# CUG-EMI/HMCMT2D

Measured on NVIDIA B200. Metric: leapfrog_steps_per_sec, higher is better.
Workload: dtype f64 (complex128)

## Files before the change

hmcmt2d_b200/csrc/hmcmt_b200.cu:

```cuda
#include <dlfcn.h>
#include <nccl.h>

#include <algorithm>
#include <cmath>
#include <cstdlib>
#include <cstring>
#include <new>
#include <vector>

#include "../../include/hmcmt_b200.h"
#include "band_factor.cuh"
#include "band_solve.cuh"
#include "mf_solver.cuh"
#include "mt_kernels.cuh"

using namespace hmcmt;

namespace {

template <typename Tp>
struct DevBuf {
    Tp* p = nullptr;
    size_t n = 0;
    int alloc(size_t count) {
// ... 796 lines not shown
        pl->useMf = pl->T == 0 || wantMf;
        if (pl->useMf) pl->T = 0;
    }
    {
        const char* env = std::getenv("HMCMT_SPLIT");
        int want = env ? std::atoi(env) : 1;
        pl->dom = BandDom{M.N, M.nf, pl->b, M.nl, (!pl->useMf && want && M.nl >= 9) ? 1 : 0, M.nl / 2};
        if (!pl->useMf) {
            LocalDom L0 = LocalDom::make(pl->dom, 0);
            pl->steps0 = L0.sTot;
            pl->steps1 = pl->dom.split ? LocalDom::make(pl->dom, 1).sOwn : 0;
            pl->S = pl->steps0 + pl->steps1;
        }
    }
    pl->nSysPerChain = pl->nModes * pl->nFreq;
    pl->nSys = pl->nSysPerChain * pl->nChains;
    pl->nFull = pl->nFreq * pl->nRx * pl->nComp;
    pl->sm = SysMap{pl->nFreq, pl->nModes, pl->modeList[0], pl->modeList[1]};
    pl->h_yLen.assign(pr->yLen, pr->yLen + ny);
    pl->h_zLen.assign(pr->zLen, pr->zLen + nz);
    pl->h_freqs.assign(pr->freqs, pr->freqs + pr->nFreq);
    std::vector<double> yNode(ny + 1), zNode0(nz + 1), zNode(nz + 1);
    yNode[0] = 0; zNode0[0] = 0;
    for (int j = 0; j < ny; ++j) yNode[j + 1] = yNode[j] + pr->yLen[j];
    for (int k = 0; k < nz; ++k) zNode0[k + 1] = zNode0[k] + pr->zLen[k];
    for (auto& v : yNode) v -= pr->origin[0];
    for (int k = 0; k <= nz; ++k) zNode[k] = zNode0[k] - pr->origin[1];
    int zid = -1;
    for (int k = 0; k <= nz; ++k) if (std::fabs(zNode[k] - pr->rxLoc[1]) < 0.1) { zid = k; break; }
    if (zid < 0 || zid >= nz) { delete pl; return kErrArg; }
    M.zid = zid;
    std::vector<double> yCen(ny);
    for (int j = 0; j < ny; ++j) yCen[j] = 0.5 * (yNode[j] + yNode[j + 1]);
    std::vector<int> fid(pr->nRx), iL(pr->nRx), iR(pr->nRx), tjL(pr->nRx), tjR(pr->nRx);
    std::vector<double> d1(pr->nRx), d2(pr->nRx), wL(pr->nRx), wR(pr->nRx), twL(pr->nRx), twR(pr->nRx);
    for (int r = 0; r < pr->nRx; ++r) {
        double y = pr->rxLoc[2 * r];
        int id = -1;
        for (int j = 0; j <= ny; ++j) if (yNode[j] > y) { id = j; break; }
        if (id <= 0) { delete pl; return kErrArg; }
        fid[r] = id; d1[r] = y - yNode[id - 1]; d2[r] = yNode[id] - y;
        linear_interp(y, yNode, iL[r], iR[r], wL[r], wR[r]);
        linear_interp(y, yCen, tjL[r], tjR[r], twL[r], twR[r]);
    }
    std::vector<double> wdFull(pl->nFull, 0.0), wpFull(dataKind ? pl->nFull : 0, 0.0);
    std::vector<cplx> obsFull(pl->nFull, mk(0.0, 0.0));
    pl->h_packed2full.resize(pr->nData);
    const long nDt = dataKind ? 2 * pr->nComp : pr->nComp;
    long prev = -1;
    for (int i = 0; i < pr->nData; ++i) {
        long f = pr->freqID[i] - 1, r = pr->rxID[i] - 1, c = pr->dtID[i] - 1;
        if (f < 0 || f >= pr->nFreq || r < 0 || r >= pr->nRx || c < 0 || c >= nDt) { delete pl; return kErrArg; }
        const long ci = dataKind ? c / 2 : c, part = dataKind ? c % 2 : 0;
        const long slot = (f * pr->nRx + r) * pl->nComp + ci;
        const long full = dataKind ? 2 * slot + part : slot;
        if (full <= prev) {
            fprintf(stderr, "[hmcmt_b200] data rows must be sorted by (freq, rx, comp) without duplicates\n");
            delete pl;
            return kErrArg;
        }
        prev = full;
        pl->h_packed2full[i] = (int)full;
        const double w = 1.0 / std::fabs(pr->dataErr[i]);
        if (!dataKind) {
            wdFull[slot] = w;
            obsFull[slot] = mk(pr->obsData[2 * i], pr->obsData[2 * i + 1]);
        } else if (part == 0) {
            wdFull[slot] = w;
            obsFull[slot].x = pr->obsData[i];
        } else {
            wpFull[slot] = w;
            obsFull[slot].y = pr->obsData[i];
        }
    }
    std::vector<int> cell2act(M.nCell, -1);
    for (int a = 0; a < pr->nAC; ++a) {
        int c = pr->activeIdx[a];
        if (c < 0 || c >= M.nCell) { delete pl; return kErrArg; }
        cell2act[c] = a;
    }
    int rc = kOk;
    auto ok = [&](int r) { if (r && !rc) rc = r; };
    ok(pl->yLen.upload(pr->yLen, ny)); ok(pl->zLen.upload(pr->zLen, nz)); ok(pl->zNode.upload(zNode0.data(), nz + 1));
    ok(pl->freqs.upload(pr->freqs, pr->nFreq));
    ok(pl->fid.upload(fid.data(), pr->nRx)); ok(pl->iL.upload(iL.data(), pr->nRx)); ok(pl->iR.upload(iR.data(), pr->nRx));
    ok(pl->fdy1.upload(d1.data(), pr->nRx)); ok(pl->fdy2.upload(d2.data(), pr->nRx));
    ok(pl->wL.upload(wL.data(), pr->nRx)); ok(pl->wR.upload(wR.data(), pr->nRx));
    ok(pl->tjL.upload(tjL.data(), pr->nRx)); ok(pl->tjR.upload(tjR.data(), pr->nRx));
    ok(pl->twL.upload(twL.data(), pr->nRx)); ok(pl->twR.upload(twR.data(), pr->nRx));
    ok(pl->cell2act.upload(cell2act.data(), M.nCell)); ok(pl->act2cell.upload(pr->activeIdx, pr->nAC));
    ok(pl->bg.upload(pr->bgModel, M.nCell));
    ok(pl->wmPtr.upload(pr->wmRowPtr, pr->nAC + 1));
    int nnzWm = pr->wmRowPtr[pr->nAC];
    ok(pl->wmIdx.upload(pr->wmColIdx, nnzWm)); ok(pl->wmVal.upload(pr->wmVal, nnzWm));
    ok(pl->wd.upload(wdFull.data(), pl->nFull)); ok(pl->obs.upload(obsFull.data(), pl->nFull));
    ok(pl->wdPha.upload(wpFull.data(), wpFull.size()));
    ok(pl->packed2full.upload(pl->h_packed2full.data(), pr->nData));
    {
        std::vector<int> f2p((dataKind ? 2 : 1) * (size_t)pl->nFull, -1);
        for (int i = 0; i < pr->nData; ++i) f2p[pl->h_packed2full[i]] = i;
        ok(pl->full2packed.upload(f2p.data(), f2p.size()));
    }
    const size_t nCh = pl->nChains, nSys = pl->nSys, N = M.N;
    ok(pl->m.alloc(nCh * pr->nAC)); ok(pl->p.alloc(nCh * pr->nAC)); ok(pl->mref.alloc(nCh * pr->nAC));
    ok(pl->curM.alloc(nCh * pr->nAC)); ok(pl->curP.alloc(nCh * pr->nAC)); ok(pl->zmom.alloc(nCh * pr->nAC)); ok(pl->driftPart.alloc(nCh * 128));
    ok(pl->sigma.alloc(nCh * M.nCell)); ok(pl->meanSig.alloc(nCh * nz));
    ok(pl->planes.alloc(nCh * pl->nModes * 4 * N));
    ok(pl->bc.alloc(nSys * M.nb)); ok(pl->bcs.alloc(nSys * M.nb));
    ok(pl->rhs.alloc(nSys * N)); ok(pl->x.alloc(nSys * N)); ok(pl->lam.alloc(nSys * N));
    ok(pl->F.alloc(nSys * M.nNode)); ok(pl->Lam.alloc(nSys * M.nNode));
    ok(pl->srows.alloc(nSys * 2 * (ny + 1))); ok(pl->qrow.alloc(nSys * ny));
    ok(pl->scratch.alloc(nSys * 3 * prof_stride(nz)));
    ok(pl->Gpart.alloc(nSys * M.nCell)); ok(pl->phiPart.alloc(nSys)); ok(pl->phi.alloc(nCh));
    ok(pl->gsig.alloc(nCh * pr->nAC)); ok(pl->gdata.alloc(nCh * pr->nAC)); ok(pl->gtotal.alloc(nCh * pr->nAC)); ok(pl->xbuf.alloc((size_t)nCh * (pl->nAC + 1))); ok(pl->energies.alloc(nCh * 2));
    ok(pl->chainScal.alloc(nCh * 4));
    ok(pl->predFull.alloc(nCh * pl->nFull)); ok(pl->respFull.alloc(nCh * pl->nFull)); ok(pl->vin.alloc(nCh * pl->nFull)); ok(pl->predPacked.alloc(nCh * pr->nData));
    ok(pl->panels.alloc(nSys * (size_t)pl->S * panel_doubles(pl->T)));
    ok(pl->ainvz.alloc(nSys * (size_t)pl->S * AZ)); ok(pl->zadj.alloc(nSys * (size_t)pl->S * 8));
    const size_t wexpN = split_scratch_entries(TS * pl->T);
    ok(pl->wexp.alloc(pl->dom.split ? nSys * wexpN : 0));
    ok(pl->conCols.alloc(nSys * contract_cols_out(ny, nz)));
    ok(pl->fwdJobs.alloc(nSys));
    ok(pl->status.alloc(nSys)); ok(pl->driftFlag.alloc(1)); ok(pl->Lsteps.alloc(nCh));
    ok(pl->sysDesc.alloc(nSys)); ok(pl->jobs.alloc(nSys));
    if (rc) { hmcmt_destroy(pl); return rc; }
    cudaMemset(pl->status.p, 0, sizeof(int) * nSys);
    cudaMemset(pl->driftFlag.p, 0, sizeof(int));
    cudaMemset(pl->m.p, 0, sizeof(double) * nCh * pr->nAC);
    cudaMemset(pl->p.p, 0, sizeof(double) * nCh * pr->nAC);
    cudaMemset(pl->mref.p, 0, sizeof(double) * nCh * pr->nAC);
    M.yLen = pl->yLen.p; M.zLen = pl->zLen.p; M.zNode = pl->zNode.p;
    pl->rx = RxDev{pr->nRx, pl->fid.p, pl->fdy1.p, pl->fdy2.p, pl->iL.p, pl->iR.p, pl->wL.p, pl->wR.p, pl->tjL.p, pl->tjR.p, pl->twL.p, pl->twR.p};
    std::vector<BandSys> sd(nSys);
    std::vector<SolveJob> jb(nSys), jfw(nSys);
    for (size_t s = 0; s < nSys; ++s) {
        int f = (int)(s % pl->nFreq);
        int t = (int)(s / pl->nFreq);
        int mi = t % pl->nModes, ch = t / pl->nModes;
        double* P = pl->planes.p + ((size_t)(ch * pl->nModes + mi) * 4) * N;
        BandSys& d = sd[s];
        d.dr = P; d.dm = P + N; d.e1 = P + 2 * N; d.e2 = P + 3 * N;
        d.omega = 2.0 * kPi * pr->freqs[f];
        d.band = nullptr;
        d.rhs = pl->rhs.p + s * N;
        d.panels[0] = pl->panels.p + s * (size_t)pl->S * panel_doubles(pl->T);
        d.panels[1] = d.panels[0] + (size_t)pl->steps0 * panel_doubles(pl->T);
        d.ainvz[0] = pl->ainvz.p + s * (size_t)pl->S * AZ;
        d.ainvz[1] = d.ainvz[0] + (size_t)pl->steps0 * AZ;
        d.wexp = pl->dom.split ? pl->wexp.p + s * wexpN : nullptr;
        d.x = pl->x.p + s * N;
        d.status = pl->status.p + s;
        SolveJob& j = jb[s];
        j.panels[0] = d.panels[0]; j.panels[1] = d.panels[1];
        j.ainvz[0] = d.ainvz[0]; j.ainvz[1] = d.ainvz[1];
        j.rhs = pl->lam.p + s * N; j.x = pl->lam.p + s * N;
        j.zbuf[0] = pl->zadj.p + s * (size_t)pl->S * 8;
        j.zbuf[1] = j.zbuf[0] + (size_t)pl->steps0 * 8;
        j.wexp = d.wexp;
        SolveJob& jf = jfw[s];
        jf = j;
        jf.rhs = nullptr; jf.x = d.x;
    }
    if (cudaMemcpy(pl->sysDesc.p, sd.data(), sizeof(BandSys) * nSys, cudaMemcpyHostToDevice) != cudaSuccess ||
        cudaMemcpy(pl->jobs.p, jb.data(), sizeof(SolveJob) * nSys, cudaMemcpyHostToDevice) != cudaSuccess ||
        (pl->fwdJobs.p && cudaMemcpy(pl->fwdJobs.p, jfw.data(), sizeof(SolveJob) * nSys, cudaMemcpyHostToDevice) != cudaSuccess)) {
        hmcmt_destroy(pl);
        return kErrCuda;
    }
    {
        const size_t rxSmem = (size_t)(6 * (M.ny + 1) + 3 * M.ny) * sizeof(cplx);
        const size_t bcSmem = (size_t)boundary_profiles_per_block(M.nz) * M.nz * 6 * sizeof(cplx);
        if (bcSmem > 227 * 1024) {
            fprintf(stderr, "[hmcmt_b200] nz = %d: the boundary kernel needs %zu bytes of shared memory per profile\n", M.nz, bcSmem);
            hmcmt_destroy(pl);
            return kErrArg;
        }
        if (bcSmem > 48 * 1024 && cudaFuncSetAttribute(k_boundary, cudaFuncAttributeMaxDynamicSharedMemorySize, (int)bcSmem) != cudaSuccess) {
            hmcmt_destroy(pl);
            return kErrCuda;
        }
        pl->conStaged = contract_cols_smem(M.ny, M.nz, 1) <= 200 * 1024 ? 1 : 0;
        const size_t cSmem = contract_cols_smem(M.ny, M.nz, pl->conStaged);
        if ((rxSmem > 48 * 1024 && cudaFuncSetAttribute(rx_kernel(pl), cudaFuncAttributeMaxDynamicSharedMemorySize, (int)rxSmem) != cudaSuccess) ||
            (cSmem > 48 * 1024 && cudaFuncSetAttribute(k_contract_cols, cudaFuncAttributeMaxDynamicSharedMemorySize, (int)cSmem) != cudaSuccess)) {
            hmcmt_destroy(pl);
            return kErrArg;
        }
    }
    if (pl->useMf) {
        std::vector<std::vector<int>> sn;
        std::vector<mf::Entry> ent;
        mf::mf_order_grid(M.nl, M.nf, mf_leaf_size(), sn, mf_cross_size(), mf_push_size());
        mf::mf_grid_entries(M.nl, M.nf, ent);
        mf::Symbolic S;
        if (!mf::mf_symbolic(M.N, sn, ent, mf_small_front(), S)) { hmcmt_destroy(pl); return kErrArg; }
        int mrc = kOk;
        pl->mfs = mf::Solver::create(std::move(S), pl->nSys, 2, 3 * (int64_t)M.N, &mrc);
        if (!pl->mfs) { hmcmt_destroy(pl); return mrc; }
        std::vector<unsigned char> nzR(M.N, 0), nzA(M.N, 0);
        for (int kn = 1; kn <= nz - 1; ++kn)
            for (int jn = 1; jn <= ny - 1; ++jn) {
                const int q = M.fastZ ? (jn - 1) * M.nf + (kn - 1) : (kn - 1) * M.nf + (jn - 1);
                if (jn == 1 || jn == ny - 1 || kn == 1 || kn == nz - 1) nzR[q] = 1;
                if (kn == M.zid || kn == M.zid + 1) nzA[q] = 1;
            }
        pl->patRx = pl->mfs->add_rhs_pattern(nzA);
        if (pl->patRx < 0) { hmcmt_destroy(pl); return kErrAlloc; }
        if (const char* e = std::getenv("HMCMT_MF_PRUNE"); !e || std::atoi(e)) {
            pl->patRhs = pl->mfs->add_rhs_pattern(nzR);
            pl->patAdj = pl->patRx;
            if (pl->patRhs < 0) { hmcmt_destroy(pl); return kErrAlloc; }
        }
        std::vector<mf::MtValSys> mv(nSys);
        for (size_t s = 0; s < nSys; ++s) { mv[s].planes = sd[s].dr; mv[s].omega = sd[s].omega; }
        if (pl->mfSys.upload(mv.data(), nSys) != kOk) { hmcmt_destroy(pl); return kErrAlloc; }
    }
    if (cudaStreamCreateWithFlags(&pl->stream, cudaStreamNonBlocking) != cudaSuccess ||
        cudaStreamCreateWithFlags(&pl->side, cudaStreamNonBlocking) != cudaSuccess ||
        cudaEventCreateWithFlags(&pl->evFork, cudaEventDisableTiming) != cudaSuccess ||
        cudaEventCreateWithFlags(&pl->evJoin, cudaEventDisableTiming) != cudaSuccess ||
        cudaEventCreateWithFlags(&pl->evPre, cudaEventDisableTiming) != cudaSuccess ||
        cudaEventCreateWithFlags(&pl->evRhs, cudaEventDisableTiming) != cudaSuccess ||
        cudaEventCreate(&pl->evA) != cudaSuccess || cudaEventCreate(&pl->evB) != cudaSuccess) {
        hmcmt_destroy(pl);
        return kErrCuda;
    }
    if (const char* e = std::getenv("HMCMT_GRAPH"); e && !std::atoi(e)) pl->graphState = -1;
    if (pl->useMf) {
        const char* env = std::getenv("HMCMT_GROUPS");
        int G = env ? std::atoi(env) : kDefaultGroups;
        G = std::max(1, std::min(G, std::min(pl->nSys, 8)));
        for (int g = 0; G >= 2 && g < G; ++g) {
            cudaStream_t s = nullptr;
            cudaEvent_t e = nullptr;
            if (cudaStreamCreateWithFlags(&s, cudaStreamNonBlocking) != cudaSuccess) { hmcmt_destroy(pl); return kErrCuda; }
            pl->groupStreams.push_back(s);
            if (cudaEventCreateWithFlags(&e, cudaEventDisableTiming) != cudaSuccess) { hmcmt_destroy(pl); return kErrCuda; }
            pl->groupDone.push_back(e);
        }
    }
    *out = pl;
    return kOk;
}

int hmcmt_plan_create(const hmcmt_problem* pr, hmcmt_plan** out) { return plan_create(pr, out, 0); }
int hmcmt_plan_create_rho_phase(const hmcmt_problem* pr, hmcmt_plan** out) { return plan_create(pr, out, 1); }

void hmcmt_destroy(hmcmt_plan* pl) {
    if (!pl) return;
    cudaSetDevice(pl->device);
    if (pl->comm) {
        if (pl->stream) cudaStreamSynchronize(pl->stream);
        if (NcclApi* a = nccl_api()) a->commDestroy(pl->comm);
        pl->comm = nullptr;
    }
    if (pl->stream) { cudaStreamSynchronize(pl->stream); cudaStreamDestroy(pl->stream); }
    if (pl->side) { cudaStreamSynchronize(pl->side); cudaStreamDestroy(pl->side); }
    if (pl->graphExec) cudaGraphExecDestroy(pl->graphExec);
    for (cudaStream_t s : pl->groupStreams) { cudaStreamSynchronize(s); cudaStreamDestroy(s); }
    for (cudaEvent_t e : pl->groupDone) cudaEventDestroy(e);
    if (pl->evPre) cudaEventDestroy(pl->evPre);
    if (pl->evRhs) cudaEventDestroy(pl->evRhs);
    if (pl->evFork) cudaEventDestroy(pl->evFork);
    if (pl->evJoin) cudaEventDestroy(pl->evJoin);
    if (pl->evA) cudaEventDestroy(pl->evA);
    if (pl->evB) cudaEventDestroy(pl->evB);
    for (auto& e : pl->factorEvents) { cudaEventDestroy(e.first); cudaEventDestroy(e.second); }
    for (cudaEvent_t e : pl->factorMid) cudaEventDestroy(e);
    pl->yLen.release(); pl->zLen.release(); pl->zNode.release(); pl->freqs.release(); pl->fdy1.release(); pl->fdy2.release();
    pl->wL.release(); pl->wR.release(); pl->twL.release(); pl->twR.release(); pl->tjL.release(); pl->tjR.release(); pl->bg.release(); pl->wmVal.release(); pl->wd.release(); pl->wdPha.release(); pl->m.release(); pl->p.release();
    pl->mref.release(); pl->sigma.release(); pl->meanSig.release(); pl->planes.release(); pl->Gpart.release(); pl->phiPart.release();
    pl->phi.release(); pl->gsig.release(); pl->gdata.release(); pl->gtotal.release(); pl->energies.release(); pl->panels.release(); pl->curM.release();
    pl->curP.release(); pl->driftPart.release(); pl->chainScal.release(); pl->zmom.release(); pl->fid.release(); pl->iL.release(); pl->iR.release();
    pl->cell2act.release(); pl->act2cell.release(); pl->wmPtr.release(); pl->wmIdx.release(); pl->status.release();
    pl->driftFlag.release(); pl->packed2full.release(); pl->full2packed.release(); pl->Lsteps.release(); pl->obs.release(); pl->bc.release(); pl->bcs.release();
    pl->rhs.release(); pl->x.release(); pl->F.release(); pl->lam.release(); pl->Lam.release(); pl->srows.release(); pl->qrow.release();
    pl->scratch.release(); pl->predFull.release(); pl->ainvz.release(); pl->zadj.release(); pl->vin.release();
    pl->predPacked.release(); pl->conCols.release(); pl->dbc.release(); pl->jvFull.release(); pl->dsigA.release(); pl->gnBuf.release(); pl->gnVec.release(); pl->gnPart.release(); pl->gnS.release(); pl->gnE.release(); pl->gnAct.release(); pl->gnI.release(); pl->xbuf.release(); pl->wexp.release(); pl->respFull.release(); pl->gradK.release(); pl->Lband.release(); pl->massBuf.release(); pl->massStatus.release(); delete pl->massSolver; pl->massSolver = nullptr; pl->mfSys.release(); delete pl->mfs; pl->mfs = nullptr; pl->fwdJobs.release(); pl->sysDesc.release(); pl->jobs.release();
    if (pl->pin) cudaFreeHost(pl->pin);
    delete pl;
}

int64_t hmcmt_plan_info(const hmcmt_plan* pl, int what) {
    if (!pl) return -1;
    switch (what) {
        case 0: return pl->M.N;
        case 1: return pl->M.nNode;
        case 2: return pl->M.nCell;
        case 3: return pl->M.nb;
        case 4: return pl->b;
        case 5: return pl->T;
        case 6: return pl->S;
        case 7: return pl->nSysPerChain;
        case 8: return pl->M.zid;
        case 9: return pl->useMf ? pl->mfs->factor_doubles() * 8 : (int64_t)pl->S * (panel_doubles(pl->T) * 8 + AZ * 16);
        case 10: return pl->launches;
        case 11: return pl->useMf ? 1 : 0;
        case 12: return pl->useMf ? (int64_t)pl->mfs->factor_flops() : (int64_t)(4.0 * pl->M.N * (double)pl->b * pl->b);
        case 13: return pl->dom.split;
        default: return -1;
    }
}

int hmcmt_sync(hmcmt_plan* pl) {
    if (!pl) return kErrArg;
    HMCMT_CUDA_TRY(cudaStreamSynchronize(pl->stream));
    return kOk;
}
int hmcmt_set_mass_matrix(hmcmt_plan* pl, int32_t kind) {
    if (!pl || kind < 0 || kind > 1) return kErrArg;
    HMCMT_CUDA_TRY(cudaSetDevice(pl->device));
    if (kind == 0) { pl->massOn = false; return kOk; }
    if (pl->massSolver) { pl->massOn = true; return kOk; }
    const int n = pl->nAC;
    std::vector<int> ptr(n + 1), idx;
    std::vector<double> val;
    HMCMT_CUDA_TRY(cudaMemcpy(ptr.data(), pl->wmPtr.p, sizeof(int) * (n + 1), cudaMemcpyDeviceToHost));
    idx.resize(ptr[n]); val.resize(ptr[n]);
    HMCMT_CUDA_TRY(cudaMemcpy(idx.data(), pl->wmIdx.p, sizeof(int) * ptr[n], cudaMemcpyDeviceToHost));
    HMCMT_CUDA_TRY(cudaMemcpy(val.data(), pl->wmVal.p, sizeof(double) * ptr[n], cudaMemcpyDeviceToHost));
    std::vector<mf::Entry> ent;
    std::vector<int> aptr(n + 1, 0);
    int bw = 0;
    for (int a = 0; a < n; ++a)
        for (int q = ptr[a]; q < ptr[a + 1]; ++q) {
            const int j = idx[q];
            if (j > a) continue;
            ent.push_back(mf::Entry{a, j, q});
            bw = std::max(bw, a - j);
            if (j != a) { ++aptr[a + 1]; ++aptr[j + 1]; }
        }
    for (int a = 0; a < n; ++a) aptr[a + 1] += aptr[a];
    std::vector<int> adj(aptr[n]), at(aptr.begin(), aptr.end() - 1);
    for (const mf::Entry& e : ent)
        if (e.row != e.col) { adj[at[e.row]++] = e.col; adj[at[e.col]++] = e.row; }
    std::vector<std::vector<int>> sn;
    mf::mf_order_graph(n, aptr, adj, mf_leaf_size(), sn);
    mf::Symbolic S;
    if (!mf::mf_symbolic(n, sn, ent, mf_small_front(), S)) return kErrArg;
    int rc = kOk;
    pl->massSolver = mf::Solver::create(std::move(S), 1, pl->nChains, (int64_t)ptr[n], &rc);
    if (!pl->massSolver) return rc;
    {
        std::vector<cplx> cv(ptr[n]);
        for (int q = 0; q < ptr[n]; ++q) cv[q] = mk(val[q], 0.0);
        HMCMT_CUDA_TRY(cudaMemcpy(pl->massSolver->vals(), cv.data(), sizeof(cplx) * cv.size(), cudaMemcpyHostToDevice));
    }
    if ((rc = pl->massStatus.alloc(1)) != kOk) return rc;
    HMCMT_CUDA_TRY(cudaMemset(pl->massStatus.p, 0, sizeof(int)));
    rc = pl->massSolver->factor(pl->stream, pl->massStatus.p, &pl->launches);
    if (rc) return rc;
    int hst = 0;
    HMCMT_CUDA_TRY(cudaMemcpyAsync(&hst, pl->massStatus.p, sizeof(int), cudaMemcpyDeviceToHost, pl->stream));
    HMCMT_CUDA_TRY(cudaStreamSynchronize(pl->stream));
    if (hst) return hst;
    std::vector<double> Lb((size_t)n * (bw + 1), 0.0);
    for (int a = 0; a < n; ++a)
        for (int q = ptr[a]; q < ptr[a + 1]; ++q)
            if (idx[q] <= a) Lb[(size_t)a * (bw + 1) + (a - idx[q])] = val[q];
    for (int j = 0; j < n; ++j) {
        double* rj = Lb.data() + (size_t)j * (bw + 1);
        double d = rj[0];
        for (int k = std::max(0, j - bw); k < j; ++k) d -= rj[j - k] * rj[j - k];
        if (!(d > 0.0)) return kErrNotPosDef;
        d = std::sqrt(d);
        rj[0] = d;
        for (int i = j + 1; i <= std::min(n - 1, j + bw); ++i) {
            double* ri = Lb.data() + (size_t)i * (bw + 1);
            double v = ri[i - j];
            for (int k = std::max(0, i - bw); k < j; ++k) v -= ri[i - k] * rj[j - k];
            ri[i - j] = v / d;
        }
    }
    if ((rc = pl->Lband.upload(Lb.data(), Lb.size())) != kOk) return rc;
    if ((rc = pl->gradK.alloc((size_t)pl->nChains * n)) != kOk) return rc;
    if ((rc = pl->massBuf.alloc((size_t)pl->nChains * n)) != kOk) return rc;
    pl->massBw = bw;
    pl->massOn = true;
    return kOk;
}

int hmcmt_status(hmcmt_plan* pl) {
    if (!pl) return kErrArg;
    HMCMT_CUDA_TRY(cudaSetDevice(pl->device));
    return check_status(pl);
}
int hmcmt_set_response_kind(hmcmt_plan* pl, int32_t kind) {
    if (!pl || kind < 0 || kind > 1) return kErrArg;
    pl->respKind = kind;
    return kOk;
}
int hmcmt_get_responses(hmcmt_plan* pl, double* out) {
    if (!pl || !out || !pl->haveForward) return kErrArg;
    HMCMT_CUDA_TRY(cudaSetDevice(pl->device));
    const cplx* src = (pl->respKind == 1 || pl->dataKind == 1) ? pl->respFull.p : pl->predFull.p;
    HMCMT_CUDA_TRY(cudaMemcpyAsync(out, src, sizeof(cplx) * (size_t)pl->nChains * pl->nFull, cudaMemcpyDeviceToHost, pl->stream));
    HMCMT_CUDA_TRY(cudaStreamSynchronize(pl->stream));
    return kOk;
}
int hmcmt_timer_start(hmcmt_plan* pl) {
    if (!pl) return kErrArg;
    HMCMT_CUDA_TRY(cudaEventRecord(pl->evA, pl->stream));
    return kOk;
}
int hmcmt_timer_stop(hmcmt_plan* pl, float* ms) {
    if (!pl || !ms) return kErrArg;
    HMCMT_CUDA_TRY(cudaEventRecord(pl->evB, pl->stream));
    HMCMT_CUDA_TRY(cudaEventSynchronize(pl->evB));
    HMCMT_CUDA_TRY(cudaEventElapsedTime(ms, pl->evA, pl->evB));
    return kOk;
}
int hmcmt_kernel_time_split(hmcmt_plan* pl, float* factor_only_ms, float* forward_solve_ms) {
    if (!pl) return kErrArg;
    HMCMT_CUDA_TRY(cudaStreamSynchronize(pl->stream));
    float a = 0.f, b = 0.f;
    for (size_t i = 0; i < pl->factorEventsUsed; ++i) {
        float ms = 0.f;
        HMCMT_CUDA_TRY(cudaEventElapsedTime(&ms, pl->factorEvents[i].first, pl->factorMid[i]));
        a += ms;
        HMCMT_CUDA_TRY(cudaEventElapsedTime(&ms, pl->factorMid[i], pl->factorEvents[i].second));
        b += ms;
    }
    if (factor_only_ms) *factor_only_ms = a;
    if (forward_solve_ms) *forward_solve_ms = b;
    return kOk;
}
int hmcmt_kernel_time(hmcmt_plan* pl, int reset, float* factor_ms, int64_t* factor_launches) {
    if (!pl) return kErrArg;
    HMCMT_CUDA_TRY(cudaStreamSynchronize(pl->stream));
    float tot = 0.f;
    for (size_t i = 0; i < pl->factorEventsUsed; ++i) {
        float ms = 0.f;
        HMCMT_CUDA_TRY(cudaEventElapsedTime(&ms, pl->factorEvents[i].first, pl->factorEvents[i].second));
        tot += ms;
    }
    if (factor_ms) *factor_ms = tot;
    if (factor_launches) *factor_launches = (int64_t)pl->factorEventsUsed;
    if (reset) { pl->factorEventsUsed = 0; pl->timeFactor = reset > 0; }
    return kOk;
}

static int upload_model(hmcmt_plan* pl, const double* m) {
    size_t bytes = sizeof(double) * (size_t)pl->nChains * pl->nAC;
    int rc = ensure_pin(pl, std::max(bytes, (size_t)1 << 20));
    if (rc) return rc;
    std::memcpy(pl->pin, m, bytes);
    HMCMT_CUDA_TRY(cudaMemcpyAsync(pl->m.p, pl->pin, bytes, cudaMemcpyHostToDevice, pl->stream));
    return kOk;
}
static size_t datum_bytes(const hmcmt_plan* pl) { return pl->dataKind ? sizeof(double) : sizeof(cplx); }
static int pack_pred(hmcmt_plan* pl) {
    const dim3 grid((pl->nData + 255) / 256, pl->nChains);
    if (pl->dataKind)
        k_pack_pred_real<<<grid, 256, 0, pl->stream>>>(pl->nData, pl->nFull, pl->packed2full.p, reinterpret_cast<const double*>(pl->respFull.p),
                                                       reinterpret_cast<double*>(pl->predPacked.p));
    else
        k_pack_pred<<<grid, 256, 0, pl->stream>>>(pl->nData, pl->nFull, pl->packed2full.p, pl->predFull.p, pl->predPacked.p);
    LAUNCH_CHECK(pl);
    return kOk;
}
static int download_pred(hmcmt_plan* pl, double* pred) {
    int rc = pack_pred(pl);
    if (rc) return rc;
    HMCMT_CUDA_TRY(cudaMemcpyAsync(pred, pl->predPacked.p, datum_bytes(pl) * (size_t)pl->nChains * pl->nData, cudaMemcpyDeviceToHost, pl->stream));
    return kOk;
}

static int forward_common(hmcmt_plan* pl, double* pred, double* exTE, double* hxTM);

int hmcmt_forward(hmcmt_plan* pl, const double* m, double* pred, double* exTE, double* hxTM) {
    if (!pl || !m) return kErrArg;
    HMCMT_CUDA_TRY(cudaSetDevice(pl->device));
    pl->sigmaDirect = false;
    int rc = upload_model(pl, m);
    if (rc) return rc;
    return forward_common(pl, pred, exTE, hxTM);
}

int hmcmt_forward_sigma(hmcmt_plan* pl, const double* sigma, double* pred, double* exTE, double* hxTM) {
    if (!pl || !sigma) return kErrArg;
    HMCMT_CUDA_TRY(cudaSetDevice(pl->device));
    pl->sigmaDirect = true;
    HMCMT_CUDA_TRY(cudaMemcpyAsync(pl->sigma.p, sigma, sizeof(double) * (size_t)pl->nChains * pl->M.nCell, cudaMemcpyHostToDevice, pl->stream));
    HMCMT_CUDA_TRY(cudaStreamSynchronize(pl->stream));
    return forward_common(pl, pred, exTE, hxTM);
}

static int forward_common(hmcmt_plan* pl, double* pred, double* exTE, double* hxTM) {
    int rc = compute_step(pl, false, nullptr);
    if (rc) return rc;
    if (pred) { rc = download_pred(pl, pred); if (rc) return rc; }
    const MeshDev& M = pl->M;
    for (int ch = 0; ch < pl->nChains; ++ch)
        for (int mi = 0; mi < pl->nModes; ++mi) {
            double* dst = pl->modeList[mi] == 0 ? exTE : hxTM;
            if (!dst) continue;
            size_t sys0 = ((size_t)ch * pl->nModes + mi) * pl->nFreq;
            HMCMT_CUDA_TRY(cudaMemcpyAsync(dst + 2 * (size_t)ch * pl->nFreq * M.nNode, pl->F.p + sys0 * M.nNode,
                                           sizeof(cplx) * (size_t)pl->nFreq * M.nNode, cudaMemcpyDeviceToHost, pl->stream));
        }
    HMCMT_CUDA_TRY(cudaStreamSynchronize(pl->stream));
    return check_status(pl);
}

int hmcmt_jtvec(hmcmt_plan* pl, const double* v, double* gsig) {
    if (!pl || !v || !gsig) return kErrArg;
    if (!pl->haveForward) return kErrArg;
    HMCMT_CUDA_TRY(cudaSetDevice(pl->device));
    std::vector<cplx> full((size_t)pl->nChains * pl->nFull, mk(0.0, 0.0));
    double* fullD = reinterpret_cast<double*>(full.data());
    for (int ch = 0; ch < pl->nChains; ++ch)
        for (int i = 0; i < pl->nData; ++i) {
            const size_t src = (size_t)ch * pl->nData + i;
            if (pl->dataKind) fullD[(size_t)ch * 2 * pl->nFull + pl->h_packed2full[i]] = v[src];
            else full[(size_t)ch * pl->nFull + pl->h_packed2full[i]] = mk(v[2 * src], v[2 * src + 1]);
        }
    HMCMT_CUDA_TRY(cudaMemcpyAsync(pl->vin.p, full.data(), sizeof(cplx) * full.size(), cudaMemcpyHostToDevice, pl->stream));
    HMCMT_CUDA_TRY(cudaStreamSynchronize(pl->stream));
    int rc = kOk;
    if (!pl->haveSens) rc = launch_sens_side(pl);
    if (rc) return rc;
    rc = rx_phase(pl, true, pl->vin.p);
    if (rc) return rc;
    rc = adjoint_phase(pl);
    if (rc) return rc;
    HMCMT_CUDA_TRY(cudaMemcpyAsync(gsig, pl->gsig.p, sizeof(double) * (size_t)pl->nChains * pl->nAC, cudaMemcpyDeviceToHost, pl->stream));
    HMCMT_CUDA_TRY(cudaStreamSynchronize(pl->stream));
    return check_status(pl);
}

int hmcmt_jacobian(hmcmt_plan* pl, double* J) {
    if (!pl || !J || !pl->haveForward) return kErrArg;
    HMCMT_CUDA_TRY(cudaSetDevice(pl->device));
    const MeshDev& M = pl->M;
    cudaStream_t st = pl->stream;
    const size_t nJ = (size_t)pl->nChains * pl->nData * pl->nAC * (pl->dataKind ? 1 : 2);
    DevBuf<double> dJ;
    int rc = dJ.alloc(nJ);
    if (rc) return rc;
    HMCMT_CUDA_TRY(cudaMemsetAsync(dJ.p, 0, nJ * sizeof(double), st));
    if (!pl->haveSens) rc = launch_sens_side(pl);
    struct Group { unsigned mask; int2 comp; };
    std::vector<Group> groups;
    const CompMap& cm = pl->cm;
    if (!pl->tipper) groups.push_back(Group{(1u << pl->nComp) - 1u, make_int2(0, 1)});
    else if (cm.zc[0] >= 0 || cm.zc[1] >= 0)
        groups.push_back(Group{(cm.zc[0] >= 0 ? 1u << cm.zc[0] : 0u) | (cm.zc[1] >= 0 ? 1u << cm.zc[1] : 0u), make_int2(cm.zc[0], cm.zc[1])});
    if (pl->tipper) groups.push_back(Group{1u << cm.tc, make_int2(cm.tmi == 0 ? cm.tc : -1, cm.tmi == 1 ? cm.tc : -1)});
    for (const Group& grp : groups)
        for (int r = 0; r < pl->nRx && rc == kOk; ++r)
            for (int part = 0; part < 2 && rc == kOk; ++part) {
                k_jac_vin<<<dim3((pl->nFull + 255) / 256, pl->nChains), 256, 0, st>>>(pl->nFull, pl->nRx, pl->nComp, grp.mask, r,
                                                                                     part == 0 ? mk(1.0, 0.0) : mk(0.0, 1.0), pl->vin.p);
                ++pl->launches;
                rc = rx_phase(pl, true, pl->vin.p);
                if (rc == kOk) rc = adjoint_phase(pl, false);
                if (rc != kOk) break;
                const dim3 grid((pl->nAC + 255) / 256, pl->nSys);
                if (pl->dataKind)
                    k_jac_rows_real<<<grid, 256, 0, st>>>(pl->nAC, M.nCell, pl->nFreq, pl->nRx, pl->nModes, pl->nData, r, part, pl->act2cell.p,
                                                          pl->full2packed.p, pl->Gpart.p, dJ.p);
                else
                    k_jac_rows<<<grid, 256, 0, st>>>(pl->nAC, M.nCell, pl->nFreq, pl->nRx, pl->nModes, pl->nComp, grp.comp, pl->nData, r,
                                                     part, pl->act2cell.p, pl->full2packed.p, pl->Gpart.p, dJ.p);
                ++pl->launches;
            }
    if (rc == kOk && cudaGetLastError() != cudaSuccess) rc = kErrCuda;
    if (rc == kOk && cudaMemcpyAsync(J, dJ.p, nJ * sizeof(double), cudaMemcpyDeviceToHost, st) != cudaSuccess) rc = kErrCuda;
    if (cudaStreamSynchronize(st) != cudaSuccess && rc == kOk) rc = kErrCuda;
    dJ.release();
    if (rc) return rc;
    rc = rx_phase(pl, false, nullptr);
    if (rc) return rc;
    return check_status(pl);
}

static int ensure_tangent(hmcmt_plan* pl) {
    if (pl->jvFull.p) return kOk;
    const MeshDev& M = pl->M;
    int rc;
    if ((rc = pl->dbc.alloc((size_t)pl->nSys * M.nb)) || (rc = pl->dsigA.alloc((size_t)pl->nChains * pl->nAC))) return rc;
    const size_t smem = (size_t)(6 * (M.ny + 1) + 2 * M.ny) * sizeof(cplx);
    auto k = pl->dataKind ? k_rx_tangent<true, false> : pl->tipper ? k_rx_tangent<false, true> : k_rx_tangent<false, false>;
    if (smem > 48 * 1024) HMCMT_CUDA_TRY(cudaFuncSetAttribute(k, cudaFuncAttributeMaxDynamicSharedMemorySize, (int)smem));
    return pl->jvFull.alloc((size_t)pl->nChains * pl->nFull);
}

static int jvec_device(hmcmt_plan* pl) {
    const MeshDev& M = pl->M;
    cudaStream_t st = pl->stream;
    const int nSys = pl->nSys;
    int rc = kOk;
    if (!pl->haveSens && (rc = launch_sens_side(pl))) return rc;
    HMCMT_CUDA_TRY(cudaStreamWaitEvent(st, pl->evJoin, 0));
    k_bc_tangent<<<dim3((M.ny + 1 + 127) / 128, nSys), 128, 0, st>>>(M, pl->sm, pl->freqs.p, pl->cell2act.p, pl->dsigA.p, pl->nAC,
                                                                     pl->scratch.p, pl->dbc.p);
    LAUNCH_CHECK(pl);
    k_tangent_rhs<<<dim3((M.N + 255) / 256, nSys), 256, 0, st>>>(M, pl->sm, pl->freqs.p, pl->sigma.p, pl->cell2act.p, pl->dsigA.p, pl->nAC,
                                                                 pl->F.p, pl->bcs.p, pl->dbc.p, pl->lam.p);
    LAUNCH_CHECK(pl);
    if (pl->useMf) {
        if ((rc = pl->mfs->forward_slot(st, 0, pl->lam.p, M.N, &pl->launches, 0, nSys, 0)) ||
            (rc = pl->mfs->backward_slot(st, 0, pl->lam.p, M.N, &pl->launches, 0, nSys, pl->patRx)))
            return rc;
    } else {
        if ((rc = launch_solve(st, pl->T, pl->jobs.p, nSys, pl->dom))) return rc;
// ... 555 lines not shown
```

hmcmt2d_b200/csrc/mf_kernels.cuh:

```cuda
#pragma once
#include "band_factor.cuh"
#include "mf_solver.cuh"

namespace hmcmt {
namespace mf {

__host__ __device__ __forceinline__ size_t kg_off(int ld, int i, int j, int plane) {
    return ((size_t)((j >> 2) * 2 + plane) * ld + i) * 4 + (j & 3);
}

struct Tables {
    const Front* fronts;
    const int* rows;
    const int* rel;
    const int* children;
    const OrigEntry* orig;
    const Chunk* chunks;
    const int* pos2orig;
    double* fac;
    double* arena[2];
    int64_t facStride, arenaStride[2];
    const cplx* vals;
    int64_t valStride;
    int* status;
    unsigned long long* prof;
};
#define MF_PROF_MARK(slot) do { if (tb.prof && threadIdx.x == 0) { const long long _t = clock64(); atomicAdd(tb.prof + _pc * 8 + (slot), (unsigned long long)(_t - _t0)); _t0 = _t; } } while (0)

__device__ __forceinline__ int tl_off(int r, int c) { return ((c >> 2) << 5) | (r << 2) | (c & 3); }
__device__ __forceinline__ double* mf_tile(double* tiles, int I, int J) { return tiles + (size_t)(I * (I + 1) / 2 + J) * 128; }
__device__ __forceinline__ int mf_pc_row(int I, int npb) { return I < npb ? I * (I + 1) / 2 : npb * (npb + 1) / 2 + (I - npb) * npb; }
template <bool PC>
__device__ __forceinline__ double* mf_tile(double* tiles, int npb, int I, int J) {
    return PC ? tiles + (size_t)(mf_pc_row(I, npb) + J) * 128 : mf_tile(tiles, I, J);
}

struct TileFrag {
    double re[2], im[2];
};
__device__ __forceinline__ void frag_load(TileFrag& f, const double* T, int lane) {
    f.re[0] = T[lane]; f.re[1] = T[32 + lane]; f.im[0] = T[64 + lane]; f.im[1] = T[96 + lane];
}
__device__ __forceinline__ void frag_load_t(TileFrag& f, const double* T, int g, int t) {
    const int o0 = tl_off(t, g), o1 = tl_off(4 + t, g);
    f.re[0] = T[o0]; f.re[1] = T[o1]; f.im[0] = T[64 + o0]; f.im[1] = T[64 + o1];
}
__device__ __forceinline__ void frag_store(const TileFrag& f, double* T, int lane) {
    T[lane] = f.re[0]; T[32 + lane] = f.re[1]; T[64 + lane] = f.im[0]; T[96 + lane] = f.im[1];
}
__device__ __forceinline__ void cfrag_load(TileFrag& c, const double* T, int g, int t) {
    const int o = tl_off(g, 2 * t);
    const double2 r = *reinterpret_cast<const double2*>(T + o), i = *reinterpret_cast<const double2*>(T + 64 + o);
    c.re[0] = r.x; c.re[1] = r.y; c.im[0] = i.x; c.im[1] = i.y;
}
__device__ __forceinline__ void cfrag_store(const TileFrag& c, double* T, int g, int t, double sign = 1.0) {
    const int o = tl_off(g, 2 * t);
    *reinterpret_cast<double2*>(T + o) = make_double2(sign * c.re[0], sign * c.re[1]);
    *reinterpret_cast<double2*>(T + 64 + o) = make_double2(sign * c.im[0], sign * c.im[1]);
}
__device__ __forceinline__ void frag_mma(TileFrag& c, TileFrag& x, const TileFrag& a, const TileFrag& b) {
#pragma unroll
    for (int kk = 0; kk < 2; ++kk) {
        dmma884(c.re, a.re[kk], b.re[kk]);
        dmma884(c.im, a.re[kk], b.im[kk]);
        dmma884(x.re, -a.im[kk], b.im[kk]);
        dmma884(x.im, a.im[kk], b.re[kk]);
    }
}
__device__ __forceinline__ void frag_zero(TileFrag& c) { c.re[0] = c.re[1] = c.im[0] = c.im[1] = 0.0; }
__device__ __forceinline__ void frag_add(TileFrag& c, const TileFrag& x) {
    c.re[0] += x.re[0]; c.re[1] += x.re[1]; c.im[0] += x.im[0]; c.im[1] += x.im[1];
}

template <int NW, bool PC = false, bool STREAM = false>
__device__ __forceinline__ void mf_front_factor(double* __restrict__ tiles, double* __restrict__ scratch, double* __restrict__ mbuf,
                                                double* __restrict__ nainv, int* __restrict__ fail, const int nb, const int npb,
                                                const int sReal, unsigned long long* __restrict__ prof = nullptr,
                                                double* mglob = nullptr, const int ldm = 0) {
    const int tid = threadIdx.x, lane = tid & 31;
    long long _s0 = prof ? clock64() : 0;
#define MF_SWEEP_MARK(slot) do { if (prof && tid == 0) { const long long _t = clock64(); atomicAdd(prof + (slot), (unsigned long long)(_t - _s0)); _s0 = _t; } } while (0)
    const int warp = __shfl_sync(0xffffffffu, tid >> 5, 0);
    const int g = lane >> 2, t = lane & 3;
    double* const rawb = scratch;
    double* const mmb = scratch + (size_t)npb * 128;
    for (int kb = 0; kb < npb; ++kb) {
        if (warp == 0) {
            const double* D = mf_tile(tiles, kb, kb);
            auto sym = [&](int r, int c, int pl) { return r >= c ? D[pl * 64 + tl_off(r, c)] : D[pl * 64 + tl_off(c, r)]; };
            cplx a0 = mk(sym(g, 2 * t, 0), sym(g, 2 * t, 1)), a1 = mk(sym(g, 2 * t + 1, 0), sym(g, 2 * t + 1, 1));
            bool bad = false;
            const int left = sReal - 8 * kb;
            gj_invert8<(NW > 4)>(a0, a1, bad, g, t, left < 8 ? (left < 0 ? 0 : left) : 8);
            if (__any_sync(0xffffffffu, bad) && lane == 0) *fail = 1;
            TileFrag p;
            p.re[0] = -a0.x; p.re[1] = -a1.x; p.im[0] = -a0.y; p.im[1] = -a1.y;
            cfrag_store(p, nainv, g, t);
            __syncwarp();
            double* Dw = mf_tile(tiles, kb, kb);
            cfrag_store(p, Dw, g, t);
        }
        if (npb == 1) break;
        __syncthreads();
        MF_SWEEP_MARK(0);
        for (int I = warp; I < npb; I += NW) {
            if (I == kb) continue;
            TileFrag a, b, c, x;
            if (I > kb) frag_load(a, mf_tile(tiles, I, kb), lane);
            else frag_load_t(a, mf_tile(tiles, kb, I), g, t);
            frag_load(b, nainv, lane);
            frag_zero(c); frag_zero(x);
            frag_mma(c, x, a, b);
            frag_add(c, x);
            frag_store(a, rawb + (size_t)I * 128, lane);
            cfrag_store(c, mmb + (size_t)I * 128, g, t);
        }
        __syncthreads();
        MF_SWEEP_MARK(1);
        {
            int I = 0, J = warp;
            while (J > I) { J -= I + 1; ++I; }
            for (int L = warp; L < npb * (npb + 1) / 2; L += NW) {
                double* T = mf_tile(tiles, I, J);
                if (I == kb && J == kb) {
                } else if (J == kb) {
                    TileFrag c;
                    cfrag_load(c, mmb + (size_t)I * 128, g, t);
                    cfrag_store(c, T, g, t, -1.0);
                } else if (I == kb) {
                    const double* Ms = mmb + (size_t)J * 128;
                    TileFrag c;
                    c.re[0] = Ms[tl_off(2 * t, g)]; c.re[1] = Ms[tl_off(2 * t + 1, g)];
                    c.im[0] = Ms[64 + tl_off(2 * t, g)]; c.im[1] = Ms[64 + tl_off(2 * t + 1, g)];
                    cfrag_store(c, T, g, t, -1.0);
                } else {
                    TileFrag a, b, c, x;
                    frag_load(a, mmb + (size_t)I * 128, lane);
                    frag_load(b, rawb + (size_t)J * 128, lane);
                    cfrag_load(c, T, g, t);
                    frag_zero(x);
                    frag_mma(c, x, a, b);
                    frag_add(c, x);
                    cfrag_store(c, T, g, t);
                }
                J += NW;
                while (J > I) { J -= I + 1; ++I; }
            }
        }
        __syncthreads();
        MF_SWEEP_MARK(1);
    }
    const int nub = nb - npb;
    if (nub == 0) { __syncthreads(); return; }
    __syncthreads();
    if (npb == 1) MF_SWEEP_MARK(0);
    for (int Iu = warp; Iu < nub; Iu += NW) {
        const int I = npb + Iu;
        for (int kb = 0; kb < npb; ++kb) {
            TileFrag c, x;
            frag_zero(c); frag_zero(x);
            for (int j = 0; j < npb; ++j) {
                TileFrag a, b;
                frag_load(a, mf_tile<PC>(tiles, npb, I, j), lane);
                if (kb >= j) frag_load(b, mf_tile(tiles, kb, j), lane);
                else frag_load_t(b, mf_tile(tiles, j, kb), g, t);
                frag_mma(c, x, a, b);
            }
            frag_add(c, x);
            if (STREAM) {
                double* o = mglob + kg_off(ldm, 8 * Iu + g, 8 * kb + 2 * t, 0);
                *reinterpret_cast<double2*>(o) = make_double2(-c.re[0], -c.re[1]);
                *reinterpret_cast<double2*>(o + 4 * ldm) = make_double2(-c.im[0], -c.im[1]);
            } else {
                cfrag_store(c, mbuf + (size_t)(Iu * npb + kb) * 128, g, t);
            }
        }
    }
    __syncthreads();
    MF_SWEEP_MARK(2);
    if (PC) return;
    {
        const int nU = nub * (nub + 1) / 2;
        int I = 0, J = warp;
        while (J > I) { J -= I + 1; ++I; }
        constexpr bool kPair = NW > 4;
        for (int L = warp; L < nU; L += (kPair ? 2 : 1) * NW) {
            const int I0 = I, J0 = J;
            J += NW;
            while (J > I) { J -= I + 1; ++I; }
            const bool two = kPair && L + NW < nU;
            const int I1 = I, J1 = J;
            if (kPair) {
                J += NW;
                while (J > I) { J -= I + 1; ++I; }
            }
            double* T0 = mf_tile(tiles, npb + I0, npb + J0);
            double* T1 = mf_tile(tiles, npb + I1, npb + J1);
            TileFrag c0, x0, c1, x1;
            cfrag_load(c0, T0, g, t);
            frag_zero(x0);
            if (two) { cfrag_load(c1, T1, g, t); frag_zero(x1); }
            for (int kb = 0; kb < npb; ++kb) {
                TileFrag a, b;
                frag_load(a, mbuf + (size_t)(I0 * npb + kb) * 128, lane);
                frag_load(b, mf_tile(tiles, npb + J0, kb), lane);
                frag_mma(c0, x0, a, b);
                if (two) {
                    frag_load(a, mbuf + (size_t)(I1 * npb + kb) * 128, lane);
                    frag_load(b, mf_tile(tiles, npb + J1, kb), lane);
                    frag_mma(c1, x1, a, b);
                }
            }
            frag_add(c0, x0);
            cfrag_store(c0, T0, g, t);
            if (two) { frag_add(c1, x1); cfrag_store(c1, T1, g, t); }
        }
    }
    __syncthreads();
    MF_SWEEP_MARK(3);
#undef MF_SWEEP_MARK
}

template <bool TRANSPOSED>
__device__ __forceinline__ void mf_store_tile(const double* __restrict__ T, double* __restrict__ dst, int ld, int row0, int col0,
                                              double sign, int lane) {
#pragma unroll
    for (int h = 0; h < 2; ++h) {
        const int idx = lane + 32 * h;
        const int chunk = idx >> 4, w = idx & 15, pl = chunk >> 1, cg = chunk & 1, r = w >> 1, c2 = (w & 1) * 2;
        double2 v;
        if (!TRANSPOSED) v = *reinterpret_cast<const double2*>(T + chunk * 32 + w * 2);
        else v = make_double2(T[pl * 64 + tl_off(cg * 4 + c2, r)], T[pl * 64 + tl_off(cg * 4 + c2 + 1, r)]);
        double* out = dst + kg_off(ld, row0 + r, col0 + cg * 4, pl) + c2;
        *reinterpret_cast<double2*>(out) = make_double2(sign * v.x, sign * v.y);
    }
}

template <int NW, bool STREAM>
__device__ __forceinline__ void mf_small_front(const Tables& tb, const SmallDesc* __restrict__ descs) {
    constexpr int NT = NW * 32;
    constexpr bool kMid = NW >= 8;
    static_assert(!STREAM || kMid, "streamed M' exists in the pivot-column layout only");
    extern __shared__ __align__(16) unsigned char mf_smem[];
    SmallDesc& F = *reinterpret_cast<SmallDesc*>(mf_smem);
    const int sys = blockIdx.y, tid = threadIdx.x, lane = tid & 31;
    const int warp = __shfl_sync(0xffffffffu, tid >> 5, 0);
    constexpr int _pc = NW <= 2 ? 0 : (NW == 4 ? 1 : (NW == 8 ? 2 : 3));
    long long _t0 = clock64();
    static_assert(sizeof(SmallDesc) % 4 == 0 && sizeof(SmallDesc) <= kFrontDescBytes, "SmallDesc is copied word by word into the head of the dynamic shared memory");
    for (int i = tid; i < (int)(sizeof(SmallDesc) / 4); i += NT)
        reinterpret_cast<int*>(&F)[i] = reinterpret_cast<const int*>(descs + blockIdx.x)[i];
    __syncthreads();
    const int fp = F.sp + F.up, nb = fp >> 3, npb = F.sp >> 3, nub = nb - npb;
    const int nT = kMid ? mf_pc_row(nb, npb) : nb * (nb + 1) / 2;
    double* tiles = reinterpret_cast<double*>(mf_smem + kFrontDescBytes);
    double* mbuf = tiles + (size_t)nT * 128;
    double* nainv = mbuf + (size_t)(STREAM || 2 * npb > nub * npb ? 2 * npb : nub * npb) * 128;
    int* fail = reinterpret_cast<int*>(nainv + 128);
    int2* relS = reinterpret_cast<int2*>(fail + 4);
    auto rel_parts = [npb](int r) {
        return make_int2((kMid ? mf_pc_row(r >> 3, npb) : (r >> 3) * ((r >> 3) + 1) / 2) * 128 + (r & 7) * 4, (r >> 3) * 128 + ((r & 4) << 3) + (r & 3));
    };
    const int nChild = F.nChild;
    {
        int base = 0;
        for (int c = 0; c < nChild; ++c) {
            const int cu = F.cU[c];
            const int* rel = tb.rel + F.cRel[c];
            for (int i = tid; i < cu; i += NT) relS[base + i] = rel_parts(rel[i]);
            base += cu;
        }
    }
    int* invS = reinterpret_cast<int*>(relS + ((F.cU[0] + F.cU[1] + F.cU[2] + F.cU[3] + 1) & ~1));
    const double* carena = tb.arena[F.par ^ 1] + (size_t)sys * tb.arenaStride[F.par ^ 1];
    constexpr int kBatch = 1;
    struct Batch {
        double2 r01[kBatch], r23[kBatch], i01[kBatch], i23[kBatch];
        int ii[kBatch], jg[kBatch];
        int c;
    };
    int curC = 0, curQ = warp * kBatch;
    auto load_batch = [&](Batch& bt) {
        while (curC < nChild) {
            const int cu = F.cU[curC];
            if (curQ < (((kMid ? F.cPiv[curC] : cu) + 3) >> 2) * ((cu + 31) >> 5)) break;
            ++curC;
            curQ = warp * kBatch;
        }
        bt.c = curC < nChild ? curC : -1;
        if (bt.c < 0) return;
        const int cu = F.cU[curC], ld = F.cLd[curC], off = F.cFirst[curC];
        const double* U = carena + F.cOff[curC];
        const int ng = ((kMid ? F.cPiv[curC] : cu) + 3) >> 2, nrb = (cu + 31) >> 5;
#pragma unroll
        for (int bq = 0; bq < kBatch; ++bq) {
            const int q = curQ + bq;
            const int jg = nrb == 1 ? q : q / nrb, i = (q - jg * nrb) * 32 + lane;
            bt.jg[bq] = jg;
            bt.ii[bq] = (q < ng * nrb && i < cu && i >= 4 * jg) ? i : -1;
            if (bt.ii[bq] >= 0) {
                const double* pr = U + kg_off(ld, off + i, off + 4 * jg, 0);
                const double* pi = U + kg_off(ld, off + i, off + 4 * jg, 1);
                bt.r01[bq] = *reinterpret_cast<const double2*>(pr); bt.r23[bq] = *reinterpret_cast<const double2*>(pr + 2);
                bt.i01[bq] = *reinterpret_cast<const double2*>(pi); bt.i23[bq] = *reinterpret_cast<const double2*>(pi + 2);
            }
        }
        curQ += NW * kBatch;
    };
    Batch b0, b1;
    load_batch(b0);
    load_batch(b1);
    const cplx* vals = tb.vals + (size_t)sys * tb.valStride;
    OrigEntry oe0{0, 0, -1};
    cplx ov0 = mk(0.0, 0.0);
    if (tid < F.nOrig) {
        oe0 = tb.orig[F.origPtr + tid];
        ov0 = oe0.src < 0 ? mk(1.0, 0.0) : vals[oe0.src];
    }
    for (int i = tid; i < nT * 64; i += NT) reinterpret_cast<double2*>(tiles)[i] = make_double2(0.0, 0.0);
    if (kMid)
        for (int i = tid; i < nChild * F.up; i += NT) invS[i] = -1;
    if (tid == 0) *fail = 0;
    __syncthreads();
    MF_PROF_MARK(0);
    if (kMid) {
        int base = 0;
        for (int c = 0; c < nChild; ++c) {
            const int cu = F.cU[c];
            const int* rel = tb.rel + F.cRel[c];
            for (int i = F.cPiv[c] + tid; i < cu; i += NT) invS[base + rel[i] - F.sp] = i;
            base += F.up;
        }
    }
    auto addr = [&](int a, int b) {
        return tiles + (size_t)((kMid ? mf_pc_row(a >> 3, npb) : (a >> 3) * ((a >> 3) + 1) / 2) + (b >> 3)) * 128 + tl_off(a & 7, b & 7);
    };
    {
        auto scatter = [&](const Batch& bt) {
            const int2* relC = relS + ((bt.c > 0 ? F.cU[0] : 0) + (bt.c > 1 ? F.cU[1] : 0) + (bt.c > 2 ? F.cU[2] : 0));
            const int jEnd = kMid ? F.cPiv[bt.c] : 0;
#pragma unroll
            for (int bq = 0; bq < kBatch; ++bq) {
                const int i = bt.ii[bq];
                if (i < 0) continue;
                const int jg = bt.jg[bq];
                const double re[4] = {bt.r01[bq].x, bt.r01[bq].y, bt.r23[bq].x, bt.r23[bq].y};
                const double im[4] = {bt.i01[bq].x, bt.i01[bq].y, bt.i23[bq].x, bt.i23[bq].y};
                double* rowp = tiles + relC[i].x;
#pragma unroll
                for (int jj = 0; jj < 4; ++jj) {
                    if (4 * jg + jj > i || (kMid && 4 * jg + jj >= jEnd)) break;
                    double* d = rowp + relC[4 * jg + jj].y;
                    d[0] += re[jj];
                    d[64] += im[jj];
                }
            }
        };
        for (int c = 0; c < nChild; ++c) {
            while (b0.c == c) {
                scatter(b0);
                b0 = b1;
                load_batch(b1);
            }
            __syncwarp();
            __syncthreads();
        }
        if (nChild == 0) __syncthreads();
    }
    MF_PROF_MARK(2);
    if (tid < F.nOrig) {
        double* d = addr(oe0.lrow, oe0.lcol);
        d[0] += ov0.x;
        d[64] += ov0.y;
    }
    for (int e = tid + NT; e < F.nOrig; e += NT) {
        const OrigEntry oe = tb.orig[F.origPtr + e];
        const cplx v = oe.src < 0 ? mk(1.0, 0.0) : vals[oe.src];
        double* d = addr(oe.lrow, oe.lcol);
        d[0] += v.x;
        d[64] += v.y;
    }
    __syncthreads();
    MF_PROF_MARK(1);
    double* fac = tb.fac + (size_t)sys * tb.facStride;
    mf_front_factor<NW, kMid, STREAM>(tiles, mbuf, mbuf, nainv, fail, nb, npb, F.s, tb.prof ? tb.prof + 32 + _pc * 4 : nullptr,
                                      fac + F.mOff, F.up);
    if (kMid && nub > 0) {
        const long long tD = tb.prof ? clock64() : 0;
        const int g = lane >> 2, t = lane & 3, up = F.up;
        double* U = tb.arena[F.par] + (size_t)sys * tb.arenaStride[F.par] + F.uOff;
        auto gather = [&](TileFrag& c, int I, int J) {
            const int a = 8 * I + g, b = 8 * J + 2 * t;
            frag_zero(c);
#pragma unroll
            for (int ch = 0; ch < kSmallChildren; ++ch) {
                const int* inv = invS + ch * up;
                const int ia = ch < nChild ? inv[a] : -1;
                if (ia < 0) continue;
                const int ib0 = inv[b], ib1 = inv[b + 1];
                const double* Uc = carena + F.cOff[ch];
                const int ld = F.cLd[ch], off = F.cFirst[ch];
                if (ib0 >= 0 && ib0 <= ia) { c.re[0] += Uc[kg_off(ld, off + ia, off + ib0, 0)]; c.im[0] += Uc[kg_off(ld, off + ia, off + ib0, 1)]; }
                if (ib1 >= 0 && ib1 <= ia) { c.re[1] += Uc[kg_off(ld, off + ia, off + ib1, 0)]; c.im[1] += Uc[kg_off(ld, off + ia, off + ib1, 1)]; }
            }
        };
        auto store = [&](const TileFrag& c, int I, int J) {
            double* o = U + kg_off(up, 8 * I + g, 8 * J + 2 * t, 0);
            *reinterpret_cast<double2*>(o) = make_double2(c.re[0], c.re[1]);
            *reinterpret_cast<double2*>(o + 4 * up) = make_double2(c.im[0], c.im[1]);
        };
        if (!STREAM) {
            const int nU = nub * (nub + 1) / 2;
            int I = 0, J = warp;
            while (J > I) { J -= I + 1; ++I; }
            for (int L = warp; L < nU; L += 2 * NW) {
                const int I0 = I, J0 = J;
                J += NW;
                while (J > I) { J -= I + 1; ++I; }
                const bool two = L + NW < nU;
                const int I1 = I, J1 = J;
                J += NW;
                while (J > I) { J -= I + 1; ++I; }
                TileFrag c0, x0, c1, x1;
                gather(c0, I0, J0);
                frag_zero(x0);
                if (two) { gather(c1, I1, J1); frag_zero(x1); }
                for (int kb = 0; kb < npb; ++kb) {
                    TileFrag a, b;
                    frag_load(a, mbuf + (size_t)(I0 * npb + kb) * 128, lane);
                    frag_load(b, mf_tile<true>(tiles, npb, npb + J0, kb), lane);
                    frag_mma(c0, x0, a, b);
                    if (two) {
                        frag_load(a, mbuf + (size_t)(I1 * npb + kb) * 128, lane);
                        frag_load(b, mf_tile<true>(tiles, npb, npb + J1, kb), lane);
                        frag_mma(c1, x1, a, b);
                    }
                }
                frag_add(c0, x0);
                store(c0, I0, J0);
                if (two) { frag_add(c1, x1); store(c1, I1, J1); }
            }
        } else {
            constexpr int kRow = 4;
            const double* Mg = fac + F.mOff;
            auto load_a = [&](TileFrag& a, int I, int kb) {
#pragma unroll
                for (int kk = 0; kk < 2; ++kk) {
                    const double* p = Mg + kg_off(up, 8 * I + g, 8 * kb + 4 * kk + t, 0);
                    a.re[kk] = -p[0];
                    a.im[kk] = -p[4 * up];
                }
            };
            int I = 0, q = warp;
            while (q > I / kRow) { q -= I / kRow + 1; ++I; }
            while (I < nub) {
                const int J0 = kRow * q, nJ = min(kRow, I + 1 - J0);
                TileFrag c[kRow], x[kRow];
#pragma unroll
                for (int r = 0; r < kRow; ++r)
                    if (r < nJ) { gather(c[r], I, J0 + r); frag_zero(x[r]); }
                TileFrag a;
                load_a(a, I, 0);
                for (int kb = 0; kb < npb; ++kb) {
                    TileFrag an;
                    if (kb + 1 < npb) load_a(an, I, kb + 1);
#pragma unroll
                    for (int r = 0; r < kRow; ++r)
                        if (r < nJ) {
                            TileFrag b;
                            frag_load(b, mf_tile<true>(tiles, npb, npb + J0 + r, kb), lane);
                            frag_mma(c[r], x[r], a, b);
                        }
                    a = an;
                }
#pragma unroll
                for (int r = 0; r < kRow; ++r)
                    if (r < nJ) { frag_add(c[r], x[r]); store(c[r], I, J0 + r); }
                q += NW;
                while (I < nub && q > I / kRow) { q -= I / kRow + 1; ++I; }
            }
        }
        if (tb.prof && tid == 0) atomicAdd(tb.prof + 32 + _pc * 4 + 3, (unsigned long long)(clock64() - tD));
    }
    MF_PROF_MARK(4);
    if (tid == 0 && *fail) tb.status[sys] = kErrSingular;
    const int sp = F.sp, up = F.up;
    {
        double* G = fac + F.gOff;
        for (int I = warp; I < npb; I += NW)
            for (int J = 0; J < npb; ++J) {
                if (I >= J) mf_store_tile<false>(mf_tile(tiles, I, J), G, sp, I * 8, J * 8, -1.0, lane);
                else mf_store_tile<true>(mf_tile(tiles, J, I), G, sp, I * 8, J * 8, -1.0, lane);
            }
    }
    if (!STREAM && up > 0) {
        double* M = fac + F.mOff;
        for (int I = warp; I < nub; I += NW)
            for (int J = 0; J < npb; ++J) mf_store_tile<false>(mbuf + (size_t)(I * npb + J) * 128, M, up, I * 8, J * 8, -1.0, lane);
    }
    if (!kMid && up > 0) {
        double* U = tb.arena[F.par] + (size_t)sys * tb.arenaStride[F.par] + F.uOff;
        int I = 0, J = warp;
        while (J > I) { J -= I + 1; ++I; }
        for (int L = warp; L < nub * (nub + 1) / 2; L += NW) {
            mf_store_tile<false>(mf_tile(tiles, npb + I, npb + J), U, up, I * 8, J * 8, 1.0, lane);
            J += NW;
            while (J > I) { J -= I + 1; ++I; }
        }
    }
    MF_PROF_MARK(5);
    if (tb.prof && tid == 0) { atomicAdd(tb.prof + _pc * 8 + 6, 1ull); atomicAdd(tb.prof + _pc * 8 + 7, (unsigned long long)npb); }
}

template <int NW>
__global__ void __launch_bounds__(NW * 32, NW <= 4 ? (NW == 1 ? 16 : 32 / NW) : (NW == 8 ? 4 : 2))
mf_small_kernel(Tables tb, const SmallDesc* __restrict__ descs) {
    mf_small_front<NW, false>(tb, descs);
}
__global__ void __launch_bounds__(16 * 32, 1) mf_small_stream_kernel(Tables tb, const SmallDesc* __restrict__ descs) {
    mf_small_front<16, true>(tb, descs);
}

__global__ void mf_asm_orig_kernel(Tables tb, const int2* __restrict__ pairs, int n) {
    const int idx = blockIdx.x * blockDim.x + threadIdx.x, sys = blockIdx.y;
    if (idx >= n) return;
    const int2 pr = pairs[idx];
    const Front& F = tb.fronts[pr.x];
    const OrigEntry oe = tb.orig[pr.y];
    const cplx v = oe.src < 0 ? mk(1.0, 0.0) : tb.vals[(size_t)sys * tb.valStride + oe.src];
    double* A = tb.arena[F.depth & 1] + (size_t)sys * tb.arenaStride[F.depth & 1] + F.frontOff;
    const int fp = F.sp + F.up;
    A[kg_off(fp, oe.lrow, oe.lcol, 0)] += v.x;
    A[kg_off(fp, oe.lrow, oe.lcol, 1)] += v.y;
}
struct AsmTile {
    int front, bi, bj;
    int invPtr;
};
__global__ void __launch_bounds__(256)
mf_asm_gather_kernel(Tables tb, const AsmTile* __restrict__ tilesList, const int* __restrict__ invMaps) {
    const AsmTile at = tilesList[blockIdx.x];
    const int sys = blockIdx.y;
    const Front P = tb.fronts[at.front];
    const int fp = P.sp + P.up, par = P.depth & 1;
    double* A = tb.arena[par] + (size_t)sys * tb.arenaStride[par] + P.frontOff;
    const double* carena = tb.arena[par ^ 1] + (size_t)sys * tb.arenaStride[par ^ 1];
    for (int item = threadIdx.x; item < 64 * 16; item += 256) {
        const int a = at.bi * 64 + (item & 63), b0 = at.bj * 64 + (item >> 6) * 4;
        if (a >= fp || b0 >= ((a >> 3) + 1) * 8) continue;
        double re[4] = {0.0, 0.0, 0.0, 0.0}, im[4] = {0.0, 0.0, 0.0, 0.0};
        for (int c = 0; c < P.nChild; ++c) {
            const int* inv = invMaps + at.invPtr + (size_t)c * fp;
            const int ia = inv[a];
            if (ia < 0) continue;
            const Front& C = tb.fronts[tb.children[P.childPtr + c]];
            const int ld = C.isBig ? C.sp + C.up : C.up, off = C.isBig ? C.sp : 0;
            const double* U = carena + C.frontOff;
#pragma unroll
            for (int k = 0; k < 4; ++k) {
                if (b0 + k > a) break;
                const int ib = inv[b0 + k];
                if (ib < 0) continue;
                re[k] += U[kg_off(ld, off + ia, off + ib, 0)];
                im[k] += U[kg_off(ld, off + ia, off + ib, 1)];
            }
        }
        double* pr = A + kg_off(fp, a, b0, 0);
        double* pi = A + kg_off(fp, a, b0, 1);
        *reinterpret_cast<double2*>(pr) = make_double2(re[0], re[1]); *reinterpret_cast<double2*>(pr + 2) = make_double2(re[2], re[3]);
        *reinterpret_cast<double2*>(pi) = make_double2(im[0], im[1]); *reinterpret_cast<double2*>(pi + 2) = make_double2(im[2], im[3]);
    }
}

constexpr int kInvWarps = 8;
__global__ void __launch_bounds__(kInvWarps * 32)
mf_inv_kernel(Tables tb, const int* __restrict__ list, int c) {
    constexpr int NT = kInvWarps * 32;
    extern __shared__ __align__(16) unsigned char mf_smem[];
    const Front F = tb.fronts[list[blockIdx.x]];
    const Chunk ch = tb.chunks[F.chunkPtr + c];
    const int sys = blockIdx.y, tid = threadIdx.x, lane = tid & 31, warp = tid >> 5;
    const int sc = ch.p1 - ch.p0, nb = sc >> 3, fp = F.sp + F.up;
    const int nT = nb * (nb + 1) / 2;
    double* tiles = reinterpret_cast<double*>(mf_smem);
    double* scratch = tiles + (size_t)nT * 128;
    double* nainv = scratch + (size_t)2 * nb * 128;
    int* fail = reinterpret_cast<int*>(nainv + 128);
    const double* A = tb.arena[F.depth & 1] + (size_t)sys * tb.arenaStride[F.depth & 1] + F.frontOff;
    if (tid == 0) *fail = 0;
    for (int idx = tid; idx < nT * 64; idx += NT) {
        const int L = idx >> 6, w = idx & 63, chunk = w >> 4, pl = chunk >> 1, cg = chunk & 1, r = (w & 15) >> 1, c2 = (w & 1) * 2;
        int I = 0, J = L;
        while (J > I) { J -= I + 1; ++I; }
        const double* src = A + kg_off(fp, ch.p0 + I * 8 + r, ch.p0 + J * 8 + cg * 4, pl) + c2;
        *reinterpret_cast<double2*>(tiles + (size_t)L * 128 + chunk * 32 + (w & 15) * 2) = *reinterpret_cast<const double2*>(src);
    }
    __syncthreads();
    const int sReal = F.s - ch.p0 < sc ? (F.s - ch.p0 < 0 ? 0 : F.s - ch.p0) : sc;
    mf_front_factor<kInvWarps>(tiles, scratch, scratch, nainv, fail, nb, nb, sReal);
    if (tid == 0 && *fail) tb.status[sys] = kErrSingular;
    double* G = tb.fac + (size_t)sys * tb.facStride + ch.gOff;
    for (int q = warp; q < nb * nb; q += kInvWarps) {
        const int I = q / nb, J = q - I * nb;
        if (I >= J) mf_store_tile<false>(mf_tile(tiles, I, J), G, sc, I * 8, J * 8, -1.0, lane);
        else mf_store_tile<true>(mf_tile(tiles, J, I), G, sc, I * 8, J * 8, -1.0, lane);
    }
}

struct GemmJob {
    int64_t aOff, bOff, cOff;
    int aSp, bSp, cSp;
    int ldA, rA, kA, ldB, rB, kB, ldC, rC, cC;
    int m, n, K;
    int lower, beta;
    double alpha;
};
struct GemmTile {
    int job, bi, bj;
};
constexpr int kGemmKC = 16, kGemmStages = 3, kGemmThreads = 256;
constexpr int kGemmStageDoubles = 2 * (kGemmKC / 4) * 2 * 64 * 4;
constexpr size_t kGemmSmemBytes = (size_t)kGemmStages * kGemmStageDoubles * sizeof(double);

__global__ void __launch_bounds__(kGemmThreads)
mf_gemm_kernel(Tables tb, const GemmJob* __restrict__ jobs, const GemmTile* __restrict__ tilesList) {
    extern __shared__ __align__(16) unsigned char mf_smem[];
    double* sm = reinterpret_cast<double*>(mf_smem);
    const GemmTile gt = tilesList[blockIdx.x];
    const GemmJob jb = jobs[gt.job];
    const int sys = blockIdx.y, tid = threadIdx.x, lane = tid & 31;
    const int warp = __shfl_sync(0xffffffffu, tid >> 5, 0);
    const int g = lane >> 2, t = lane & 3;
    const int wr = warp >> 1, wc = warp & 1;
    auto base = [&](int sp, int64_t off) -> double* {
        return (sp == 2 ? tb.fac + (size_t)sys * tb.facStride : tb.arena[sp] + (size_t)sys * tb.arenaStride[sp]) + off;
    };
    const double* A = base(jb.aSp, jb.aOff);
    const double* B = base(jb.bSp, jb.bOff);
    double* C = base(jb.cSp, jb.cOff);
    const int r0 = gt.bi * 64, c0 = gt.bj * 64;
    const int nk = (jb.K + kGemmKC - 1) / kGemmKC;
    auto load_stage = [&](int ks, int st) {
        double* dst = sm + (size_t)st * kGemmStageDoubles;
        const int k0 = ks * kGemmKC;
#pragma unroll
        for (int it = 0; it < 2 * (kGemmKC / 4) * 2 * 128 / kGemmThreads; ++it) {
            const int c = tid + it * kGemmThreads;
            const int which = c / ((kGemmKC / 4) * 2 * 128);
            const int cc = c - which * ((kGemmKC / 4) * 2 * 128);
            const int grp = cc >> 8, pl = (cc >> 7) & 1, row = (cc & 127) >> 1, half = cc & 1;
            const int k = k0 + 4 * grp;
            const double* src;
            bool ok;
            if (which == 0) {
                ok = (r0 + row < jb.m) && (k < jb.K);
                src = A + kg_off(jb.ldA, jb.rA + r0 + row, jb.kA + k, pl) + half * 2;
            } else {
                ok = (c0 + row < jb.n) && (k < jb.K);
                src = B + kg_off(jb.ldB, jb.rB + c0 + row, jb.kB + k, pl) + half * 2;
            }
            cp_async16(dst + (size_t)c * 2, ok ? src : A, ok ? 16u : 0u);
        }
        cp_async_commit();
    };
    double cre[2][4][2], cim[2][4][2];
#pragma unroll
    for (int a = 0; a < 2; ++a)
#pragma unroll
        for (int b = 0; b < 4; ++b) cre[a][b][0] = cre[a][b][1] = cim[a][b][0] = cim[a][b][1] = 0.0;
    unsigned act = 0;
#pragma unroll
    for (int a = 0; a < 2; ++a)
#pragma unroll
        for (int b = 0; b < 4; ++b) {
            const int rb = r0 + wr * 16 + a * 8, cb = c0 + wc * 32 + b * 8;
            if (rb < jb.m && cb < jb.n && !(jb.lower && jb.cC + cb > jb.rC + rb)) act |= 1u << (a * 4 + b);
        }
    for (int s = 0; s < kGemmStages - 1; ++s) {
        if (s < nk) load_stage(s, s); else cp_async_commit();
    }
    for (int ks = 0; ks < nk; ++ks) {
        cp_async_wait<kGemmStages - 2>();
        __syncthreads();
        if (ks + kGemmStages - 1 < nk) load_stage(ks + kGemmStages - 1, (ks + kGemmStages - 1) % kGemmStages); else cp_async_commit();
        if (!act) continue;
        const double* sA = sm + (size_t)(ks % kGemmStages) * kGemmStageDoubles;
        const double* sB = sA + (kGemmKC / 4) * 2 * 64 * 4;
        const int ngrp = min(kGemmKC / 4, (jb.K - ks * kGemmKC + 3) >> 2);
#pragma unroll
        for (int grp = 0; grp < kGemmKC / 4; ++grp) {
            if (grp >= ngrp) break;
            double are[2], aim[2], nai[2], bre[4], bim[4];
#pragma unroll
            for (int a = 0; a < 2; ++a) {
                are[a] = sA[((grp * 2 + 0) * 64 + wr * 16 + a * 8 + g) * 4 + t];
                aim[a] = sA[((grp * 2 + 1) * 64 + wr * 16 + a * 8 + g) * 4 + t];
                nai[a] = -aim[a];
            }
#pragma unroll
            for (int b = 0; b < 4; ++b) {
                bre[b] = sB[((grp * 2 + 0) * 64 + wc * 32 + b * 8 + g) * 4 + t];
                bim[b] = sB[((grp * 2 + 1) * 64 + wc * 32 + b * 8 + g) * 4 + t];
            }
#pragma unroll
            for (int a = 0; a < 2; ++a)
#pragma unroll
                for (int b = 0; b < 4; ++b) {
                    const int on = (act >> (a * 4 + b)) & 1;
                    dmma884_p(cre[a][b], are[a], bre[b], on);
                    dmma884_p(cim[a][b], are[a], bim[b], on);
                }
#pragma unroll
            for (int a = 0; a < 2; ++a)
#pragma unroll
                for (int b = 0; b < 4; ++b) {
                    const int on = (act >> (a * 4 + b)) & 1;
                    dmma884_p(cre[a][b], nai[a], bim[b], on);
                    dmma884_p(cim[a][b], aim[a], bre[b], on);
                }
        }
    }
    cp_async_wait<0>();
#pragma unroll
    for (int a = 0; a < 2; ++a)
#pragma unroll
        for (int b = 0; b < 4; ++b) {
            const int rb = r0 + wr * 16 + a * 8, cb = c0 + wc * 32 + b * 8;
            if (!((act >> (a * 4 + b)) & 1)) continue;
            double* pr = C + kg_off(jb.ldC, jb.rC + rb + g, jb.cC + cb + 2 * t, 0);
            double* pi = C + kg_off(jb.ldC, jb.rC + rb + g, jb.cC + cb + 2 * t, 1);
            double2 vr = make_double2(jb.alpha * cre[a][b][0], jb.alpha * cre[a][b][1]);
            double2 vi = make_double2(jb.alpha * cim[a][b][0], jb.alpha * cim[a][b][1]);
            if (jb.beta) {
                const double2 orr = *reinterpret_cast<const double2*>(pr), oi = *reinterpret_cast<const double2*>(pi);
                vr.x += orr.x; vr.y += orr.y; vi.x += oi.x; vi.y += oi.y;
            }
            *reinterpret_cast<double2*>(pr) = vr;
            *reinterpret_cast<double2*>(pi) = vi;
        }
}

__global__ void mf_mt_vals_kernel(int N, const MtValSys* __restrict__ sysv, cplx* __restrict__ vals, int64_t valStride) {
    const int e = blockIdx.x * blockDim.x + threadIdx.x, sys = blockIdx.y;
    if (e >= 3 * N) return;
    const MtValSys sv = sysv[sys];
    cplx v;
    if (e < N) v = mk(sv.planes[e], sv.omega * sv.planes[N + e]);
    else v = mk(sv.planes[(size_t)N + e], 0.0);
    vals[(size_t)sys * valStride + e] = v;
}

struct SolveArgs {
    const cplx* B;
    cplx* X;
    int64_t ldb, ldx;
    cplx* v;
    cplx* upd;
    int64_t vStride, uStride;
    int nrhs;
};

__global__ void __launch_bounds__(kSolveMfThreads)
mf_fwd_kernel(Tables tb, SolveArgs sa, const int* __restrict__ list) {
    extern __shared__ __align__(16) unsigned char mf_smem[];
    cplx* w = reinterpret_cast<cplx*>(mf_smem);
    const Front F = tb.fronts[list[blockIdx.x]];
    const int vec = blockIdx.y, sys = vec / sa.nrhs, tid = threadIdx.x, nthr = blockDim.x;
    const int fp = F.sp + F.up;
    const cplx* b = sa.B + (size_t)vec * sa.ldb;
    cplx* v = sa.v + (size_t)vec * sa.vStride;
    cplx* upd = sa.upd + (size_t)vec * sa.uStride;
    for (int i = tid; i < fp; i += nthr) {
        cplx x = mk(0.0, 0.0);
        if (i < F.s) x = b[tb.pos2orig[F.cbp + i]];
        w[i] = x;
    }
    __syncthreads();
    for (int c = 0; c < F.nChild; ++c) {
        const Front& C = tb.fronts[tb.children[F.childPtr + c]];
        const int* rel = tb.rel + C.rowPtr;
        const cplx* uv = upd + C.updOff;
        const int cu = C.u;
        for (int i = tid; i < cu; i += nthr) w[rel[i]] += uv[i];
        __syncthreads();
    }
    const double* fac = tb.fac + (size_t)sys * tb.facStride;
    for (int c = 0; c < F.nChunk; ++c) {
        const Chunk ch = tb.chunks[F.chunkPtr + c];
        const int sc = ch.p1 - ch.p0, mr = fp - ch.p1;
        const double* M = fac + ch.mOff;
        for (int i = tid; i < mr; i += nthr) {
            cplx acc = mk(0.0, 0.0);
            for (int kg = 0; kg < (sc >> 2); ++kg) {
                const double* pr = M + kg_off(mr, i, 4 * kg, 0);
                const double* pi = M + kg_off(mr, i, 4 * kg, 1);
                const double2 r01 = *reinterpret_cast<const double2*>(pr), r23 = *reinterpret_cast<const double2*>(pr + 2);
                const double2 i01 = *reinterpret_cast<const double2*>(pi), i23 = *reinterpret_cast<const double2*>(pi + 2);
                const cplx* wk = w + ch.p0 + 4 * kg;
                cfma(acc, mk(r01.x, i01.x), wk[0]);
                cfma(acc, mk(r01.y, i01.y), wk[1]);
                cfma(acc, mk(r23.x, i23.x), wk[2]);
                cfma(acc, mk(r23.y, i23.y), wk[3]);
            }
            w[ch.p1 + i] -= acc;
        }
        __syncthreads();
    }
    for (int i = tid; i < F.sp; i += nthr) v[F.cbp + i] = w[i];
    for (int i = tid; i < F.up; i += nthr) upd[F.updOff + i] = w[F.sp + i];
}

template <int NV>
__device__ __forceinline__ void mf_bwd_front(const Tables& tb, const Front& F, int sys, cplx* const (&v)[NV], cplx* const (&x)[NV],
                                             cplx* smem) {
    const int tid = threadIdx.x, lane = tid & 31, warp = tid >> 5, nthr = blockDim.x;
    const int fp = F.sp + F.up;
    cplx* xf[NV];
    cplx* tmp[NV];
#pragma unroll
    for (int t = 0; t < NV; ++t) { xf[t] = smem + t * fp; tmp[t] = smem + NV * fp + t * F.sp; }
// ... 266 lines not shown
```

hmcmt2d_b200/csrc/mf_solver.cu:

```cuda
#include "mf_solver.cuh"

#include <algorithm>
#include <cstdio>
#include <cstdlib>

#include "mf_kernels.cuh"

namespace hmcmt {
namespace mf {

namespace {
struct PerDeviceOnceMf {
    bool done[64] = {};
    bool need() {
        int dev = 0;
        if (cudaGetDevice(&dev) != cudaSuccess || dev < 0 || dev >= 64) return true;
        if (done[dev]) return false;
        done[dev] = true;
        return true;
    }
};
constexpr size_t kMaxSmem = 227 * 1024;

template <int NW>
int launch_small(cudaStream_t st, const Tables& tb, const SmallDesc* list, int n, int nsys, size_t smem) {
    static PerDeviceOnceMf once;
    if (once.need()) HMCMT_CUDA_TRY(cudaFuncSetAttribute(mf_small_kernel<NW>, cudaFuncAttributeMaxDynamicSharedMemorySize, (int)kMaxSmem));
    mf_small_kernel<NW><<<dim3(n, nsys), NW * 32, smem, st>>>(tb, list);
    return kOk;
}
int launch_stream(cudaStream_t st, const Tables& tb, const SmallDesc* list, int n, int nsys, size_t smem) {
    static PerDeviceOnceMf once;
    if (once.need()) HMCMT_CUDA_TRY(cudaFuncSetAttribute(mf_small_stream_kernel, cudaFuncAttributeMaxDynamicSharedMemorySize, (int)kMaxSmem));
    mf_small_stream_kernel<<<dim3(n, nsys), 16 * 32, smem, st>>>(tb, list);
    return kOk;
}
}

template <typename Tp>
int Solver::upload(const std::vector<Tp>& h, Tp** d) {
    *d = nullptr;
    const size_t n = std::max<size_t>(h.size(), 1);
    if (cudaMalloc(d, n * sizeof(Tp)) != cudaSuccess) return kErrAlloc;
    owned.push_back(*d);
    bytes += n * sizeof(Tp);
    if (!h.empty() && cudaMemcpy(*d, h.data(), h.size() * sizeof(Tp), cudaMemcpyHostToDevice) != cudaSuccess) return kErrCuda;
    return kOk;
}

int Solver::upload_solve_descs(const std::vector<int>& fr, const SolveDesc** d) {
    std::vector<SolveDesc> v;
    v.reserve(fr.size());
    for (int k : fr) {
        const Front& F = S.fronts[k];
        SolveDesc sd{};
        sd.sp = F.sp; sd.up = F.up; sd.s = F.s; sd.u = F.u; sd.cbp = F.cbp; sd.rowPtr = F.rowPtr; sd.updOff = (int)F.updOff;
        sd.nChild = F.nChild;
        sd.gOff = S.chunks[F.chunkPtr].gOff; sd.mOff = S.chunks[F.chunkPtr].mOff;
        for (int c = 0; c < std::min(F.nChild, kDescChildren); ++c) {
            const Front& C = S.fronts[S.children[F.childPtr + c]];
            sd.cRel[c] = C.rowPtr; sd.cUpd[c] = (int)C.updOff; sd.cU[c] = C.u;
        }
        for (int i = 0; i < std::min(F.u, kDescRows); ++i) sd.rows[i] = S.rows[F.rowPtr + i];
        v.push_back(sd);
    }
    SolveDesc* p = nullptr;
    int rc = upload(v, &p);
    *d = p;
    return rc;
}

Solver* Solver::create(Symbolic&& S, int nsys, int maxRhs, int64_t valCount, int* rc) {
    Solver* s = new Solver();
    s->S = std::move(S);
    int r = s->build(nsys, maxRhs, valCount);
    if (rc) *rc = r;
    if (r != kOk) { delete s; return nullptr; }
    return s;
}

Solver::~Solver() {
    if (d_prof) {
        unsigned long long h[48] = {};
        cudaDeviceSynchronize();
        cudaMemcpy(h, d_prof, sizeof(h), cudaMemcpyDeviceToHost);
        for (int c = 0; c < 4; ++c) {
            const unsigned long long* q = h + 8 * c;
            if (q[6])
                fprintf(stderr, "[hmcmt_b200] mf_small_kernel<%d> cycles per front (%llu fronts, %.2f pivot blocks each): zero %.0f  orig %.0f  "
                        "children %.0f  mirror %.0f  sweep %.0f  output %.0f\n", 2 << c, q[6], (double)q[7] / q[6], (double)q[0] / q[6],
                        (double)q[1] / q[6], (double)q[2] / q[6], (double)q[3] / q[6], (double)q[4] / q[6], (double)q[5] / q[6]);
            const unsigned long long* w = h + 32 + 4 * c;
            if (q[7])
                fprintf(stderr, "[hmcmt_b200]     factorisation of the front, cycles per pivot block: 8x8 inversions %.0f  rest of the pivot-block sweep %.0f  M' = F21 (-G) %.0f  U += M' F21^T %.0f\n",
                        (double)w[0] / q[7], (double)w[1] / q[7], (double)w[2] / q[7], (double)w[3] / q[7]);
        }
    }
    for (void* p : owned) cudaFree(p);
}

int Solver::build(int nsys_, int maxRhs_, int64_t valCount_) {
    nsys = nsys_; maxRhs = std::max(1, maxRhs_); valCount = valCount_;
    int rc;
#define MF_TRY(x) do { rc = (x); if (rc) return rc; } while (0)
    MF_TRY(upload(S.fronts, &d_fronts));
    MF_TRY(upload(S.rows, &d_rows));
    MF_TRY(upload(S.rel, &d_rel));
    MF_TRY(upload(S.children, &d_children));
    MF_TRY(upload(S.orig, &d_orig));
    MF_TRY(upload(S.chunks, &d_chunks));
    MF_TRY(upload(S.pos2orig, &d_pos2orig));
    auto dalloc = [&](void** p, size_t nbytes) {
        *p = nullptr;
        if (nbytes == 0) nbytes = 16;
        if (cudaMalloc(p, nbytes) != cudaSuccess) return (int)kErrAlloc;
        owned.push_back(*p);
        bytes += nbytes;
        return (int)kOk;
    };
    MF_TRY(dalloc((void**)&d_fac, (size_t)nsys * S.factorDoubles * sizeof(double)));
    for (int p = 0; p < 2; ++p) MF_TRY(dalloc((void**)&d_arena[p], (size_t)nsys * S.arenaDoubles[p] * sizeof(double)));
    MF_TRY(dalloc((void**)&d_vals, (size_t)nsys * valCount * sizeof(cplx)));
    MF_TRY(dalloc((void**)&d_v, (size_t)nsys * maxRhs * S.Np * sizeof(cplx)));
    MF_TRY(dalloc((void**)&d_upd, (size_t)nsys * maxRhs * S.updEntries * sizeof(cplx)));
    if (const char* e = std::getenv("HMCMT_MF_PROF"); e && std::atoi(e)) {
        MF_TRY(dalloc((void**)&d_prof, 48 * sizeof(unsigned long long)));
        cudaMemset(d_prof, 0, 48 * sizeof(unsigned long long));
    }

    std::vector<int> invMapsHost;
    const SchedKnobs knobs = SchedKnobs::from_env();
    sched.assign(S.maxDepth + 1, DepthSchedule());
    for (int d = 0; d <= S.maxDepth; ++d) {
        DepthSchedule& D = sched[d];
        const std::vector<int>& sm = S.byDepthSmall[d];
        const std::vector<int>& bg = S.byDepthBig[d];
        int* p = nullptr;
        D.nSmall = (int)sm.size();
        if (D.nSmall) {
            int mx = 0;
            for (int k : sm) mx = std::max(mx, S.fronts[k].fp());
            D.smallStream = mf_small_stream(S, sm);
            D.smallWarps = D.smallStream ? 16 : mf_small_warps(mx, knobs);
            D.smallSmem = 0;
            std::vector<SmallDesc> descs;
            for (int k : sm) {
                const Front& F = S.fronts[k];
                const int nb = F.fp() / 8, npb = F.sp / 8, rt = mf_rel_total(S, k);
                D.smallSmem = std::max(D.smallSmem, D.smallStream ? mf_stream_front_smem_bytes(nb, npb, rt, F.nChild)
                                                    : D.smallWarps >= 8 ? mf_mid_front_smem_bytes(nb, npb, rt, F.nChild)
                                                                        : mf_front_smem_bytes(nb, npb, rt));
                SmallDesc sd{};
                sd.sp = F.sp; sd.up = F.up; sd.s = F.s; sd.nChild = F.nChild; sd.nOrig = F.nOrig; sd.origPtr = F.origPtr;
                sd.par = F.depth & 1; sd.front = k;
                sd.gOff = S.chunks[F.chunkPtr].gOff; sd.mOff = S.chunks[F.chunkPtr].mOff; sd.uOff = F.frontOff;
                for (int c = 0; c < std::min(F.nChild, kDescChildren); ++c) {
                    const Front& C = S.fronts[S.children[F.childPtr + c]];
                    sd.cOff[c] = C.frontOff; sd.cLd[c] = C.ldU(); sd.cFirst[c] = C.offU(); sd.cU[c] = C.u; sd.cRel[c] = C.rowPtr;
                    int piv = 0;
                    while (piv < C.u && S.rel[C.rowPtr + piv] < F.sp) ++piv;
                    if (piv > 255) return kErrArg;
                    sd.cPiv[c] = (unsigned char)piv;
                }
                descs.push_back(sd);
            }
            SmallDesc* pd = nullptr;
            if (D.smallSmem > kMaxSmem) return kErrArg;
            MF_TRY(upload(descs, &pd));
            D.smallDescs = pd;
        }
        D.nBig = (int)bg.size();
        D.bigBytes = (size_t)S.bigDoublesAtDepth[d] * sizeof(double);
        std::vector<int> sw, sc(bg);
        for (int k : sm) (mf_solve_by_warp(S.fronts[k]) ? sw : sc).push_back(k);
        D.nSolveWarp = (int)sw.size();
        D.nSolveCta = (int)sc.size();
        if (D.nSolveWarp) MF_TRY(upload_solve_descs(sw, &D.solveWarpList));
        if (D.nSolveCta) { MF_TRY(upload(sc, &p)); D.solveCtaList = p; }
        {
            int mxc = 0;
            for (int k : sc) mxc = std::max(mxc, S.fronts[k].fp());
            D.solveCtaThreads = mf_solve_cta_threads(mxc, knobs);
        }
        if (!D.nBig) continue;
        MF_TRY(upload(bg, &p));
        D.bigList = p;
        std::vector<int2> op;
        int maxChunk = 0;
        for (int k : bg) {
            const Front& F = S.fronts[k];
            for (int e = 0; e < F.nOrig; ++e) op.push_back(make_int2(k, F.origPtr + e));
            maxChunk = std::max(maxChunk, F.nChunk);
        }
        int2* p2 = nullptr;
        D.nOrigPairs = (int)op.size();
        if (D.nOrigPairs) { MF_TRY(upload(op, &p2)); D.origPairs = p2; }
        {
            std::vector<AsmTile> tiles;
            for (int k : bg) {
                const Front& F = S.fronts[k];
                const int fp = F.fp(), nt = (fp + 63) / 64;
                const int invPtr = (int)invMapsHost.size();
                for (int c = 0; c < F.nChild; ++c) {
                    const Front& C = S.fronts[S.children[F.childPtr + c]];
                    std::vector<int> inv(fp, -1);
                    for (int i = 0; i < C.u; ++i) inv[S.rel[C.rowPtr + i]] = i;
                    invMapsHost.insert(invMapsHost.end(), inv.begin(), inv.end());
                }
                for (int bi = 0; bi < nt; ++bi)
                    for (int bj = 0; bj <= bi; ++bj) tiles.push_back(AsmTile{k, bi, bj, invPtr});
            }
            AsmTile* pt = nullptr;
            MF_TRY(upload(tiles, &pt));
            D.asmTiles = pt;
            D.nAsmTiles = (int)tiles.size();
        }
        for (int c = 0; c < maxChunk; ++c) {
            DepthSchedule::ChunkStep cs;
            std::vector<int> inv;
            std::vector<GemmJob> jobs;
            std::vector<GemmTile> pt, st;
            int maxSc = 0;
            for (int k : bg) {
                const Front& F = S.fronts[k];
                if (F.nChunk <= c) continue;
                const Chunk& ch = S.chunks[F.chunkPtr + c];
                const int sc = ch.p1 - ch.p0, fp = F.fp(), mr = fp - ch.p1, par = F.depth & 1;
                inv.push_back(k);
                maxSc = std::max(maxSc, sc);
                if (mr <= 0) continue;
                GemmJob jp{};
                jp.aOff = F.frontOff; jp.aSp = par; jp.ldA = fp; jp.rA = ch.p1; jp.kA = ch.p0;
                jp.bOff = ch.gOff; jp.bSp = 2; jp.ldB = sc; jp.rB = 0; jp.kB = 0;
                jp.cOff = ch.mOff; jp.cSp = 2; jp.ldC = mr; jp.rC = 0; jp.cC = 0;
                jp.m = mr; jp.n = sc; jp.K = sc; jp.lower = 0; jp.beta = 0; jp.alpha = 1.0;
                const int jpi = (int)jobs.size();
                jobs.push_back(jp);
                for (int bi = 0; bi < (mr + 63) / 64; ++bi)
                    for (int bj = 0; bj < (sc + 63) / 64; ++bj) pt.push_back(GemmTile{jpi, bi, bj});
                GemmJob js{};
                js.aOff = ch.mOff; js.aSp = 2; js.ldA = mr; js.rA = 0; js.kA = 0;
                js.bOff = F.frontOff; js.bSp = par; js.ldB = fp; js.rB = ch.p1; js.kB = ch.p0;
                js.cOff = F.frontOff; js.cSp = par; js.ldC = fp; js.rC = ch.p1; js.cC = ch.p1;
                js.m = mr; js.n = mr; js.K = sc; js.lower = 1; js.beta = 1; js.alpha = -1.0;
                const int jsi = (int)jobs.size();
                jobs.push_back(js);
                for (int bi = 0; bi < (mr + 63) / 64; ++bi)
                    for (int bj = 0; bj <= bi; ++bj) st.push_back(GemmTile{jsi, bi, bj});
            }
            MF_TRY(upload(inv, &p));
            cs.invList = p; cs.nInv = (int)inv.size();
            cs.invSmem = mf_front_smem_bytes(maxSc / 8, maxSc / 8);
            GemmJob* pj = nullptr;
            GemmTile* ptile = nullptr;
            MF_TRY(upload(jobs, &pj));
            cs.jobs = pj;
            MF_TRY(upload(pt, &ptile));
            cs.panelTiles = ptile; cs.nPanelTiles = (int)pt.size();
            MF_TRY(upload(st, &ptile));
            cs.schurTiles = ptile; cs.nSchurTiles = (int)st.size();
            D.chunkSteps.push_back(cs);
        }
    }
    MF_TRY(upload(invMapsHost, &d_invMaps));
    solveSmem = (size_t)(2 * S.maxFp + 16) * sizeof(cplx);
    if (solveSmem > kMaxSmem) return kErrArg;
    {
        int mx = 0;
        for (const Front& F : S.fronts) if (!mf_solve_by_warp(F)) mx = std::max(mx, F.fp() + F.sp);
        pairSmem = (size_t)2 * mx * sizeof(cplx);
    }
#undef MF_TRY
    return kOk;
}

int Solver::set_mt_values(cudaStream_t st, int N, const MtValSys* dSys, int sys0, int n) {
    if (valCount < 3 * (int64_t)N) return kErrArg;
    if (n < 0) n = nsys - sys0;
    if (sys0 < 0 || n < 1 || sys0 + n > nsys) return kErrArg;
    mf_mt_vals_kernel<<<dim3((3 * N + 255) / 256, n), 256, 0, st>>>(N, dSys + sys0, d_vals + (size_t)sys0 * valCount, valCount);
    HMCMT_CUDA_TRY(cudaGetLastError());
    return kOk;
}

int Solver::factor(cudaStream_t st, int* dStatus, int64_t* nLaunches, int sys0, int n) {
    if (n < 0) n = this->nsys - sys0;
    if (sys0 < 0 || n < 1 || sys0 + n > this->nsys) return kErrArg;
    const int nsys = n;
    Tables tb{};
    tb.fronts = d_fronts; tb.rows = d_rows; tb.rel = d_rel; tb.children = d_children; tb.orig = d_orig; tb.chunks = d_chunks;
    tb.pos2orig = d_pos2orig; tb.fac = d_fac + (size_t)sys0 * S.factorDoubles;
    tb.arena[0] = d_arena[0] + (size_t)sys0 * S.arenaDoubles[0]; tb.arena[1] = d_arena[1] + (size_t)sys0 * S.arenaDoubles[1];
    tb.facStride = S.factorDoubles; tb.arenaStride[0] = S.arenaDoubles[0]; tb.arenaStride[1] = S.arenaDoubles[1];
    tb.vals = d_vals + (size_t)sys0 * valCount; tb.valStride = valCount; tb.status = dStatus ? dStatus + sys0 : nullptr; tb.prof = d_prof;
    static PerDeviceOnceMf once;
    if (once.need()) {
        HMCMT_CUDA_TRY(cudaFuncSetAttribute(mf_inv_kernel, cudaFuncAttributeMaxDynamicSharedMemorySize, (int)kMaxSmem));
        HMCMT_CUDA_TRY(cudaFuncSetAttribute(mf_gemm_kernel, cudaFuncAttributeMaxDynamicSharedMemorySize, (int)kGemmSmemBytes));
    }
    int64_t nl = 0;
    for (int d = S.maxDepth; d >= 0; --d) {
        const DepthSchedule& D = sched[d];
        if (D.nSmall) {
            int rc = kOk;
            if (D.smallStream) rc = launch_stream(st, tb, D.smallDescs, D.nSmall, nsys, D.smallSmem);
            else if (D.smallWarps == 1) rc = launch_small<1>(st, tb, D.smallDescs, D.nSmall, nsys, D.smallSmem);
            else if (D.smallWarps == 2) rc = launch_small<2>(st, tb, D.smallDescs, D.nSmall, nsys, D.smallSmem);
            else if (D.smallWarps == 4) rc = launch_small<4>(st, tb, D.smallDescs, D.nSmall, nsys, D.smallSmem);
            else if (D.smallWarps == 8) rc = launch_small<8>(st, tb, D.smallDescs, D.nSmall, nsys, D.smallSmem);
            else rc = launch_small<16>(st, tb, D.smallDescs, D.nSmall, nsys, D.smallSmem);
            if (rc) return rc;
            ++nl;
        }
        if (!D.nBig) continue;
        if (D.nAsmTiles) {
            mf_asm_gather_kernel<<<dim3(D.nAsmTiles, nsys), 256, 0, st>>>(tb, (const AsmTile*)D.asmTiles, d_invMaps);
            ++nl;
        }
        if (D.nOrigPairs) {
            mf_asm_orig_kernel<<<dim3((D.nOrigPairs + 255) / 256, nsys), 256, 0, st>>>(tb, D.origPairs, D.nOrigPairs);
            ++nl;
        }
        for (size_t c = 0; c < D.chunkSteps.size(); ++c) {
            const DepthSchedule::ChunkStep& cs = D.chunkSteps[c];
            if (!cs.nInv) continue;
            mf_inv_kernel<<<dim3(cs.nInv, nsys), kInvWarps * 32, cs.invSmem, st>>>(tb, cs.invList, (int)c);
            ++nl;
            if (cs.nPanelTiles) {
                mf_gemm_kernel<<<dim3(cs.nPanelTiles, nsys), kGemmThreads, kGemmSmemBytes, st>>>(
                    tb, (const GemmJob*)cs.jobs, (const GemmTile*)cs.panelTiles);
                ++nl;
            }
            if (cs.nSchurTiles) {
                mf_gemm_kernel<<<dim3(cs.nSchurTiles, nsys), kGemmThreads, kGemmSmemBytes, st>>>(
                    tb, (const GemmJob*)cs.jobs, (const GemmTile*)cs.schurTiles);
                ++nl;
            }
        }
    }
    HMCMT_CUDA_TRY(cudaGetLastError());
    if (nLaunches) *nLaunches += nl;
    return kOk;
}

int Solver::add_rhs_pattern(const std::vector<unsigned char>& nz) {
    if ((int)nz.size() != S.N) return kErrArg;
    std::vector<char> active(S.K, 0);
    for (int k = 0; k < S.K; ++k) {
        const Front& F = S.fronts[k];
        for (int i = 0; i < F.s && !active[k]; ++i) {
            const int o = S.pos2orig[F.cbp + i];
            if (o >= 0 && nz[o]) active[k] = 1;
        }
        if (active[k] && F.parent >= 0) active[F.parent] = 1;
    }
    PatternLists L;
    int rc;
#define MF_TRY(x) do { rc = (x); if (rc) return rc; } while (0)
    for (int d = 0; d <= S.maxDepth; ++d) {
        std::vector<int> sw, sc, pw, pc;
        for (int k : S.byDepthBig[d]) if (active[k]) sc.push_back(k);
        for (int k : S.byDepthSmall[d]) if (active[k]) (mf_solve_by_warp(S.fronts[k]) ? sw : sc).push_back(k);
        for (int k : S.byDepthBig[d]) if (!active[k]) pc.push_back(k);
        for (int k : S.byDepthSmall[d]) if (!active[k]) (mf_solve_by_warp(S.fronts[k]) ? pw : pc).push_back(k);
        L.nPairWarpBoth.push_back((int)pw.size());
        L.nPairCtaBoth.push_back((int)pc.size());
        pw.insert(pw.end(), sw.begin(), sw.end());
        pc.insert(pc.end(), sc.begin(), sc.end());
        const SolveDesc* pd = nullptr;
        if (!sw.empty()) MF_TRY(upload_solve_descs(sw, &pd));
        L.warpList.push_back(pd);
        L.nWarp.push_back((int)sw.size());
        int* p = nullptr;
        if (!sc.empty()) MF_TRY(upload(sc, &p));
        L.ctaList.push_back(sc.empty() ? nullptr : p);
        L.nCta.push_back((int)sc.size());
        L.nFronts += (int)(sw.size() + sc.size());
        pd = nullptr;
        if (!pw.empty()) MF_TRY(upload_solve_descs(pw, &pd));
        L.pairWarpList.push_back(pd);
        p = nullptr;
        if (!pc.empty()) MF_TRY(upload(pc, &p));
        L.pairCtaList.push_back(p);
    }
#undef MF_TRY
    patterns.push_back(std::move(L));
    return (int)patterns.size();
}

int Solver::fwd_fronts(int pattern) const {
    return pattern >= 1 && pattern <= (int)patterns.size() ? patterns[pattern - 1].nFronts : S.K;
}

Tables Solver::tables(int sys0) const {
    Tables tb{};
    tb.fronts = d_fronts; tb.rows = d_rows; tb.rel = d_rel; tb.children = d_children; tb.orig = d_orig; tb.chunks = d_chunks;
    tb.pos2orig = d_pos2orig; tb.fac = d_fac + (size_t)sys0 * S.factorDoubles;
    tb.arena[0] = d_arena[0] + (size_t)sys0 * S.arenaDoubles[0]; tb.arena[1] = d_arena[1] + (size_t)sys0 * S.arenaDoubles[1];
    tb.facStride = S.factorDoubles; tb.arenaStride[0] = S.arenaDoubles[0]; tb.arenaStride[1] = S.arenaDoubles[1];
    tb.vals = d_vals; tb.valStride = valCount; tb.status = nullptr; tb.prof = nullptr;
    return tb;
}

SolveArgs Solver::solve_args(const cplx* B, int64_t ldb, cplx* X, int64_t ldx, int sys0, int nrhs, int slot) const {
    const size_t vec0 = (size_t)sys0 * nrhs, ws0 = (size_t)sys0 * maxRhs + slot;
    const int64_t per = nrhs == 1 ? maxRhs : 1;
    return SolveArgs{B ? B + vec0 * ldb : nullptr, X ? X + vec0 * ldx : nullptr, ldb, ldx, d_v + ws0 * S.Np, d_upd + ws0 * S.updEntries,
                     per * S.Np, per * S.updEntries, nrhs};
}

int Solver::set_solve_attributes() {
    static PerDeviceOnceMf once;
    if (once.need()) {
        HMCMT_CUDA_TRY(cudaFuncSetAttribute(mf_fwd_kernel, cudaFuncAttributeMaxDynamicSharedMemorySize, (int)kMaxSmem));
        HMCMT_CUDA_TRY(cudaFuncSetAttribute(mf_bwd_kernel, cudaFuncAttributeMaxDynamicSharedMemorySize, (int)kMaxSmem));
        HMCMT_CUDA_TRY(cudaFuncSetAttribute(mf_bwd_pair_kernel, cudaFuncAttributeMaxDynamicSharedMemorySize, (int)kMaxSmem));
    }
    return kOk;
}

int Solver::clear_ws(cudaStream_t st, const SolveArgs& sa, int nvec) {
    const struct { cplx* p; int64_t len, stride; } ws[2] = {{sa.v, (int64_t)S.Np, sa.vStride}, {sa.upd, S.updEntries, sa.uStride}};
    for (const auto& w : ws) {
        if (w.stride == w.len) HMCMT_CUDA_TRY(cudaMemsetAsync(w.p, 0, (size_t)nvec * w.len * sizeof(cplx), st));
        else HMCMT_CUDA_TRY(cudaMemset2DAsync(w.p, (size_t)w.stride * sizeof(cplx), 0, (size_t)w.len * sizeof(cplx), nvec, st));
    }
    return kOk;
}

int Solver::fwd_sweep(cudaStream_t st, const Tables& tb, const SolveArgs& sa, int nvec, int pattern, int64_t& nl) {
    const PatternLists* P = pattern ? &patterns[pattern - 1] : nullptr;
    for (int d = S.maxDepth; d >= 0; --d) {
        const DepthSchedule& D = sched[d];
        const int nW = P ? P->nWarp[d] : D.nSolveWarp, nC = P ? P->nCta[d] : D.nSolveCta;
        const SolveDesc* wl = P ? P->warpList[d] : D.solveWarpList;
        const int* cl = P ? P->ctaList[d] : D.solveCtaList;
        if (nW) {
            mf_fwd_warp_kernel<<<dim3((nW + kSolveWarpsPerCta - 1) / kSolveWarpsPerCta, nvec), kSolveWarpsPerCta * 32, 0, st>>>(tb, sa, wl, nW);
            ++nl;
        }
        if (nC) {
            mf_fwd_kernel<<<dim3(nC, nvec), D.solveCtaThreads, solveSmem, st>>>(tb, sa, cl);
            ++nl;
        }
    }
    return kOk;
}

int Solver::solve(cudaStream_t st, int nrhs, const cplx* B, int64_t ldb, cplx* X, int64_t ldx, int64_t* nLaunches, int sys0, int n,
                  int pattern) {
    if (nrhs < 1 || nrhs > maxRhs || pattern < 0 || pattern > (int)patterns.size()) return kErrArg;
    if (n < 0) n = this->nsys - sys0;
    if (sys0 < 0 || n < 1 || sys0 + n > this->nsys) return kErrArg;
    int rc = set_solve_attributes();
    if (rc) return rc;
    const Tables tb = tables(sys0);
    const SolveArgs sa = solve_args(B, ldb, X, ldx, sys0, nrhs, 0);
    const int nvec = n * nrhs;
    int64_t nl = 0;
    if (pattern && (rc = clear_ws(st, sa, nvec))) return rc;
    fwd_sweep(st, tb, sa, nvec, pattern, nl);
    for (int d = 0; d <= S.maxDepth; ++d) {
        const DepthSchedule& D = sched[d];
        if (D.nSolveWarp) {
            mf_bwd_warp_kernel<<<dim3((D.nSolveWarp + kSolveWarpsPerCta - 1) / kSolveWarpsPerCta, nvec), kSolveWarpsPerCta * 32, 0, st>>>(
                tb, sa, D.solveWarpList, D.nSolveWarp);
            ++nl;
        }
        if (D.nSolveCta) {
            mf_bwd_kernel<<<dim3(D.nSolveCta, nvec), D.solveCtaThreads, solveSmem, st>>>(tb, sa, D.solveCtaList);
            ++nl;
        }
    }
    HMCMT_CUDA_TRY(cudaGetLastError());
    if (nLaunches) *nLaunches += nl;
    return kOk;
}

int Solver::forward_slot(cudaStream_t st, int slot, const cplx* B, int64_t ldb, int64_t* nLaunches, int sys0, int n, int pattern) {
    if (slot < 0 || slot >= maxRhs || pattern < 0 || pattern > (int)patterns.size()) return kErrArg;
    if (n < 0) n = this->nsys - sys0;
    if (sys0 < 0 || n < 1 || sys0 + n > this->nsys) return kErrArg;
    int rc = set_solve_attributes();
    if (rc) return rc;
    const SolveArgs sa = solve_args(B, ldb, nullptr, 0, sys0, 1, slot);
    int64_t nl = 0;
    if (pattern && (rc = clear_ws(st, sa, n))) return rc;
    fwd_sweep(st, tables(sys0), sa, n, pattern, nl);
    HMCMT_CUDA_TRY(cudaGetLastError());
    if (nLaunches) *nLaunches += nl;
    return kOk;
}

int Solver::backward_slot(cudaStream_t st, int slot, cplx* X, int64_t ldx, int64_t* nLaunches, int sys0, int n, int pattern) {
    if (slot < 0 || slot >= maxRhs || pattern < 1 || pattern > (int)patterns.size()) return kErrArg;
    if (n < 0) n = this->nsys - sys0;
    if (sys0 < 0 || n < 1 || sys0 + n > this->nsys) return kErrArg;
    int rc = set_solve_attributes();
    if (rc) return rc;
    const Tables tb = tables(sys0);
    const SolveArgs sa = solve_args(nullptr, 0, X, ldx, sys0, 1, slot);
    const PatternLists& P = patterns[pattern - 1];
    int64_t nl = 0;
    for (int d = 0; d <= S.maxDepth; ++d) {
        if (const int nW = P.nWarp[d]) {
            mf_bwd_warp_kernel<<<dim3((nW + kSolveWarpsPerCta - 1) / kSolveWarpsPerCta, n), kSolveWarpsPerCta * 32, 0, st>>>(
                tb, sa, P.warpList[d], nW);
            ++nl;
        }
        if (const int nC = P.nCta[d]) {
            mf_bwd_kernel<<<dim3(nC, n), sched[d].solveCtaThreads, solveSmem, st>>>(tb, sa, P.ctaList[d]);
            ++nl;
        }
    }
    HMCMT_CUDA_TRY(cudaGetLastError());
    if (nLaunches) *nLaunches += nl;
    return kOk;
}

int Solver::backward_pair(cudaStream_t st, cplx* Xa, cplx* Xb, int64_t ldx, int64_t* nLaunches, int sys0, int n, int done) {
    if (maxRhs < 2 || done < 1 || done > (int)patterns.size() || pairSmem > kMaxSmem) return kErrArg;
    if (n < 0) n = this->nsys - sys0;
    if (sys0 < 0 || n < 1 || sys0 + n > this->nsys) return kErrArg;
    int rc = set_solve_attributes();
    if (rc) return rc;
    const Tables tb = tables(sys0);
    const SolveArgs sa = solve_args(nullptr, 0, Xa, ldx, sys0, 1, 0), sb = solve_args(nullptr, 0, Xb, ldx, sys0, 1, 1);
    const PatternLists& P = patterns[done - 1];
    int64_t nl = 0;
    for (int d = 0; d <= S.maxDepth; ++d) {
        const DepthSchedule& D = sched[d];
        if (D.nSolveWarp) {
            mf_bwd_pair_warp_kernel<<<dim3((D.nSolveWarp + kSolveWarpsPerCta - 1) / kSolveWarpsPerCta, n), kSolveWarpsPerCta * 32, 0, st>>>(
                tb, sa, sb, P.pairWarpList[d], D.nSolveWarp, P.nPairWarpBoth[d]);
            ++nl;
        }
        if (D.nSolveCta) {
            mf_bwd_pair_kernel<<<dim3(D.nSolveCta, n), D.solveCtaThreads, pairSmem, st>>>(tb, sa, sb, P.pairCtaList[d], P.nPairCtaBoth[d]);
            ++nl;
        }
    }
    HMCMT_CUDA_TRY(cudaGetLastError());
    if (nLaunches) *nLaunches += nl;
    return kOk;
}

}
}
```

hmcmt2d_b200/csrc/mf_solver.cuh:

```cuda
#pragma once
#include <cstdint>
#include <vector>

#include "common.cuh"
#include "mf_symbolic.h"

namespace hmcmt {
namespace mf {

struct MtValSys {
    const double* planes;
    double omega;
};

constexpr int kDescChildren = kSmallChildren;
struct SmallDesc {
    int sp, up, s, nChild;
    int nOrig, origPtr, par, front;
    int64_t gOff, mOff, uOff;
    int64_t cOff[kDescChildren];
    int cLd[kDescChildren], cFirst[kDescChildren], cU[kDescChildren], cRel[kDescChildren];
    unsigned char cPiv[kDescChildren];
};

constexpr int kDescRows = 40;
struct SolveDesc {
    int sp, up, s, u;
    int cbp, rowPtr, updOff, nChild;
    int64_t gOff, mOff;
    int cRel[kDescChildren], cUpd[kDescChildren], cU[kDescChildren];
    int rows[kDescRows];
};

struct DepthSchedule {
    int nSmall = 0, smallWarps = 4;
    bool smallStream = false;
    size_t smallSmem = 0;
    const SmallDesc* smallDescs = nullptr;
    int nBig = 0;
    const int* bigList = nullptr;
    int nOrigPairs = 0;
    const int2* origPairs = nullptr;
    const void* asmTiles = nullptr;
    int nAsmTiles = 0;
    struct ChunkStep {
        const int* invList = nullptr;
        int nInv = 0;
        size_t invSmem = 0;
        const void* jobs = nullptr;
        const void* panelTiles = nullptr;
        int nPanelTiles = 0;
        const void* schurTiles = nullptr;
        int nSchurTiles = 0;
    };
    std::vector<ChunkStep> chunkSteps;
    size_t bigBytes = 0;
    const SolveDesc* solveWarpList = nullptr;
    const int* solveCtaList = nullptr;
    int nSolveWarp = 0, nSolveCta = 0;
    int solveCtaThreads = 256;
};

struct Tables;
struct SolveArgs;

class Solver {
  public:
    static Solver* create(Symbolic&& S, int nsys, int maxRhs, int64_t valCount, int* rc);
    ~Solver();
    cplx* vals() { return d_vals; }
    int64_t val_stride() const { return valCount; }
    const Symbolic& symbolic() const { return S; }
    int set_mt_values(cudaStream_t st, int N, const MtValSys* dSys, int sys0 = 0, int n = -1);
    int factor(cudaStream_t st, int* dStatus, int64_t* nLaunches = nullptr, int sys0 = 0, int n = -1);
    int solve(cudaStream_t st, int nrhs, const cplx* B, int64_t ldb, cplx* X, int64_t ldx, int64_t* nLaunches = nullptr, int sys0 = 0,
              int n = -1, int pattern = 0);
    int forward_slot(cudaStream_t st, int slot, const cplx* B, int64_t ldb, int64_t* nLaunches, int sys0, int n, int pattern);
    int backward_slot(cudaStream_t st, int slot, cplx* X, int64_t ldx, int64_t* nLaunches, int sys0, int n, int pattern);
    int backward_pair(cudaStream_t st, cplx* Xa, cplx* Xb, int64_t ldx, int64_t* nLaunches, int sys0, int n, int done);
    int add_rhs_pattern(const std::vector<unsigned char>& nz);
    int fwd_fronts(int pattern) const;
    size_t device_bytes() const { return bytes; }
    double factor_flops() const { return S.flops; }
    int64_t factor_doubles() const { return S.factorDoubles; }

  private:
    Solver() = default;
    int build(int nsys, int maxRhs, int64_t valCount);
    template <typename Tp>
    int upload(const std::vector<Tp>& h, Tp** d);
    int upload_solve_descs(const std::vector<int>& fronts, const SolveDesc** d);
    Tables tables(int sys0) const;
    SolveArgs solve_args(const cplx* B, int64_t ldb, cplx* X, int64_t ldx, int sys0, int nrhs, int slot) const;
    int set_solve_attributes();
    int clear_ws(cudaStream_t st, const SolveArgs& sa, int nvec);
    int fwd_sweep(cudaStream_t st, const Tables& tb, const SolveArgs& sa, int nvec, int pattern, int64_t& nl);
    Symbolic S;
    int nsys = 0, maxRhs = 1;
    int64_t valCount = 0;
    size_t bytes = 0;
    std::vector<void*> owned;
    std::vector<DepthSchedule> sched;
    struct PatternLists {
        std::vector<const SolveDesc*> warpList;
        std::vector<const int*> ctaList;
        std::vector<int> nWarp, nCta;
        int nFronts = 0;
        std::vector<const SolveDesc*> pairWarpList;
        std::vector<const int*> pairCtaList;
        std::vector<int> nPairWarpBoth, nPairCtaBoth;
    };
    std::vector<PatternLists> patterns;
    Front* d_fronts = nullptr;
    int *d_rows = nullptr, *d_rel = nullptr, *d_children = nullptr, *d_pos2orig = nullptr;
    OrigEntry* d_orig = nullptr;
    Chunk* d_chunks = nullptr;
    double* d_fac = nullptr;
    double* d_arena[2] = {nullptr, nullptr};
    cplx *d_vals = nullptr, *d_v = nullptr, *d_upd = nullptr;
    int* d_invMaps = nullptr;
    size_t solveSmem = 0;
    size_t pairSmem = 0;
    unsigned long long* d_prof = nullptr;
};

}
}
```

hmcmt2d_b200/csrc/mf_symbolic.h:

```cpp
#pragma once
#include <algorithm>
#include <cstdint>
#include <cstdlib>
#include <functional>
#include <numeric>
#include <queue>
#include <vector>

namespace hmcmt {
namespace mf {

constexpr int kTile = 8;
constexpr int kChunkMax = 96;

inline int pad8(int x) { return (x + 7) & ~7; }

constexpr size_t kFrontDescBytes = 160;
constexpr int kSmallChildren = 4;
inline size_t mf_front_smem_bytes(int nb, int npb, int relTotal = 0) {
    const size_t nT = (size_t)nb * (nb + 1) / 2, nS = 2 * (size_t)npb, nM = (size_t)(nb - npb) * npb;
    return kFrontDescBytes + (nT + (nS > nM ? nS : nM) + 1) * 128 * sizeof(double) + 16 + (((size_t)relTotal + 1) & ~(size_t)1) * 2 * sizeof(int);
}
inline size_t mf_mid_front_smem_bytes(int nb, int npb, int relTotal, int nChild) {
    const size_t nub = (size_t)(nb - npb), nT = (size_t)npb * (npb + 1) / 2 + nub * npb, nS = 2 * (size_t)npb, nM = nub * npb;
    return kFrontDescBytes + (nT + (nS > nM ? nS : nM) + 1) * 128 * sizeof(double) + 16 + (((size_t)relTotal + 1) & ~(size_t)1) * 2 * sizeof(int) +
           (size_t)nChild * nub * 8 * sizeof(int);
}
inline size_t mf_stream_front_smem_bytes(int nb, int npb, int relTotal, int nChild) {
    const size_t nub = (size_t)(nb - npb), nT = (size_t)npb * (npb + 1) / 2 + nub * npb, nS = 2 * (size_t)npb;
    return kFrontDescBytes + (nT + nS + 1) * 128 * sizeof(double) + 16 + (((size_t)relTotal + 1) & ~(size_t)1) * 2 * sizeof(int) +
           (size_t)nChild * nub * 8 * sizeof(int);
}
constexpr size_t kFrontSmemMax = 227 * 1024;
constexpr int kFullFrontMaxFp = 144;
inline bool mf_front_needs_stream(int nb, int npb, int relTotal, int nChild) {
    return mf_mid_front_smem_bytes(nb, npb, relTotal, nChild) > kFrontSmemMax;
}
inline size_t mf_large_front_smem_bytes(int nb, int npb, int relTotal, int nChild) {
    return mf_front_needs_stream(nb, npb, relTotal, nChild) ? mf_stream_front_smem_bytes(nb, npb, relTotal, nChild)
                                                            : mf_mid_front_smem_bytes(nb, npb, relTotal, nChild);
}

struct Entry {
    int row, col, src;
};

struct OrigEntry {
    int lrow, lcol, src;
};

struct Chunk {
    int p0, p1;
    int64_t gOff, mOff;
};

struct Front {
    int s, sp, u, up;
    int cbp;
    int rowPtr;
    int parent, depth;
    int childPtr, nChild;
    int origPtr, nOrig;
    int chunkPtr, nChunk;
    int isBig;
    int64_t frontOff;
    int64_t updOff;
    int fp() const { return sp + up; }
    int ldU() const { return isBig ? sp + up : up; }
    int offU() const { return isBig ? sp : 0; }
};

struct Symbolic {
    int N = 0, Np = 0, K = 0, maxDepth = 0;
    std::vector<int> pos2orig;
    std::vector<int> orig2pos;
    std::vector<Front> fronts;
    std::vector<int> rows;
    std::vector<int> rel;
    std::vector<int> children;
    std::vector<OrigEntry> orig;
    std::vector<Chunk> chunks;
    std::vector<std::vector<int>> byDepthSmall, byDepthBig;
    std::vector<int64_t> bigDoublesAtDepth;
    int64_t factorDoubles = 0;
    int64_t arenaDoubles[2] = {0, 0};
    int64_t updEntries = 0;
    int maxFpSmall = 0, maxFpBig = 0, maxFp = 0;
    double flops = 0.0;
};


inline void mf_order_grid(int nl, int nf, int leaf, std::vector<std::vector<int>>& out, int cross = 0, int push = 0) {
    std::function<int(int, int, int, int, bool&)> rec = [&](int l0, int l1, int f0, int f1, bool& isLeaf) -> int {
        const int nL = l1 - l0, nF = f1 - f0;
        isLeaf = false;
        if (nL <= 0 || nF <= 0) return -1;
        if (nL * nF <= leaf) {
            std::vector<int> v;
            v.reserve((size_t)nL * nF);
            for (int l = l0; l < l1; ++l)
                for (int f = f0; f < f1; ++f) v.push_back(l * nf + f);
            out.push_back(std::move(v));
            isLeaf = true;
            return (int)out.size() - 1;
        }
        std::vector<int> sep;
        bool la = false, lb = false, lc = false, ld = false;
        if (std::max(nL, nF) <= cross && std::min(nL, nF) >= 3) {
            const int ml = (l0 + l1) / 2, mf = (f0 + f1) / 2;
            rec(l0, ml, f0, mf, la);
            rec(l0, ml, mf + 1, f1, lb);
            rec(ml + 1, l1, f0, mf, lc);
            rec(ml + 1, l1, mf + 1, f1, ld);
            for (int f = f0; f < f1; ++f) sep.push_back(ml * nf + f);
            for (int l = l0; l < l1; ++l)
                if (l != ml) sep.push_back(l * nf + mf);
        } else {
            const bool byLine = nL >= nF;
            const int mid = byLine ? (l0 + l1) / 2 : (f0 + f1) / 2;
            const int a = byLine ? rec(l0, mid, f0, f1, la) : rec(l0, l1, f0, mid, la);
            const int b = byLine ? rec(mid + 1, l1, f0, f1, lb) : rec(l0, l1, mid + 1, f1, lb);
            if (byLine) for (int f = f0; f < f1; ++f) sep.push_back(mid * nf + f);
            else for (int l = l0; l < l1; ++l) sep.push_back(l * nf + mid);
            const int cap = pad8((int)sep.size());
            auto absorb = [&](int ci, bool childIsLeaf, int adj) {
                if (ci < 0 || !childIsLeaf || push <= 0) return;
                std::vector<int>& v = out[ci];
                const int s = (int)v.size(), e = s % 8;
                if (s <= 8 || e == 0 || e > push || (int)sep.size() + e > cap) return;
                int moved = 0;
                for (size_t i = 0; i < v.size() && moved < e;) {
                    const int q = v[i], l = q / nf, f = q - l * nf;
                    if ((byLine ? l : f) == adj) { sep.push_back(q); v.erase(v.begin() + i); ++moved; }
                    else ++i;
                }
            };
            absorb(a, la, mid - 1);
            absorb(b, lb, mid + 1);
        }
        out.push_back(std::move(sep));
        return (int)out.size() - 1;
    };
    bool dummy = false;
    rec(0, nl, 0, nf, dummy);
}

inline void mf_order_graph(int n, const std::vector<int>& adjPtr, const std::vector<int>& adj, int leaf,
                           std::vector<std::vector<int>>& out) {
    std::vector<int> region(n, 0);
    std::vector<int> level(n, -1), queue;
    queue.reserve(n);
    int nextRegion = 1;
    struct Item {
        std::vector<int> nodes;
        std::vector<int> sep;
        int stage;
    };
    std::vector<Item> stack;
    {
        Item it;
        it.nodes.resize(n);
        std::iota(it.nodes.begin(), it.nodes.end(), 0);
        it.stage = 0;
        stack.push_back(std::move(it));
    }
    auto bfs = [&](int start, int rid, const std::vector<int>& nodes, int& nLevels) {
        for (int v : nodes) level[v] = -1;
        queue.clear();
        queue.push_back(start);
        level[start] = 0;
        size_t head = 0;
        while (head < queue.size()) {
            const int v = queue[head++];
            for (int k = adjPtr[v]; k < adjPtr[v + 1]; ++k) {
                const int w = adj[k];
                if (region[w] == rid && level[w] < 0) {
                    level[w] = level[v] + 1;
                    queue.push_back(w);
                }
            }
        }
        nLevels = level[queue.back()] + 1;
    };
    while (!stack.empty()) {
        if (stack.back().stage == 1) {
            if (!stack.back().sep.empty()) out.push_back(std::move(stack.back().sep));
            stack.pop_back();
            continue;
        }
        Item it = std::move(stack.back());
        stack.pop_back();
        std::vector<int>& nodes = it.nodes;
        if (nodes.empty()) continue;
        if ((int)nodes.size() <= leaf) {
            out.push_back(std::move(nodes));
            continue;
        }
        const int rid = nextRegion++;
        for (int v : nodes) region[v] = rid;
        int nLevels = 0;
        bfs(nodes[0], rid, nodes, nLevels);
        if (queue.size() < nodes.size()) {
            Item a, b;
            a.stage = b.stage = 0;
            for (int v : nodes) (level[v] >= 0 ? a.nodes : b.nodes).push_back(v);
            Item marker;
            marker.stage = 1;
            stack.push_back(std::move(marker));
            stack.push_back(std::move(b));
            stack.push_back(std::move(a));
            continue;
        }
        for (int rep = 0; rep < 2; ++rep) {
            const int far = queue.back();
            bfs(far, rid, nodes, nLevels);
        }
        if (nLevels < 3) {
            out.push_back(std::move(nodes));
            continue;
        }
        std::vector<int> cnt(nLevels, 0);
        for (int v : nodes) ++cnt[level[v]];
        const double tot = (double)nodes.size();
        int best = -1;
        double acc = 0.0;
        for (int L = 0; L < nLevels; ++L) {
            const double before = acc;
            acc += cnt[L];
            if (L == 0 || L == nLevels - 1) continue;
            if (before >= 0.35 * tot && before <= 0.65 * tot)
                if (best < 0 || cnt[L] < cnt[best]) best = L;
        }
        if (best < 0) {
            acc = 0.0;
            for (int L = 0; L < nLevels; ++L) {
                acc += cnt[L];
                if (acc >= 0.5 * tot) { best = std::min(std::max(L, 1), nLevels - 2); break; }
            }
        }
        Item a, b, marker;
        a.stage = b.stage = 0;
        marker.stage = 1;
        for (int v : nodes) {
            if (level[v] < best) a.nodes.push_back(v);
            else if (level[v] > best) b.nodes.push_back(v);
            else marker.sep.push_back(v);
        }
        for (int v : marker.sep) region[v] = -1;
        stack.push_back(std::move(marker));
        stack.push_back(std::move(b));
        stack.push_back(std::move(a));
    }
}

inline bool mf_symbolic(int N, const std::vector<std::vector<int>>& snodes, const std::vector<Entry>& entries, int fSmall,
                        Symbolic& S) {
    S = Symbolic();
    S.N = N;
    const int K = (int)snodes.size();
    S.K = K;
    S.fronts.resize(K);
    S.orig2pos.assign(N, -1);
    std::vector<int> cbp(K + 1, 0);
    for (int k = 0; k < K; ++k) cbp[k + 1] = cbp[k] + pad8((int)snodes[k].size());
    S.Np = cbp[K];
    S.pos2orig.assign(S.Np, -1);
    std::vector<int> snOf(S.Np, -1);
    for (int k = 0; k < K; ++k) {
        for (int i = 0; i < (int)snodes[k].size(); ++i) {
            const int o = snodes[k][i];
            if (o < 0 || o >= N || S.orig2pos[o] >= 0) return false;
            S.orig2pos[o] = cbp[k] + i;
            S.pos2orig[cbp[k] + i] = o;
        }
        for (int p = cbp[k]; p < cbp[k + 1]; ++p) snOf[p] = k;
    }
    for (int o = 0; o < N; ++o) if (S.orig2pos[o] < 0) return false;
    std::vector<int> aPtr(S.Np + 1, 0);
    for (const Entry& e : entries) {
        const int a = S.orig2pos[e.row], b = S.orig2pos[e.col];
        if (a != b) ++aPtr[std::min(a, b) + 1];
    }
    for (int p = 0; p < S.Np; ++p) aPtr[p + 1] += aPtr[p];
    std::vector<int> aIdx(aPtr[S.Np]), fill(aPtr.begin(), aPtr.end() - 1);
    for (const Entry& e : entries) {
        const int a = S.orig2pos[e.row], b = S.orig2pos[e.col];
        if (a != b) aIdx[fill[std::min(a, b)]++] = std::max(a, b);
    }
    std::vector<std::vector<int>> pending(K);
    std::vector<int> mark(S.Np, -1);
    S.rows.clear();
    std::vector<std::vector<int>> kids(K);
    for (int k = 0; k < K; ++k) {
        Front& F = S.fronts[k];
        F.s = (int)snodes[k].size();
        F.sp = pad8(F.s);
        F.cbp = cbp[k];
        const int c1 = cbp[k + 1];
        std::vector<int> st;
        for (int p = cbp[k]; p < cbp[k] + F.s; ++p)
            for (int q = aPtr[p]; q < aPtr[p + 1]; ++q) {
                const int r = aIdx[q];
                if (r >= c1 && mark[r] != k) { mark[r] = k; st.push_back(r); }
            }
        for (int r : pending[k])
            if (r >= c1 && mark[r] != k) { mark[r] = k; st.push_back(r); }
        std::vector<int>().swap(pending[k]);
        std::sort(st.begin(), st.end());
        F.u = (int)st.size();
        F.up = pad8(F.u);
        F.rowPtr = (int)S.rows.size();
        F.parent = -1;
        if (F.u) {
            F.parent = snOf[st[0]];
            kids[F.parent].push_back(k);
            std::vector<int>& pp = pending[F.parent];
            pp.insert(pp.end(), st.begin(), st.end());
        }
        S.rows.insert(S.rows.end(), st.begin(), st.end());
        for (int i = F.u; i < F.up; ++i) S.rows.push_back(-1);
    }
    S.maxDepth = 0;
    for (int k = K - 1; k >= 0; --k) {
        Front& F = S.fronts[k];
        F.depth = F.parent < 0 ? 0 : S.fronts[F.parent].depth + 1;
        S.maxDepth = std::max(S.maxDepth, F.depth);
        F.childPtr = (int)S.children.size();
        F.nChild = (int)kids[k].size();
        S.children.insert(S.children.end(), kids[k].begin(), kids[k].end());
    }
    S.rel.assign(S.rows.size(), -1);
    for (int k = 0; k < K; ++k) {
        const Front& F = S.fronts[k];
        if (F.parent < 0) continue;
        const Front& P = S.fronts[F.parent];
        const int* prow = S.rows.data() + P.rowPtr;
        for (int i = 0; i < F.u; ++i) {
            const int r = S.rows[F.rowPtr + i];
            int loc;
            if (r < P.cbp + P.sp) loc = r - P.cbp;
            else {
                const int* it = std::lower_bound(prow, prow + P.u, r);
                if (it == prow + P.u || *it != r) return false;
                loc = P.sp + (int)(it - prow);
            }
            S.rel[F.rowPtr + i] = loc;
        }
    }
    {
        std::vector<int> cnt(K + 1, 0);
        for (const Entry& e : entries) {
            const int lo = std::min(S.orig2pos[e.row], S.orig2pos[e.col]);
            ++cnt[snOf[lo] + 1];
        }
        for (int k = 0; k < K; ++k) cnt[k + 1] += S.fronts[k].sp - S.fronts[k].s;
        for (int k = 0; k < K; ++k) cnt[k + 1] += cnt[k];
        S.orig.resize(cnt[K]);
        std::vector<int> at(cnt.begin(), cnt.end() - 1);
        for (int k = 0; k < K; ++k) {
            S.fronts[k].origPtr = cnt[k];
            S.fronts[k].nOrig = cnt[k + 1] - cnt[k];
        }
        for (const Entry& e : entries) {
            const int a = S.orig2pos[e.row], b = S.orig2pos[e.col];
            const int lo = std::min(a, b), hi = std::max(a, b);
            const int k = snOf[lo];
            const Front& F = S.fronts[k];
            int lrow;
            if (hi < F.cbp + F.sp) lrow = hi - F.cbp;
            else {
                const int* r0 = S.rows.data() + F.rowPtr;
                const int* it = std::lower_bound(r0, r0 + F.u, hi);
                if (it == r0 + F.u || *it != hi) return false;
                lrow = F.sp + (int)(it - r0);
            }
            S.orig[at[k]++] = OrigEntry{lrow, lo - F.cbp, e.src};
        }
        for (int k = 0; k < K; ++k)
            for (int i = S.fronts[k].s; i < S.fronts[k].sp; ++i) S.orig[at[k]++] = OrigEntry{i, i, -1};
    }
    S.byDepthSmall.assign(S.maxDepth + 1, {});
    S.byDepthBig.assign(S.maxDepth + 1, {});
    int64_t fac = 0, arena[2] = {0, 0}, upd = 0;
    std::vector<int64_t> arenaAtDepth(S.maxDepth + 1, 0);
    for (int k = 0; k < K; ++k) {
        Front& F = S.fronts[k];
        const int fp = F.fp();
        int relTotal = 0;
        for (int c = 0; c < F.nChild; ++c) relTotal += S.fronts[S.children[F.childPtr + c]].u;
        const size_t smem = fp <= kFullFrontMaxFp ? mf_front_smem_bytes(fp / 8, F.sp / 8, relTotal)
                                                  : mf_large_front_smem_bytes(fp / 8, F.sp / 8, relTotal, F.nChild);
        F.isBig = (fp > fSmall || F.nChild > kSmallChildren || smem > kFrontSmemMax) ? 1 : 0;
        S.maxFp = std::max(S.maxFp, fp);
        (F.isBig ? S.maxFpBig : S.maxFpSmall) = std::max(F.isBig ? S.maxFpBig : S.maxFpSmall, fp);
        (F.isBig ? S.byDepthBig : S.byDepthSmall)[F.depth].push_back(k);
        F.updOff = upd;
        upd += F.up;
        F.chunkPtr = (int)S.chunks.size();
        const int cmax = F.isBig ? kChunkMax : F.sp;
        for (int p0 = 0; p0 < F.sp; p0 += cmax) {
            const int p1 = std::min(p0 + cmax, F.sp), sc = p1 - p0;
            Chunk c{p0, p1, fac, 0};
            fac += 2 * (int64_t)sc * sc;
            c.mOff = fac;
            fac += 2 * (int64_t)(fp - p1) * sc;
            S.chunks.push_back(c);
            const double a = sc, b = fp - p1;
            S.flops += 8.0 * (0.5 * a * a * a + a * a * b + 0.5 * a * b * b);
        }
        F.nChunk = (int)S.chunks.size() - F.chunkPtr;
    }
    S.bigDoublesAtDepth.assign(S.maxDepth + 1, 0);
    for (int d = 0; d <= S.maxDepth; ++d) {
        for (int k : S.byDepthBig[d]) {
            Front& F = S.fronts[k];
            F.frontOff = arenaAtDepth[d];
            arenaAtDepth[d] += 2 * (int64_t)F.fp() * F.fp();
        }
        S.bigDoublesAtDepth[d] = arenaAtDepth[d];
        for (int k : S.byDepthSmall[d]) {
            Front& F = S.fronts[k];
            F.frontOff = arenaAtDepth[d];
            arenaAtDepth[d] += 2 * (int64_t)F.up * F.up;
        }
    }
    for (int d = 0; d <= S.maxDepth; ++d) arena[d & 1] = std::max(arena[d & 1], arenaAtDepth[d]);
    S.factorDoubles = fac;
    S.arenaDoubles[0] = arena[0];
    S.arenaDoubles[1] = arena[1];
    S.updEntries = upd;
    return true;
}

inline int mf_rel_total(const Symbolic& S, int k) {
    const Front& F = S.fronts[k];
    int n = 0;
    for (int c = 0; c < F.nChild; ++c) n += S.fronts[S.children[F.childPtr + c]].u;
    return n;
}

constexpr int kSolveWarpMaxFp = 64;
constexpr int kSolveMfThreads = 256;

struct SchedKnobs {
    int fp1 = 40, fp2 = 40, fp4 = 64, fp8 = 96;
    int solveThreads = 0;
    static SchedKnobs from_env() {
        auto knob = [](const char* name, int dflt) { const char* e = std::getenv(name); return e ? std::atoi(e) : dflt; };
        SchedKnobs k;
        k.fp1 = knob("HMCMT_MF_FP1", k.fp1); k.fp2 = knob("HMCMT_MF_FP2", k.fp2);
        k.fp4 = knob("HMCMT_MF_FP4", k.fp4); k.fp8 = knob("HMCMT_MF_FP8", k.fp8);
        k.solveThreads = knob("HMCMT_MF_SOLVE_THREADS", 0);
        return k;
    }
};

inline int mf_small_warps(int maxFp, const SchedKnobs& k) {
    const int w = maxFp <= k.fp1 ? 1 : (maxFp <= k.fp2 ? 2 : (maxFp <= k.fp4 ? 4 : (maxFp <= k.fp8 ? 8 : 16)));
    return maxFp > kFullFrontMaxFp && w < 8 ? 8 : w;
}
inline bool mf_small_stream(const Symbolic& S, const std::vector<int>& launch) {
    for (int k : launch) {
        const Front& F = S.fronts[k];
        if (F.fp() > kFullFrontMaxFp && mf_front_needs_stream(F.fp() / 8, F.sp / 8, mf_rel_total(S, k), F.nChild)) return true;
    }
    return false;
}
inline bool mf_solve_by_warp(const Front& F) { return !F.isBig && F.fp() <= kSolveWarpMaxFp && F.nChild <= kSmallChildren; }
inline int mf_solve_cta_threads(int maxFp, const SchedKnobs& k) {
    return k.solveThreads ? k.solveThreads : (maxFp <= 144 ? 128 : kSolveMfThreads);
}

inline bool mf_analyse_csc(int64_t n, const int64_t* rowval, const int64_t* colptr, int leaf, int fSmall, Symbolic& S) {
    std::vector<Entry> ent;
    ent.reserve((size_t)(colptr[n] - 1) / 2 + n);
    std::vector<int> ptr(n + 1, 0);
    for (int64_t j = 0; j < n; ++j)
        for (int64_t k = colptr[j] - 1; k < colptr[j + 1] - 1; ++k) {
            const int64_t i = rowval[k] - 1;
            if (i < 0 || i >= n) return false;
            if (i < j) continue;
            ent.push_back(Entry{(int)i, (int)j, (int)k});
            if (i != j) { ++ptr[i + 1]; ++ptr[j + 1]; }
        }
    for (int64_t i = 0; i < n; ++i) ptr[i + 1] += ptr[i];
    std::vector<int> adj(ptr[n]), at(ptr.begin(), ptr.end() - 1);
    for (const Entry& e : ent)
        if (e.row != e.col) { adj[at[e.row]++] = e.col; adj[at[e.col]++] = e.row; }
    std::vector<std::vector<int>> sn;
    mf_order_graph((int)n, ptr, adj, leaf, sn);
    return mf_symbolic((int)n, sn, ent, fSmall, S);
}

inline void mf_grid_entries(int nl, int nf, std::vector<Entry>& e) {
    const int N = nl * nf;
    e.clear();
    e.reserve((size_t)3 * N);
    for (int l = 0; l < nl; ++l)
        for (int f = 0; f < nf; ++f) {
            const int q = l * nf + f;
            e.push_back(Entry{q, q, q});
            if (f > 0) e.push_back(Entry{q, q - 1, N + q});
            if (l > 0) e.push_back(Entry{q, q - nf, 2 * N + q});
        }
}

}
}
```

hmcmt2d_b200/csrc/mumps_shim.cu:

```cuda
#include <algorithm>
#include <cmath>
#include <cstdlib>
#include <cstring>
#include <mutex>
#include <unordered_map>
#include <vector>

#include "../../include/hmcmt_b200.h"
#include "band_factor.cuh"
#include "band_solve.cuh"
#include "mf_solver.cuh"

namespace hmcmt {
int round_T(int b);
int launch_factor(cudaStream_t st, int T, const BandSys* sys, int nsys, const BandDom& dom, const SolveJob* fwdJobs, int* nLaunches);
int launch_solve(cudaStream_t st, int T, const SolveJob* jobs, int njobs, const BandDom& dom);
int mf_leaf_size();
int mf_small_front();
}
using namespace hmcmt;

namespace {

constexpr int kShimMaxRhs = 16;

struct Factor {
    int n = 0, b = 0, T = 0, S = 0;
    bool isReal = false;
    double* panels = nullptr;
    cplx* ainvz = nullptr;
    mf::Solver* mfs = nullptr;
    const void* pattern = nullptr;
    int64_t epoch = 0;
};
std::mutex g_mu;
std::unordered_map<int64_t, Factor*> g_factors;
int64_t g_next = 1;

std::unordered_map<const void*, std::vector<mf::Solver*>> g_pool;
constexpr size_t kPoolMax = 256;
int64_t g_epoch = 0;

void free_factor(Factor* f) {
    if (!f) return;
    if (f->panels) cudaFree(f->panels);
    if (f->ainvz) cudaFree(f->ainvz);
    if (f->mfs) {
        std::lock_guard<std::mutex> lk(g_mu);
        std::vector<mf::Solver*>& v = g_pool[f->pattern];
        if (f->pattern && f->epoch == g_epoch && v.size() < kPoolMax) v.push_back(f->mfs);
        else delete f->mfs;
    }
    delete f;
}

struct PatternKey {
    int64_t n, nnz;
    uint64_t h;
    bool operator==(const PatternKey& o) const { return n == o.n && nnz == o.nnz && h == o.h; }
};
struct PatternHash {
    size_t operator()(const PatternKey& k) const { return (size_t)(k.h ^ (uint64_t)k.n * 0x9e3779b97f4a7c15ull); }
};
std::unordered_map<PatternKey, mf::Symbolic*, PatternHash> g_symbolic;

uint64_t fnv(const int64_t* p, int64_t n, uint64_t h) {
    for (int64_t i = 0; i < n; ++i) { h ^= (uint64_t)p[i]; h *= 0x100000001b3ull; }
    return h;
}

const mf::Symbolic* symbolic_for(int64_t n, const int64_t* rowval, const int64_t* colptr) {
    const int64_t nnz = colptr[n] - 1;
    const mf::SchedKnobs sk = mf::SchedKnobs::from_env();
    const int64_t knobs[7] = {mf_leaf_size(), mf_small_front(), sk.fp1, sk.fp2, sk.fp4, sk.fp8, sk.solveThreads};
    PatternKey key{n, nnz, fnv(knobs, 7, fnv(rowval, nnz, fnv(colptr, n + 1, 0xcbf29ce484222325ull)))};
    {
        std::lock_guard<std::mutex> lk(g_mu);
        auto it = g_symbolic.find(key);
        if (it != g_symbolic.end()) return it->second;
    }
    mf::Symbolic* S = new mf::Symbolic();
    if (!mf::mf_analyse_csc(n, rowval, colptr, mf_leaf_size(), mf_small_front(), *S)) { delete S; return nullptr; }
    std::lock_guard<std::mutex> lk(g_mu);
    if (g_symbolic.size() >= 8) {
        for (auto& kv : g_pool)
            for (mf::Solver* sv : kv.second) delete sv;
        g_pool.clear();
        ++g_epoch;
        for (auto& kv : g_symbolic) delete kv.second;
        g_symbolic.clear();
    }
    g_symbolic[key] = S;
    return S;
}

int64_t factor_mf(int64_t n, const double* nzval, const int64_t* rowval, const int64_t* colptr, bool isReal, int64_t* status) {
    auto fail = [&](int code) { if (status) *status = code; return (int64_t)0; };
    const mf::Symbolic* S0 = symbolic_for(n, rowval, colptr);
    if (!S0) return fail(kErrArg);
    const int64_t nnz = colptr[n] - 1;
    int rc = kOk;
    mf::Solver* sv = nullptr;
    int64_t epoch = 0;
    {
        std::lock_guard<std::mutex> lk(g_mu);
        epoch = g_epoch;
        auto it = g_pool.find(S0);
        if (it != g_pool.end() && !it->second.empty()) { sv = it->second.back(); it->second.pop_back(); }
    }
    if (!sv) {
        mf::Symbolic copy = *S0;
        sv = mf::Solver::create(std::move(copy), 1, kShimMaxRhs, nnz, &rc);
    }
    if (!sv) return fail(rc);
    std::vector<cplx> hv((size_t)nnz);
    for (int64_t k = 0; k < nnz; ++k) hv[k] = isReal ? mk(nzval[k], 0.0) : mk(nzval[2 * k], nzval[2 * k + 1]);
    int* dstatus = nullptr;
    if (cudaMalloc(&dstatus, sizeof(int)) != cudaSuccess) { delete sv; return fail(kErrAlloc); }
    cudaMemset(dstatus, 0, sizeof(int));
    cudaMemcpy(sv->vals(), hv.data(), hv.size() * sizeof(cplx), cudaMemcpyHostToDevice);
    rc = sv->factor(nullptr, dstatus);
    int hst = 0;
    if (rc == kOk && cudaDeviceSynchronize() != cudaSuccess) rc = kErrCuda;
    if (rc == kOk) cudaMemcpy(&hst, dstatus, sizeof(int), cudaMemcpyDeviceToHost);
    cudaFree(dstatus);
    if (rc != kOk || hst != 0) { delete sv; return fail(rc != kOk ? rc : hst); }
    Factor* f = new Factor();
    f->n = (int)n; f->isReal = isReal; f->mfs = sv; f->pattern = S0; f->epoch = epoch;
    std::lock_guard<std::mutex> lk(g_mu);
    int64_t h = g_next++;
    g_factors[h] = f;
    return h;
}

int64_t factor_common(int64_t n, int64_t sym, const double* nzval, const int64_t* rowval, const int64_t* colptr, bool isReal,
                      int64_t* status) {
    auto fail = [&](int code) { if (status) *status = code; return (int64_t)0; };
    if (status) *status = 0;
    int ndev = 0;
    if (cudaGetDeviceCount(&ndev) != cudaSuccess || ndev == 0) {
        fprintf(stderr, "[hmcmt_b200] no CUDA device: this library has no CPU fallback\n");
        return fail(kErrNoDevice);
    }
    if (n < 1 || !nzval || !rowval || !colptr) return fail(kErrArg);
    if (sym != 1 && sym != 2) {
        fprintf(stderr, "[hmcmt_b200] factor_mumps: only symmetric matrices (sym=1,2) are supported\n");
        return fail(kErrArg);
    }
    int64_t b = 0;
    for (int64_t j = 0; j < n; ++j)
        for (int64_t k = colptr[j] - 1; k < colptr[j + 1] - 1; ++k) b = std::max<int64_t>(b, std::llabs(rowval[k] - 1 - j));
    if (b < 1) b = 1;
    int T = round_T((int)b);
    {
        const char* env = std::getenv("HMCMT_SHIM_SOLVER");
        const bool forceMf = env && !std::strcmp(env, "mf"), forceBand = env && !std::strcmp(env, "band");
        if ((T == 0 && !forceBand) || forceMf) return factor_mf(n, nzval, rowval, colptr, isReal, status);
        if (T == 0) return fail(kErrArg);
    }
    std::vector<cplx> band((size_t)n * (b + 1), mk(0.0, 0.0));
    for (int64_t j = 0; j < n; ++j)
        for (int64_t k = colptr[j] - 1; k < colptr[j + 1] - 1; ++k) {
            int64_t i = rowval[k] - 1;
            if (i < j) continue;
            cplx v = isReal ? mk(nzval[k], 0.0) : mk(nzval[2 * k], nzval[2 * k + 1]);
            band[(size_t)i * (b + 1) + (i - j)] = v;
        }
    Factor* f = new Factor();
    f->n = (int)n; f->b = (int)b; f->T = T; f->S = (int)((n + TS - 1) / TS); f->isReal = isReal;
    cplx* dband = nullptr;
    BandSys* dsys = nullptr;
    int* dstatus = nullptr;
    auto cleanup = [&]() { if (dband) cudaFree(dband); if (dsys) cudaFree(dsys); if (dstatus) cudaFree(dstatus); };
    if (cudaMalloc(&dband, band.size() * sizeof(cplx)) != cudaSuccess ||
        cudaMalloc(&f->panels, (size_t)f->S * panel_doubles(T) * sizeof(double)) != cudaSuccess ||
        cudaMalloc(&f->ainvz, (size_t)f->S * AZ * sizeof(cplx)) != cudaSuccess || cudaMalloc(&dsys, sizeof(BandSys)) != cudaSuccess ||
        cudaMalloc(&dstatus, sizeof(int)) != cudaSuccess) {
        cleanup(); free_factor(f);
        return fail(kErrAlloc);
    }
    cudaMemcpy(dband, band.data(), band.size() * sizeof(cplx), cudaMemcpyHostToDevice);
    cudaMemset(dstatus, 0, sizeof(int));
    BandSys s{};
    s.band = dband; s.omega = 0.0; s.rhs = nullptr; s.panels[0] = f->panels; s.panels[1] = nullptr; s.ainvz[0] = f->ainvz; s.ainvz[1] = nullptr; s.wexp = nullptr; s.x = nullptr; s.status = dstatus;
    cudaMemcpy(dsys, &s, sizeof(BandSys), cudaMemcpyHostToDevice);
    BandDom dom{(int)n, (int)b, (int)b, 0, 0, 0};
    int rc = launch_factor(nullptr, T, dsys, 1, dom, nullptr, nullptr);
    int hst = 0;
    if (rc == kOk && cudaDeviceSynchronize() != cudaSuccess) rc = kErrCuda;
    if (rc == kOk) cudaMemcpy(&hst, dstatus, sizeof(int), cudaMemcpyDeviceToHost);
    cleanup();
    if (rc != kOk || hst != 0) { free_factor(f); return fail(rc != kOk ? rc : hst); }
    std::lock_guard<std::mutex> lk(g_mu);
    int64_t h = g_next++;
    g_factors[h] = f;
    return h;
}

Factor* lookup(int64_t h) {
    std::lock_guard<std::mutex> lk(g_mu);
    auto it = g_factors.find(h);
    return it == g_factors.end() ? nullptr : it->second;
}

int64_t solve_common(int64_t h, int64_t nrhs, const double* rhs, double* x, bool isRealIO) {
    Factor* f = lookup(h);
    if (!f || nrhs < 1 || !rhs || !x) return kErrArg;
    const size_t n = f->n;
    std::vector<cplx> hb(n * nrhs);
    for (size_t i = 0; i < n * (size_t)nrhs; ++i) hb[i] = isRealIO ? mk(rhs[i], 0.0) : mk(rhs[2 * i], rhs[2 * i + 1]);
    if (f->mfs) {
        cplx* db = nullptr;
        if (cudaMalloc(&db, hb.size() * sizeof(cplx)) != cudaSuccess) return kErrAlloc;
        cudaMemcpy(db, hb.data(), hb.size() * sizeof(cplx), cudaMemcpyHostToDevice);
        int rc = kOk;
        for (int64_t r0 = 0; r0 < nrhs && rc == kOk; r0 += kShimMaxRhs) {
            const int nr = (int)std::min<int64_t>(kShimMaxRhs, nrhs - r0);
            rc = f->mfs->solve(nullptr, nr, db + r0 * n, (int64_t)n, db + r0 * n, (int64_t)n);
        }
        if (rc == kOk && cudaDeviceSynchronize() != cudaSuccess) rc = kErrCuda;
        if (rc == kOk) {
            cudaMemcpy(hb.data(), db, hb.size() * sizeof(cplx), cudaMemcpyDeviceToHost);
            for (size_t i = 0; i < hb.size(); ++i) {
                if (isRealIO) x[i] = hb[i].x;
                else { x[2 * i] = hb[i].x; x[2 * i + 1] = hb[i].y; }
            }
        }
        cudaFree(db);
        return rc;
    }
    cplx *dx = nullptr, *dz = nullptr;
    SolveJob* djobs = nullptr;
    auto cleanup = [&]() { if (dx) cudaFree(dx); if (dz) cudaFree(dz); if (djobs) cudaFree(djobs); };
    if (cudaMalloc(&dx, hb.size() * sizeof(cplx)) != cudaSuccess || cudaMalloc(&dz, (size_t)nrhs * f->S * 8 * sizeof(cplx)) != cudaSuccess ||
        cudaMalloc(&djobs, sizeof(SolveJob) * nrhs) != cudaSuccess) {
        cleanup();
        return kErrAlloc;
    }
    cudaMemcpy(dx, hb.data(), hb.size() * sizeof(cplx), cudaMemcpyHostToDevice);
    std::vector<SolveJob> jobs(nrhs);
    for (int64_t r = 0; r < nrhs; ++r) {
        jobs[r].panels[0] = f->panels; jobs[r].panels[1] = nullptr; jobs[r].ainvz[0] = f->ainvz; jobs[r].ainvz[1] = nullptr;
        jobs[r].rhs = dx + r * n; jobs[r].x = dx + r * n; jobs[r].zbuf[0] = dz + (size_t)r * f->S * 8; jobs[r].zbuf[1] = nullptr;
        jobs[r].wexp = nullptr;
    }
    cudaMemcpy(djobs, jobs.data(), sizeof(SolveJob) * nrhs, cudaMemcpyHostToDevice);
    BandDom dom{f->n, f->b, f->b, 0, 0, 0};
    int rc = launch_solve(nullptr, f->T, djobs, (int)nrhs, dom);
    if (rc == kOk && cudaDeviceSynchronize() != cudaSuccess) rc = kErrCuda;
    if (rc == kOk) {
        cudaMemcpy(hb.data(), dx, hb.size() * sizeof(cplx), cudaMemcpyDeviceToHost);
        for (size_t i = 0; i < hb.size(); ++i) {
            if (isRealIO) x[i] = hb[i].x;
            else { x[2 * i] = hb[i].x; x[2 * i + 1] = hb[i].y; }
        }
    }
    cleanup();
    return rc;
}

void solve_sparse_common(int64_t h, int64_t nrhs, const double* nzval, const int64_t* rowval, const int64_t* colptr, double* x,
                         bool isRealIO) {
    Factor* f = lookup(h);
    if (!f || nrhs < 1) return;
    const size_t n = f->n, w = isRealIO ? 1 : 2;
    std::vector<double> dense(n * nrhs * w, 0.0);
    for (int64_t j = 0; j < nrhs; ++j)
        for (int64_t k = colptr[j] - 1; k < colptr[j + 1] - 1; ++k) {
            size_t i = (size_t)(rowval[k] - 1) + (size_t)j * n;
            if (isRealIO) dense[i] = nzval[k];
            else { dense[2 * i] = nzval[2 * k]; dense[2 * i + 1] = nzval[2 * k + 1]; }
        }
    solve_common(h, nrhs, dense.data(), x, isRealIO);
}

int64_t destroy_common(int64_t h) {
    Factor* f = nullptr;
    {
        std::lock_guard<std::mutex> lk(g_mu);
        auto it = g_factors.find(h);
        if (it == g_factors.end()) return kErrArg;
        f = it->second;
        g_factors.erase(it);
    }
    free_factor(f);
    return kOk;
}

}

extern "C" {

int64_t factor_mumps_cmplx_(const int64_t* n, const int64_t* sym, const int64_t* ooc, const double* nzval, const int64_t* rowval,
                            const int64_t* colptr, int64_t* status) {
    (void)ooc;
    if (!n || !sym) { if (status) *status = kErrArg; return 0; }
    return factor_common(*n, *sym, nzval, rowval, colptr, false, status);
}
int64_t factor_mumps_(const int64_t* n, const int64_t* sym, const int64_t* ooc, const double* nzval, const int64_t* rowval,
                      const int64_t* colptr, int64_t* status) {
    (void)ooc;
    if (!n || !sym) { if (status) *status = kErrArg; return 0; }
    return factor_common(*n, *sym, nzval, rowval, colptr, true, status);
}
int64_t solve_mumps_cmplx_(const int64_t* handle, const int64_t* nrhs, const double* rhs, double* x, const int64_t* transpose) {
    (void)transpose;
    if (!handle || !nrhs) return kErrArg;
    return solve_common(*handle, *nrhs, rhs, x, false);
}
int64_t solve_mumps_(const int64_t* handle, const int64_t* nrhs, const double* rhs, double* x, const int64_t* transpose) {
    (void)transpose;
    if (!handle || !nrhs) return kErrArg;
    return solve_common(*handle, *nrhs, rhs, x, true);
}
void solve_mumps_sparse_rhs_(const int64_t* handle, const int64_t* nzrhs, const int64_t* nrhs, const double* nzval,
                             const int64_t* rowval, const int64_t* colptr, double* x, const int64_t* transpose) {
    (void)nzrhs; (void)transpose;
    if (!handle || !nrhs) return;
    solve_sparse_common(*handle, *nrhs, nzval, rowval, colptr, x, true);
}
void solve_mumps_cmplx_sparse_rhs_(const int64_t* handle, const int64_t* nzrhs, const int64_t* nrhs, const double* nzval,
                                   const int64_t* rowval, const int64_t* colptr, double* x, const int64_t* transpose) {
    (void)nzrhs; (void)transpose;
    if (!handle || !nrhs) return;
    solve_sparse_common(*handle, *nrhs, nzval, rowval, colptr, x, false);
}
int64_t hmcmt_debug_get_factor(int64_t handle, double* panels, double* ainv, int64_t* dims) {
    Factor* f = lookup(handle);
    if (!f || f->mfs) return kErrArg;
    if (dims) { dims[0] = f->n; dims[1] = f->b; dims[2] = f->T; dims[3] = f->S; }
    if (panels) cudaMemcpy(panels, f->panels, (size_t)f->S * panel_doubles(f->T) * sizeof(double), cudaMemcpyDeviceToHost);
    if (ainv) cudaMemcpy(ainv, f->ainvz, (size_t)f->S * AZ * sizeof(cplx), cudaMemcpyDeviceToHost);
    return kOk;
}
int64_t destroy_mumps_(const int64_t* handle) { return handle ? destroy_common(*handle) : kErrArg; }
int64_t destroy_mumps_cmplx_(const int64_t* handle) { return handle ? destroy_common(*handle) : kErrArg; }

}
```

hmcmt2d_b200/lib.py:

```python
from __future__ import annotations

import ctypes as C
import os

import numpy as np

_HERE = os.path.dirname(os.path.abspath(__file__))
LIB_PATH = os.path.join(_HERE, "libhmcmt_b200.so")

_i64p = C.POINTER(C.c_int64)
_i32p = C.POINTER(C.c_int32)
_f64p = C.POINTER(C.c_double)


class HmcmtError(RuntimeError):

    MESSAGES = {-10: "numerically singular matrix", -13: "memory allocation error", -40: "matrix is not positive definite",
                -3: "bad argument", -21: "a parameter bound could not be met within 500 reflections", -98: "no CUDA device (there is no CPU fallback)", -99: "CUDA error"}

    def __init__(self, code: int, where: str):
        self.code = code
        super().__init__(f"hmcmt_b200: {where} failed with status {code}: {self.MESSAGES.get(code, 'error')}")


class Problem(C.Structure):
    _fields_ = [
        ("ny", C.c_int32), ("nz", C.c_int32), ("yLen", _f64p), ("zLen", _f64p), ("origin", C.c_double * 2),
        ("nFreq", C.c_int32), ("freqs", _f64p), ("nRx", C.c_int32), ("rxLoc", _f64p),
        ("nComp", C.c_int32), ("compMode", _i32p), ("nData", C.c_int32),
        ("freqID", _i64p), ("rxID", _i64p), ("dtID", _i64p),
        ("obsData", _f64p), ("dataErr", _f64p), ("nAC", C.c_int32), ("activeIdx", _i32p), ("bgModel", _f64p),
        ("wmRowPtr", _i32p), ("wmColIdx", _i32p), ("wmVal", _f64p),
        ("regParam", C.c_double), ("sigBounds", C.c_double * 2), ("nChains", C.c_int32), ("device", C.c_int32),
    ]


_lib = None


def load() -> C.CDLL:
    global _lib
    if _lib is not None:
        return _lib
    if not os.path.exists(LIB_PATH):
        raise ImportError(f"{LIB_PATH} is missing: build it with `python -m hmcmt2d_b200.build` "
                          "(nvcc, sm_100a). hmcmt2d_b200 has no CPU fallback.")
    lib = C.CDLL(LIB_PATH)
    vp = C.c_void_p
    lib.hmcmt_version.restype = C.c_char_p
    lib.hmcmt_plan_create.argtypes = [C.POINTER(Problem), C.POINTER(vp)]
    lib.hmcmt_plan_create_rho_phase.argtypes = [C.POINTER(Problem), C.POINTER(vp)]
    lib.hmcmt_destroy.argtypes = [vp]
    lib.hmcmt_destroy.restype = None
    lib.hmcmt_plan_info.argtypes = [vp, C.c_int]
    lib.hmcmt_plan_info.restype = C.c_int64
    lib.hmcmt_forward.argtypes = [vp, _f64p, _f64p, _f64p, _f64p]
    lib.hmcmt_forward_sigma.argtypes = [vp, _f64p, _f64p, _f64p, _f64p]
    lib.hmcmt_jtvec.argtypes = [vp, _f64p, _f64p]
    lib.hmcmt_jacobian.argtypes = [vp, _f64p]
    lib.hmcmt_jvec.argtypes = [vp, _f64p, _f64p]
    lib.hmcmt_gn_hessvec.argtypes = [vp, _f64p, C.c_int32, _f64p]
    lib.hmcmt_gauss_newton.argtypes = [vp, _f64p, C.c_int32, C.c_int32, C.c_double, C.c_int32, C.c_double, C.c_double, _f64p,
                                       _f64p, _i32p]
    lib.hmcmt_status.argtypes = [vp]
    lib.hmcmt_set_mass_matrix.argtypes = [vp, C.c_int32]
    lib.hmcmt_set_response_kind.argtypes = [vp, C.c_int32]
    lib.hmcmt_get_responses.argtypes = [vp, _f64p]
    lib.hmcmt_forward_gradient.argtypes = [vp, _f64p, _f64p, _f64p, _f64p]
    lib.hmcmt_forward_gradient_total.argtypes = [vp, _f64p, _f64p, _f64p, _f64p]
    lib.hmcmt_set_state.argtypes = [vp, _f64p, _f64p, _f64p]
    lib.hmcmt_get_state.argtypes = [vp, _f64p, _f64p]
    lib.hmcmt_leapfrog_trajectory.argtypes = [vp, C.c_double, _i32p, _f64p, _f64p]
    lib.hmcmt_leapfrog_steps_device.argtypes = [vp, C.c_double, C.c_int32]
    lib.hmcmt_step_partial.argtypes = [vp, C.c_double]
    lib.hmcmt_exchange_buffer.argtypes = [vp, C.POINTER(vp), _i64p]
    lib.hmcmt_step_finish.argtypes = [vp, C.c_double]
    lib.hmcmt_sync.argtypes = [vp]
    lib.hmcmt_nccl_unique_id.argtypes = [C.c_char_p]
    lib.hmcmt_nccl_init.argtypes = [vp, C.c_char_p, C.c_int32, C.c_int32]
    lib.hmcmt_leapfrog_steps_sharded.argtypes = [vp, C.c_double, C.c_int32]
    lib.hmcmt_timer_start.argtypes = [vp]
    lib.hmcmt_timer_stop.argtypes = [vp, C.POINTER(C.c_float)]
    lib.hmcmt_kernel_time.argtypes = [vp, C.c_int, C.POINTER(C.c_float), _i64p]
    lib.hmcmt_kernel_time_split.argtypes = [vp, C.POINTER(C.c_float), C.POINTER(C.c_float)]
    lib.hmcmt_run_chain.argtypes = [vp, C.c_double, C.c_int32, C.c_double, _f64p, _f64p, _i32p, _f64p, _f64p, C.c_int32,
                                    _f64p, _f64p, _i32p, _f64p]
    lib.hmcmt_export_system.argtypes = [vp, C.c_int32, C.c_int32, C.c_int32, _i64p, _i64p, _f64p, _f64p, _f64p]
    for name in ("factor_mumps_cmplx_", "factor_mumps_"):
        fn = getattr(lib, name)
        fn.argtypes = [_i64p, _i64p, _i64p, _f64p, _i64p, _i64p, _i64p]
        fn.restype = C.c_int64
    for name in ("solve_mumps_cmplx_", "solve_mumps_"):
        fn = getattr(lib, name)
        fn.argtypes = [_i64p, _i64p, _f64p, _f64p, _i64p]
        fn.restype = C.c_int64
    for name in ("solve_mumps_sparse_rhs_", "solve_mumps_cmplx_sparse_rhs_"):
        fn = getattr(lib, name)
        fn.argtypes = [_i64p, _i64p, _i64p, _f64p, _i64p, _i64p, _f64p, _i64p]
        fn.restype = None
    for name in ("destroy_mumps_", "destroy_mumps_cmplx_"):
        fn = getattr(lib, name)
        fn.argtypes = [_i64p]
        fn.restype = C.c_int64
    _lib = lib
    return lib


EXPORTED_SYMBOLS = [
    "factor_mumps_cmplx_", "factor_mumps_", "solve_mumps_cmplx_", "solve_mumps_", "solve_mumps_sparse_rhs_",
    "solve_mumps_cmplx_sparse_rhs_", "destroy_mumps_", "destroy_mumps_cmplx_",
    "hmcmt_plan_create", "hmcmt_plan_create_rho_phase", "hmcmt_destroy", "hmcmt_plan_info", "hmcmt_forward", "hmcmt_forward_sigma", "hmcmt_jtvec",
    "hmcmt_forward_gradient", "hmcmt_forward_gradient_total", "hmcmt_jacobian", "hmcmt_jvec", "hmcmt_gn_hessvec", "hmcmt_gauss_newton", "hmcmt_status", "hmcmt_set_mass_matrix", "hmcmt_set_response_kind", "hmcmt_get_responses",
    "hmcmt_set_state", "hmcmt_get_state", "hmcmt_leapfrog_trajectory", "hmcmt_leapfrog_steps_device", "hmcmt_sync",
    "hmcmt_step_partial", "hmcmt_exchange_buffer", "hmcmt_step_finish", "hmcmt_nccl_unique_id", "hmcmt_nccl_init",
    "hmcmt_leapfrog_steps_sharded",
    "hmcmt_timer_start", "hmcmt_timer_stop", "hmcmt_kernel_time", "hmcmt_kernel_time_split", "hmcmt_run_chain", "hmcmt_export_system", "hmcmt_version",
]


def f64(a):
    return a.ctypes.data_as(_f64p)


def i64(a):
    return a.ctypes.data_as(_i64p)


def i32(a):
    return a.ctypes.data_as(_i32p)


def check(code: int, where: str):
    if code < 0:
        raise HmcmtError(int(code), where)
    return code



class MUMPSfactorization:

    def __init__(self, ptr, n, is_complex):
        self.ptr, self.n, self.is_complex = ptr, n, is_complex


def factorMUMPS(A, sym: int = 0, ooc: int = 0) -> MUMPSfactorization:
    lib = load()
    A = A.tocsc()
    A.sort_indices()
    if A.shape[0] != A.shape[1]:
        raise ValueError("factorMUMPS: Matrix must be square!")
    n = C.c_int64(A.shape[0])
    s, o, st = C.c_int64(sym), C.c_int64(ooc), C.c_int64(0)
    rowval = (A.indices.astype(np.int64) + 1)
    colptr = (A.indptr.astype(np.int64) + 1)
    is_c = np.iscomplexobj(A.data)
    vals = np.ascontiguousarray(A.data.astype(np.complex128 if is_c else np.float64))
    fn = lib.factor_mumps_cmplx_ if is_c else lib.factor_mumps_
    ptr = fn(C.byref(n), C.byref(s), C.byref(o), vals.ctypes.data_as(_f64p), i64(rowval), i64(colptr), C.byref(st))
    check(st.value, "factorMUMPS")
    return MUMPSfactorization(ptr, A.shape[0], is_c)


def applyMUMPS(factor: MUMPSfactorization, rhs, tr: int = 0):
    lib = load()
    rhs = np.asarray(rhs)
    if rhs.shape[0] != factor.n:
        raise ValueError(f"applyMUMPS: wrong size of rhs, size(A)={factor.n}, size(rhs)={rhs.shape}")
    nrhs = 1 if rhs.ndim == 1 else rhs.shape[1]
    cplx_io = factor.is_complex or np.iscomplexobj(rhs)
    dt = np.complex128 if cplx_io else np.float64
    b = np.asfortranarray(rhs.astype(dt).reshape(factor.n, nrhs))
    x = np.zeros_like(b, order="F")
    h, nr, t = C.c_int64(factor.ptr), C.c_int64(nrhs), C.c_int64(tr)
    fn = lib.solve_mumps_cmplx_ if cplx_io else lib.solve_mumps_
    rc = fn(C.byref(h), C.byref(nr), b.ctypes.data_as(_f64p), x.ctypes.data_as(_f64p), C.byref(t))
    check(rc, "applyMUMPS")
    return x[:, 0].copy() if rhs.ndim == 1 else np.ascontiguousarray(x)


def destroyMUMPS(factor: MUMPSfactorization):
    lib = load()
    h = C.c_int64(factor.ptr)
    (lib.destroy_mumps_cmplx_ if factor.is_complex else lib.destroy_mumps_)(C.byref(h))
    factor.ptr, factor.n = -1, -1


def solveMUMPS(A, rhs, sym: int = 0, ooc: int = 0, tr: int = 0):
    f = factorMUMPS(A, sym, ooc)
    try:
        return applyMUMPS(f, rhs, tr)
    finally:
        destroyMUMPS(f)
```

include/hmcmt_b200.h:

```cpp
#ifndef HMCMT_B200_H
#define HMCMT_B200_H

#include <stdint.h>

#ifdef __cplusplus
extern "C" {
#endif


int64_t factor_mumps_cmplx_(const int64_t* n, const int64_t* sym, const int64_t* ooc, const double* nzval,
                            const int64_t* rowval, const int64_t* colptr, int64_t* status);
int64_t factor_mumps_(const int64_t* n, const int64_t* sym, const int64_t* ooc, const double* nzval,
                      const int64_t* rowval, const int64_t* colptr, int64_t* status);
int64_t solve_mumps_cmplx_(const int64_t* handle, const int64_t* nrhs, const double* rhs, double* x,
                           const int64_t* transpose);
int64_t solve_mumps_(const int64_t* handle, const int64_t* nrhs, const double* rhs, double* x,
                     const int64_t* transpose);
void solve_mumps_sparse_rhs_(const int64_t* handle, const int64_t* nzrhs, const int64_t* nrhs, const double* nzval,
                             const int64_t* rowval, const int64_t* colptr, double* x, const int64_t* transpose);
void solve_mumps_cmplx_sparse_rhs_(const int64_t* handle, const int64_t* nzrhs, const int64_t* nrhs,
                                   const double* nzval, const int64_t* rowval, const int64_t* colptr, double* x,
                                   const int64_t* transpose);
int64_t destroy_mumps_(const int64_t* handle);
int64_t destroy_mumps_cmplx_(const int64_t* handle);


typedef struct hmcmt_plan hmcmt_plan;

typedef struct hmcmt_problem {
    int32_t ny, nz;
    const double* yLen;
    const double* zLen;
    double origin[2];
    int32_t nFreq;
    const double* freqs;
    int32_t nRx;
    const double* rxLoc;
    int32_t nComp;
    const int32_t* compMode;
    int32_t nData;
    const int64_t* freqID;
    const int64_t* rxID;
    const int64_t* dtID;
    const double* obsData;
    const double* dataErr;
    int32_t nAC;
    const int32_t* activeIdx;
    const double* bgModel;
    const int32_t* wmRowPtr;
    const int32_t* wmColIdx;
    const double* wmVal;
    double regParam;
    double sigBounds[2];
    int32_t nChains;
    int32_t device;
} hmcmt_problem;

int hmcmt_plan_create(const hmcmt_problem* prob, hmcmt_plan** out);
int hmcmt_plan_create_rho_phase(const hmcmt_problem* prob, hmcmt_plan** out);
void hmcmt_destroy(hmcmt_plan* plan);
int64_t hmcmt_plan_info(const hmcmt_plan* plan, int what);

int hmcmt_forward(hmcmt_plan* plan, const double* m, double* pred, double* exTE, double* hxTM);
int hmcmt_forward_sigma(hmcmt_plan* plan, const double* sigma, double* pred, double* exTE, double* hxTM);

int hmcmt_jtvec(hmcmt_plan* plan, const double* v, double* gsig);

int hmcmt_jacobian(hmcmt_plan* plan, double* J);

int hmcmt_jvec(hmcmt_plan* plan, const double* dsig, double* jv);
int hmcmt_gn_hessvec(hmcmt_plan* plan, const double* v, int32_t with_prior, double* hv);
int hmcmt_gauss_newton(hmcmt_plan* plan, const double* m0, int32_t maxIter, int32_t maxCG, double cgTol, int32_t maxLS,
                       double maxStep, double tolRel, double* m_out, double* history, int32_t* info);

int hmcmt_forward_gradient(hmcmt_plan* plan, const double* m, double* pred, double* phid, double* grad);
int hmcmt_forward_gradient_total(hmcmt_plan* plan, const double* m, double* pred, double* phid, double* grad);

int hmcmt_set_state(hmcmt_plan* plan, const double* m, const double* p, const double* mref);
int hmcmt_get_state(hmcmt_plan* plan, double* m, double* p);

int hmcmt_leapfrog_trajectory(hmcmt_plan* plan, double dt, const int32_t* intstep, double* stats, double* pred);

int hmcmt_leapfrog_steps_device(hmcmt_plan* plan, double dt, int32_t nsteps);

int hmcmt_step_partial(hmcmt_plan* plan, double dt);
int hmcmt_exchange_buffer(hmcmt_plan* plan, void** device_ptr, int64_t* count);
int hmcmt_step_finish(hmcmt_plan* plan, double dt);
int hmcmt_nccl_unique_id(char* out128);
int hmcmt_nccl_init(hmcmt_plan* plan, const char* id128, int32_t rank, int32_t world);
int hmcmt_leapfrog_steps_sharded(hmcmt_plan* plan, double dt, int32_t nsteps);
int hmcmt_sync(hmcmt_plan* plan);
int hmcmt_status(hmcmt_plan* plan);
int hmcmt_set_mass_matrix(hmcmt_plan* plan, int32_t kind);
int hmcmt_set_response_kind(hmcmt_plan* plan, int32_t kind);
int hmcmt_get_responses(hmcmt_plan* plan, double* out);
int hmcmt_timer_start(hmcmt_plan* plan);
int hmcmt_timer_stop(hmcmt_plan* plan, float* ms);
int hmcmt_kernel_time(hmcmt_plan* plan, int reset, float* factor_ms, int64_t* factor_launches);
int hmcmt_kernel_time_split(hmcmt_plan* plan, float* factor_only_ms, float* forward_solve_ms);

int hmcmt_run_chain(hmcmt_plan* plan, double dt, int32_t nsamples, double rhoref, const double* m_start, const double* z_init,
                    const int32_t* intsteps, const double* u_accept, const double* z_mom, int32_t reuse_last_forward,
                    double* hmcmodel, double* hmstats, int32_t* accept, double* hmcdata);

int hmcmt_export_system(hmcmt_plan* plan, int32_t chain, int32_t mode, int32_t freq, int64_t* colptr, int64_t* rowval,
                        double* nzval, double* rhs, double* bc);

const char* hmcmt_version(void);

#ifdef __cplusplus
}
#endif
#endif
```

Baseline: 282.7.

## Pack one-warp small fronts into multi-warp CTAs with warp-local shared-memory slices

Adds a tiny-front kernel in which each warp of an 8-warp CTA factorises its own small front inside a private shared-memory slice. Barriers become warp-level syncs, and fronts are bin-packed into CTAs under a per-CTA shared-memory budget. The aim is to cut the launch and block-scheduling overhead of many one-warp CTAs, which a per-SM resident-block limit can leave underused, and to raise occupancy. In exchange it uses the larger pivot-column layout for these fronts, may leave unused slots in a CTA, and also adds an arena zero-fill and an arena export debug API.

Result: faster. 290.8, median of 6 (+2.9%).

```diff
diff --git a/hmcmt2d_b200/csrc/hmcmt_b200.cu b/hmcmt2d_b200/csrc/hmcmt_b200.cu
--- a/hmcmt2d_b200/csrc/hmcmt_b200.cu
+++ b/hmcmt2d_b200/csrc/hmcmt_b200.cu
@@ -1122,6 +1122,12 @@
     }
 }
 
+int hmcmt_mf_arena(hmcmt_plan* pl, int32_t part, double* out, int64_t* count) {
+    if (!pl || !pl->useMf || !count) return kErrArg;
+    HMCMT_CUDA_TRY(cudaDeviceSynchronize());
+    return pl->mfs->copy_arena(part, out, count);
+}
+
 int hmcmt_sync(hmcmt_plan* pl) {
     if (!pl) return kErrArg;
     HMCMT_CUDA_TRY(cudaStreamSynchronize(pl->stream));
diff --git a/hmcmt2d_b200/csrc/mf_kernels.cuh b/hmcmt2d_b200/csrc/mf_kernels.cuh
--- a/hmcmt2d_b200/csrc/mf_kernels.cuh
+++ b/hmcmt2d_b200/csrc/mf_kernels.cuh
@@ -25,7 +25,7 @@
     int* status;
     unsigned long long* prof;
 };
-#define MF_PROF_MARK(slot) do { if (tb.prof && threadIdx.x == 0) { const long long _t = clock64(); atomicAdd(tb.prof + _pc * 8 + (slot), (unsigned long long)(_t - _t0)); _t0 = _t; } } while (0)
+#define MF_PROF_MARK(slot) do { if (tb.prof && tid == 0) { const long long _t = clock64(); atomicAdd(tb.prof + _pc * 8 + (slot), (unsigned long long)(_t - _t0)); _t0 = _t; } } while (0)
 
 __device__ __forceinline__ int tl_off(int r, int c) { return ((c >> 2) << 5) | (r << 2) | (c & 3); }
 __device__ __forceinline__ double* mf_tile(double* tiles, int I, int J) { return tiles + (size_t)(I * (I + 1) / 2 + J) * 128; }
@@ -67,20 +67,26 @@
         dmma884(x.im, a.im[kk], b.re[kk]);
     }
 }
+template <bool WARP>
+__device__ __forceinline__ void mf_sync() {
+    if (WARP) __syncwarp();
+    else __syncthreads();
+}
 __device__ __forceinline__ void frag_zero(TileFrag& c) { c.re[0] = c.re[1] = c.im[0] = c.im[1] = 0.0; }
 __device__ __forceinline__ void frag_add(TileFrag& c, const TileFrag& x) {
     c.re[0] += x.re[0]; c.re[1] += x.re[1]; c.im[0] += x.im[0]; c.im[1] += x.im[1];
 }
 
-template <int NW, bool PC = false, bool STREAM = false>
+template <int NW, bool PC = false, bool STREAM = false, bool WARP = false>
 __device__ __forceinline__ void mf_front_factor(double* __restrict__ tiles, double* __restrict__ scratch, double* __restrict__ mbuf,
                                                 double* __restrict__ nainv, int* __restrict__ fail, const int nb, const int npb,
                                                 const int sReal, unsigned long long* __restrict__ prof = nullptr,
                                                 double* mglob = nullptr, const int ldm = 0) {
-    const int tid = threadIdx.x, lane = tid & 31;
+    static_assert(!WARP || NW == 1, "a warp-local front is factorised by one warp");
+    const int tid = WARP ? threadIdx.x & 31 : threadIdx.x, lane = tid & 31;
     long long _s0 = prof ? clock64() : 0;
 #define MF_SWEEP_MARK(slot) do { if (prof && tid == 0) { const long long _t = clock64(); atomicAdd(prof + (slot), (unsigned long long)(_t - _s0)); _s0 = _t; } } while (0)
-    const int warp = __shfl_sync(0xffffffffu, tid >> 5, 0);
+    const int warp = WARP ? 0 : __shfl_sync(0xffffffffu, tid >> 5, 0);
     const int g = lane >> 2, t = lane & 3;
     double* const rawb = scratch;
     double* const mmb = scratch + (size_t)npb * 128;
@@ -101,7 +107,7 @@
             cfrag_store(p, Dw, g, t);
         }
         if (npb == 1) break;
-        __syncthreads();
+        mf_sync<WARP>();
         MF_SWEEP_MARK(0);
         for (int I = warp; I < npb; I += NW) {
             if (I == kb) continue;
@@ -115,7 +121,7 @@
             frag_store(a, rawb + (size_t)I * 128, lane);
             cfrag_store(c, mmb + (size_t)I * 128, g, t);
         }
-        __syncthreads();
+        mf_sync<WARP>();
         MF_SWEEP_MARK(1);
         {
             int I = 0, J = warp;
@@ -147,12 +153,12 @@
                 while (J > I) { J -= I + 1; ++I; }
             }
         }
-        __syncthreads();
+        mf_sync<WARP>();
         MF_SWEEP_MARK(1);
     }
     const int nub = nb - npb;
-    if (nub == 0) { __syncthreads(); return; }
-    __syncthreads();
+    if (nub == 0) { mf_sync<WARP>(); return; }
+    mf_sync<WARP>();
     if (npb == 1) MF_SWEEP_MARK(0);
     for (int Iu = warp; Iu < nub; Iu += NW) {
         const int I = npb + Iu;
@@ -176,7 +182,7 @@
             }
         }
     }
-    __syncthreads();
+    mf_sync<WARP>();
     MF_SWEEP_MARK(2);
     if (PC) return;
     {
@@ -216,7 +222,7 @@
             if (two) { frag_add(c1, x1); cfrag_store(c1, T1, g, t); }
         }
     }
-    __syncthreads();
+    mf_sync<WARP>();
     MF_SWEEP_MARK(3);
 #undef MF_SWEEP_MARK
 }
@@ -236,24 +242,38 @@
     }
 }
 
-template <int NW, bool STREAM>
+template <int NW, bool STREAM, bool TINY = false>
 __device__ __forceinline__ void mf_small_front(const Tables& tb, const SmallDesc* __restrict__ descs) {
+    static_assert(!TINY || (NW == 1 && !STREAM), "packed fronts are one-warp fronts");
     constexpr int NT = NW * 32;
-    constexpr bool kMid = NW >= 8;
+    constexpr bool kMid = NW >= 8 || TINY;
     static_assert(!STREAM || kMid, "streamed M' exists in the pivot-column layout only");
     extern __shared__ __align__(16) unsigned char mf_smem[];
-    SmallDesc& F = *reinterpret_cast<SmallDesc*>(mf_smem);
-    const int sys = blockIdx.y, tid = threadIdx.x, lane = tid & 31;
-    const int warp = __shfl_sync(0xffffffffu, tid >> 5, 0);
+    const int sys = blockIdx.y, tid = TINY ? threadIdx.x & 31 : threadIdx.x, lane = tid & 31;
+    const int warp = TINY ? 0 : __shfl_sync(0xffffffffu, tid >> 5, 0);
     constexpr int _pc = NW <= 2 ? 0 : (NW == 4 ? 1 : (NW == 8 ? 2 : 3));
     long long _t0 = clock64();
     static_assert(sizeof(SmallDesc) % 4 == 0 && sizeof(SmallDesc) <= kFrontDescBytes, "SmallDesc is copied word by word into the head of the dynamic shared memory");
-    for (int i = tid; i < (int)(sizeof(SmallDesc) / 4); i += NT)
-        reinterpret_cast<int*>(&F)[i] = reinterpret_cast<const int*>(descs + blockIdx.x)[i];
-    __syncthreads();
+    unsigned char* smem = mf_smem;
+    if (TINY) {
+        constexpr int kWords = sizeof(SmallDesc) / 4, kSliceWord = offsetof(SmallDesc, slice) / 4;
+        static_assert(kWords <= 64, "two words per lane");
+        const int* src = reinterpret_cast<const int*>(descs + (size_t)(blockDim.x >> 5) * blockIdx.x + (threadIdx.x >> 5));
+        const int w0 = src[lane], w1 = lane + 32 < kWords ? src[lane + 32] : 0;
+        const int slice = __shfl_sync(0xffffffffu, kSliceWord < 32 ? w0 : w1, kSliceWord & 31);
+        if (slice < 0) return;
+        smem += slice;
+        reinterpret_cast<int*>(smem)[lane] = w0;
+        if (lane + 32 < kWords) reinterpret_cast<int*>(smem)[lane + 32] = w1;
+    } else {
+        for (int i = tid; i < (int)(sizeof(SmallDesc) / 4); i += NT)
+            reinterpret_cast<int*>(smem)[i] = reinterpret_cast<const int*>(descs + blockIdx.x)[i];
+    }
+    SmallDesc& F = *reinterpret_cast<SmallDesc*>(smem);
+    mf_sync<TINY>();
     const int fp = F.sp + F.up, nb = fp >> 3, npb = F.sp >> 3, nub = nb - npb;
     const int nT = kMid ? mf_pc_row(nb, npb) : nb * (nb + 1) / 2;
-    double* tiles = reinterpret_cast<double*>(mf_smem + kFrontDescBytes);
+    double* tiles = reinterpret_cast<double*>(smem + kFrontDescBytes);
     double* mbuf = tiles + (size_t)nT * 128;
     double* nainv = mbuf + (size_t)(STREAM || 2 * npb > nub * npb ? 2 * npb : nub * npb) * 128;
     int* fail = reinterpret_cast<int*>(nainv + 128);
@@ -321,7 +341,7 @@
     if (kMid)
         for (int i = tid; i < nChild * F.up; i += NT) invS[i] = -1;
     if (tid == 0) *fail = 0;
-    __syncthreads();
+    mf_sync<TINY>();
     MF_PROF_MARK(0);
     if (kMid) {
         int base = 0;
@@ -363,9 +383,9 @@
                 load_batch(b1);
             }
             __syncwarp();
-            __syncthreads();
-        }
-        if (nChild == 0) __syncthreads();
+            mf_sync<TINY>();
+        }
+        if (nChild == 0) mf_sync<TINY>();
     }
     MF_PROF_MARK(2);
     if (tid < F.nOrig) {
@@ -380,10 +400,10 @@
         d[0] += v.x;
         d[64] += v.y;
     }
-    __syncthreads();
+    mf_sync<TINY>();
     MF_PROF_MARK(1);
     double* fac = tb.fac + (size_t)sys * tb.facStride;
-    mf_front_factor<NW, kMid, STREAM>(tiles, mbuf, mbuf, nainv, fail, nb, npb, F.s, tb.prof ? tb.prof + 32 + _pc * 4 : nullptr,
+    mf_front_factor<NW, kMid, STREAM, TINY>(tiles, mbuf, mbuf, nainv, fail, nb, npb, F.s, tb.prof ? tb.prof + 32 + _pc * 4 : nullptr,
                                       fac + F.mOff, F.up);
     if (kMid && nub > 0) {
         const long long tD = tb.prof ? clock64() : 0;
@@ -411,16 +431,19 @@
         };
         if (!STREAM) {
             const int nU = nub * (nub + 1) / 2;
+            constexpr int kPer = TINY ? 1 : 2;
             int I = 0, J = warp;
             while (J > I) { J -= I + 1; ++I; }
-            for (int L = warp; L < nU; L += 2 * NW) {
+            for (int L = warp; L < nU; L += kPer * NW) {
                 const int I0 = I, J0 = J;
                 J += NW;
                 while (J > I) { J -= I + 1; ++I; }
-                const bool two = L + NW < nU;
+                const bool two = kPer == 2 && L + NW < nU;
                 const int I1 = I, J1 = J;
-                J += NW;
-                while (J > I) { J -= I + 1; ++I; }
+                if (kPer == 2) {
+                    J += NW;
+                    while (J > I) { J -= I + 1; ++I; }
+                }
                 TileFrag c0, x0, c1, x1;
                 gather(c0, I0, J0);
                 frag_zero(x0);
@@ -516,6 +539,9 @@
 __global__ void __launch_bounds__(NW * 32, NW <= 4 ? (NW == 1 ? 16 : 32 / NW) : (NW == 8 ? 4 : 2))
 mf_small_kernel(Tables tb, const SmallDesc* __restrict__ descs) {
     mf_small_front<NW, false>(tb, descs);
+}
+__global__ void __launch_bounds__(kTinyWarps * 32, kTinyCtasPerSm) mf_tiny_kernel(Tables tb, const SmallDesc* __restrict__ descs) {
+    mf_small_front<1, false, true>(tb, descs);
 }
 __global__ void __launch_bounds__(16 * 32, 1) mf_small_stream_kernel(Tables tb, const SmallDesc* __restrict__ descs) {
     mf_small_front<16, true>(tb, descs);
diff --git a/hmcmt2d_b200/csrc/mf_solver.cu b/hmcmt2d_b200/csrc/mf_solver.cu
--- a/hmcmt2d_b200/csrc/mf_solver.cu
+++ b/hmcmt2d_b200/csrc/mf_solver.cu
@@ -27,6 +27,12 @@
     static PerDeviceOnceMf once;
     if (once.need()) HMCMT_CUDA_TRY(cudaFuncSetAttribute(mf_small_kernel<NW>, cudaFuncAttributeMaxDynamicSharedMemorySize, (int)kMaxSmem));
     mf_small_kernel<NW><<<dim3(n, nsys), NW * 32, smem, st>>>(tb, list);
+    return kOk;
+}
+int launch_tiny(cudaStream_t st, const Tables& tb, const SmallDesc* list, int nCta, int warps, int nsys, size_t smem) {
+    static PerDeviceOnceMf once;
+    if (once.need()) HMCMT_CUDA_TRY(cudaFuncSetAttribute(mf_tiny_kernel, cudaFuncAttributeMaxDynamicSharedMemorySize, (int)kMaxSmem));
+    mf_tiny_kernel<<<dim3(nCta, nsys), warps * 32, smem, st>>>(tb, list);
     return kOk;
 }
 int launch_stream(cudaStream_t st, const Tables& tb, const SmallDesc* list, int n, int nsys, size_t smem) {
@@ -119,7 +125,10 @@
         return (int)kOk;
     };
     MF_TRY(dalloc((void**)&d_fac, (size_t)nsys * S.factorDoubles * sizeof(double)));
-    for (int p = 0; p < 2; ++p) MF_TRY(dalloc((void**)&d_arena[p], (size_t)nsys * S.arenaDoubles[p] * sizeof(double)));
+    for (int p = 0; p < 2; ++p) {
+        MF_TRY(dalloc((void**)&d_arena[p], (size_t)nsys * S.arenaDoubles[p] * sizeof(double)));
+        if (cudaMemset(d_arena[p], 0, (size_t)nsys * S.arenaDoubles[p] * sizeof(double)) != cudaSuccess) return kErrCuda;
+    }
     MF_TRY(dalloc((void**)&d_vals, (size_t)nsys * valCount * sizeof(cplx)));
     MF_TRY(dalloc((void**)&d_v, (size_t)nsys * maxRhs * S.Np * sizeof(cplx)));
     MF_TRY(dalloc((void**)&d_upd, (size_t)nsys * maxRhs * S.updEntries * sizeof(cplx)));
@@ -143,13 +152,16 @@
             D.smallStream = mf_small_stream(S, sm);
             D.smallWarps = D.smallStream ? 16 : mf_small_warps(mx, knobs);
             D.smallSmem = 0;
+            const bool tiny = D.smallWarps == 1 && knobs.tiny;
             std::vector<SmallDesc> descs;
+            std::vector<size_t> slices;
             for (int k : sm) {
                 const Front& F = S.fronts[k];
                 const int nb = F.fp() / 8, npb = F.sp / 8, rt = mf_rel_total(S, k);
                 D.smallSmem = std::max(D.smallSmem, D.smallStream ? mf_stream_front_smem_bytes(nb, npb, rt, F.nChild)
                                                     : D.smallWarps >= 8 ? mf_mid_front_smem_bytes(nb, npb, rt, F.nChild)
                                                                         : mf_front_smem_bytes(nb, npb, rt));
+                slices.push_back(mf_tiny_slice_bytes(nb, npb, rt, F.nChild));
                 SmallDesc sd{};
                 sd.sp = F.sp; sd.up = F.up; sd.s = F.s; sd.nChild = F.nChild; sd.nOrig = F.nOrig; sd.origPtr = F.origPtr;
                 sd.par = F.depth & 1; sd.front = k;
@@ -163,6 +175,22 @@
                     sd.cPiv[c] = (unsigned char)piv;
                 }
                 descs.push_back(sd);
+            }
+            if (tiny) {
+                std::vector<int> place;
+                std::vector<size_t> off;
+                const char* ew = std::getenv("HMCMT_MF_TINY_W");
+                const char* es = std::getenv("HMCMT_MF_TINY_SORT");
+                D.tinyWarps = ew ? std::atoi(ew) : kTinyWarps;
+                const size_t budget = (size_t)228 * 1024 * D.tinyWarps / (kTinyWarps * kTinyCtasPerSm) - 1024;
+                D.tinyCtas = mf_tiny_pack(slices, place, off, D.smallSmem, D.tinyWarps, budget, es && std::atoi(es));
+                std::vector<SmallDesc> packed((size_t)D.tinyCtas * D.tinyWarps, SmallDesc{});
+                for (SmallDesc& e : packed) e.slice = -1;
+                for (size_t i = 0; i < descs.size(); ++i) {
+                    packed[place[i]] = descs[i];
+                    packed[place[i]].slice = (int)off[i];
+                }
+                descs.swap(packed);
             }
             SmallDesc* pd = nullptr;
             if (D.smallSmem > kMaxSmem) return kErrArg;
@@ -274,6 +302,14 @@
     return kOk;
 }
 
+int Solver::copy_arena(int part, double* out, int64_t* count) const {
+    if (part < 0 || part > 2) return kErrArg;
+    const double* src = part == 0 ? d_fac : d_arena[part - 1];
+    *count = (int64_t)nsys * (part == 0 ? S.factorDoubles : S.arenaDoubles[part - 1]);
+    if (out && *count) HMCMT_CUDA_TRY(cudaMemcpy(out, src, (size_t)*count * sizeof(double), cudaMemcpyDeviceToHost));
+    return kOk;
+}
+
 int Solver::set_mt_values(cudaStream_t st, int N, const MtValSys* dSys, int sys0, int n) {
     if (valCount < 3 * (int64_t)N) return kErrArg;
     if (n < 0) n = nsys - sys0;
@@ -304,6 +340,7 @@
         if (D.nSmall) {
             int rc = kOk;
             if (D.smallStream) rc = launch_stream(st, tb, D.smallDescs, D.nSmall, nsys, D.smallSmem);
+            else if (D.tinyCtas) rc = launch_tiny(st, tb, D.smallDescs, D.tinyCtas, D.tinyWarps, nsys, D.smallSmem);
             else if (D.smallWarps == 1) rc = launch_small<1>(st, tb, D.smallDescs, D.nSmall, nsys, D.smallSmem);
             else if (D.smallWarps == 2) rc = launch_small<2>(st, tb, D.smallDescs, D.nSmall, nsys, D.smallSmem);
             else if (D.smallWarps == 4) rc = launch_small<4>(st, tb, D.smallDescs, D.nSmall, nsys, D.smallSmem);
diff --git a/hmcmt2d_b200/csrc/mf_solver.cuh b/hmcmt2d_b200/csrc/mf_solver.cuh
--- a/hmcmt2d_b200/csrc/mf_solver.cuh
+++ b/hmcmt2d_b200/csrc/mf_solver.cuh
@@ -21,6 +21,7 @@
     int64_t cOff[kDescChildren];
     int cLd[kDescChildren], cFirst[kDescChildren], cU[kDescChildren], cRel[kDescChildren];
     unsigned char cPiv[kDescChildren];
+    int slice;
 };
 
 constexpr int kDescRows = 40;
@@ -37,6 +38,8 @@
     bool smallStream = false;
     size_t smallSmem = 0;
     const SmallDesc* smallDescs = nullptr;
+    int tinyCtas = 0;
+    int tinyWarps = kTinyWarps;
     int nBig = 0;
     const int* bigList = nullptr;
     int nOrigPairs = 0;
@@ -83,6 +86,7 @@
     size_t device_bytes() const { return bytes; }
     double factor_flops() const { return S.flops; }
     int64_t factor_doubles() const { return S.factorDoubles; }
+    int copy_arena(int part, double* out, int64_t* count) const;
 
   private:
     Solver() = default;
diff --git a/hmcmt2d_b200/csrc/mf_symbolic.h b/hmcmt2d_b200/csrc/mf_symbolic.h
--- a/hmcmt2d_b200/csrc/mf_symbolic.h
+++ b/hmcmt2d_b200/csrc/mf_symbolic.h
@@ -39,6 +39,36 @@
 inline size_t mf_large_front_smem_bytes(int nb, int npb, int relTotal, int nChild) {
     return mf_front_needs_stream(nb, npb, relTotal, nChild) ? mf_stream_front_smem_bytes(nb, npb, relTotal, nChild)
                                                             : mf_mid_front_smem_bytes(nb, npb, relTotal, nChild);
+}
+
+constexpr int kTinyWarps = 8;
+constexpr int kTinyCtasPerSm = 3;
+constexpr size_t kTinyCtaSmem = 228 * 1024 / kTinyCtasPerSm - 1024;
+inline size_t mf_tiny_slice_bytes(int nb, int npb, int relTotal, int nChild) {
+    return (mf_mid_front_smem_bytes(nb, npb, relTotal, nChild) + 15) & ~(size_t)15;
+}
+inline int mf_tiny_pack(const std::vector<size_t>& bytes, std::vector<int>& place, std::vector<size_t>& off, size_t& ctaBytes,
+                        int warps = kTinyWarps, size_t budget = kTinyCtaSmem, bool bySize = false) {
+    place.assign(bytes.size(), 0);
+    off.assign(bytes.size(), 0);
+    ctaBytes = 0;
+    std::vector<int> order(bytes.size());
+    std::iota(order.begin(), order.end(), 0);
+    if (bySize) std::stable_sort(order.begin(), order.end(), [&](int a, int b) { return bytes[a] > bytes[b]; });
+    int nCta = 0, inCta = warps;
+    size_t used = 0;
+    for (int i : order) {
+        if (inCta == warps || (inCta > 0 && used + bytes[i] > budget)) {
+            ++nCta;
+            inCta = 0;
+            used = 0;
+        }
+        place[i] = warps * (nCta - 1) + inCta++;
+        off[i] = used;
+        used += bytes[i];
+        ctaBytes = std::max(ctaBytes, used);
+    }
+    return nCta;
 }
 
 struct Entry {
@@ -445,12 +475,14 @@
 struct SchedKnobs {
     int fp1 = 40, fp2 = 40, fp4 = 64, fp8 = 96;
     int solveThreads = 0;
+    int tiny = 1;
     static SchedKnobs from_env() {
         auto knob = [](const char* name, int dflt) { const char* e = std::getenv(name); return e ? std::atoi(e) : dflt; };
         SchedKnobs k;
         k.fp1 = knob("HMCMT_MF_FP1", k.fp1); k.fp2 = knob("HMCMT_MF_FP2", k.fp2);
         k.fp4 = knob("HMCMT_MF_FP4", k.fp4); k.fp8 = knob("HMCMT_MF_FP8", k.fp8);
         k.solveThreads = knob("HMCMT_MF_SOLVE_THREADS", 0);
+        k.tiny = knob("HMCMT_MF_TINY", k.tiny);
         return k;
     }
 };
diff --git a/hmcmt2d_b200/csrc/mumps_shim.cu b/hmcmt2d_b200/csrc/mumps_shim.cu
--- a/hmcmt2d_b200/csrc/mumps_shim.cu
+++ b/hmcmt2d_b200/csrc/mumps_shim.cu
@@ -72,8 +72,8 @@
 const mf::Symbolic* symbolic_for(int64_t n, const int64_t* rowval, const int64_t* colptr) {
     const int64_t nnz = colptr[n] - 1;
     const mf::SchedKnobs sk = mf::SchedKnobs::from_env();
-    const int64_t knobs[7] = {mf_leaf_size(), mf_small_front(), sk.fp1, sk.fp2, sk.fp4, sk.fp8, sk.solveThreads};
-    PatternKey key{n, nnz, fnv(knobs, 7, fnv(rowval, nnz, fnv(colptr, n + 1, 0xcbf29ce484222325ull)))};
+    const int64_t knobs[8] = {mf_leaf_size(), mf_small_front(), sk.fp1, sk.fp2, sk.fp4, sk.fp8, sk.solveThreads, sk.tiny};
+    PatternKey key{n, nnz, fnv(knobs, 8, fnv(rowval, nnz, fnv(colptr, n + 1, 0xcbf29ce484222325ull)))};
     {
         std::lock_guard<std::mutex> lk(g_mu);
         auto it = g_symbolic.find(key);
diff --git a/hmcmt2d_b200/lib.py b/hmcmt2d_b200/lib.py
--- a/hmcmt2d_b200/lib.py
+++ b/hmcmt2d_b200/lib.py
@@ -54,6 +54,7 @@
     lib.hmcmt_destroy.restype = None
     lib.hmcmt_plan_info.argtypes = [vp, C.c_int]
     lib.hmcmt_plan_info.restype = C.c_int64
+    lib.hmcmt_mf_arena.argtypes = [vp, C.c_int32, _f64p, _i64p]
     lib.hmcmt_forward.argtypes = [vp, _f64p, _f64p, _f64p, _f64p]
     lib.hmcmt_forward_sigma.argtypes = [vp, _f64p, _f64p, _f64p, _f64p]
     lib.hmcmt_jtvec.argtypes = [vp, _f64p, _f64p]
@@ -109,7 +110,7 @@
 EXPORTED_SYMBOLS = [
     "factor_mumps_cmplx_", "factor_mumps_", "solve_mumps_cmplx_", "solve_mumps_", "solve_mumps_sparse_rhs_",
     "solve_mumps_cmplx_sparse_rhs_", "destroy_mumps_", "destroy_mumps_cmplx_",
-    "hmcmt_plan_create", "hmcmt_plan_create_rho_phase", "hmcmt_destroy", "hmcmt_plan_info", "hmcmt_forward", "hmcmt_forward_sigma", "hmcmt_jtvec",
+    "hmcmt_plan_create", "hmcmt_plan_create_rho_phase", "hmcmt_destroy", "hmcmt_plan_info", "hmcmt_mf_arena", "hmcmt_forward", "hmcmt_forward_sigma", "hmcmt_jtvec",
     "hmcmt_forward_gradient", "hmcmt_forward_gradient_total", "hmcmt_jacobian", "hmcmt_jvec", "hmcmt_gn_hessvec", "hmcmt_gauss_newton", "hmcmt_status", "hmcmt_set_mass_matrix", "hmcmt_set_response_kind", "hmcmt_get_responses",
     "hmcmt_set_state", "hmcmt_get_state", "hmcmt_leapfrog_trajectory", "hmcmt_leapfrog_steps_device", "hmcmt_sync",
     "hmcmt_step_partial", "hmcmt_exchange_buffer", "hmcmt_step_finish", "hmcmt_nccl_unique_id", "hmcmt_nccl_init",
diff --git a/include/hmcmt_b200.h b/include/hmcmt_b200.h
--- a/include/hmcmt_b200.h
+++ b/include/hmcmt_b200.h
@@ -60,6 +60,7 @@
 int hmcmt_plan_create_rho_phase(const hmcmt_problem* prob, hmcmt_plan** out);
 void hmcmt_destroy(hmcmt_plan* plan);
 int64_t hmcmt_plan_info(const hmcmt_plan* plan, int what);
+int hmcmt_mf_arena(hmcmt_plan* plan, int32_t part, double* out, int64_t* count);
 
 int hmcmt_forward(hmcmt_plan* plan, const double* m, double* pred, double* exTE, double* hxTM);
 int hmcmt_forward_sigma(hmcmt_plan* plan, const double* sigma, double* pred, double* exTE, double* hxTM);
```
